# AmandineBtto/NeRAF

Measured on AMD Instinct MI355X. Metric: field-samples/sec (rays + RIR STFT bins), higher is better.
Workload: dtype f16; 1 GPU; RAF FurnishedRoom joint training step (BASELINE configs[2]): 4096 rays + 2048 RIR slices x 513 bins per GPU; radiance + grid refresh + ResNet3D + NAcF + STFT loss, backward, GradScaler + fused Adam...; rays_per_gpu=4096, slices_per_gpu=2048, global_rays=4096, global_slices=2048, parallelism=dp1, distinct_resident_batches=16, deterministic=True

## Files before the change

### include/neraf_hip.h

```cpp
#ifndef NERAF_HIP_H
#define NERAF_HIP_H

#include <stddef.h>
#include <stdint.h>

#ifdef __cplusplus
extern "C" {
#endif

typedef struct neraf_ctx neraf_ctx;
typedef void* neraf_stream_t;

enum {
  NERAF_OK = 0,
  NERAF_EINVAL = -1,
  NERAF_EHIP = -2,
  NERAF_ENOGPU = -3,
  NERAF_ESTATE = -4
};

#define NERAF_ABI_VERSION 1

int neraf_abi_version(void);
int neraf_ctx_create(neraf_ctx** out, int device);
// ... 76 lines not shown
int neraf_stft_loss_bwd(neraf_ctx* ctx, const float* pred, const float* gt, size_t n, size_t n_total,
                        int loss_type, const float* sums, const float* g_sc, const float* g_mag, const float* weights, float extra,
                        float* dpred, neraf_stream_t stream);

typedef struct neraf_grid_desc {
  int n_levels;
  int base_res;
  int max_res;
  int log2_hashmap_size;
  int n_features;
} neraf_grid_desc;

int neraf_grid_layout(const neraf_grid_desc* g, float* scales, int* resolutions, uint32_t* sizes, uint32_t* offsets);

int neraf_hash_encode(neraf_ctx* ctx, const neraf_grid_desc* g, const void* table_f16, const float* x01, long long n_points,
                      float* enc, neraf_stream_t stream);

int neraf_sample_uniform(neraf_ctx* ctx, int R, int S, float near, float far, const float* jitter, uint64_t jitter_seed,
                         float* s_bins, float* e_bins, neraf_stream_t stream);

int neraf_proposal_density(neraf_ctx* ctx, const neraf_grid_desc* g, const void* table_f16, const void* mlp_f16,
                           const float* origins, const float* dirs, const float* e_bins, int R, int S,
                           float avg_density, int coherent_rays, float* density, neraf_stream_t stream);
int neraf_proposal_density_ex(neraf_ctx* ctx, const neraf_grid_desc* g, const void* table_f16, const void* mlp_f16,
                              const float* origins, const float* dirs, const float* e_bins, int64_t e_row_stride, int R, int S,
                              float avg_density, int coherent_rays, float* density, neraf_stream_t stream);

int neraf_pdf_resample(neraf_ctx* ctx, const float* density, const float* s_bins, const float* e_bins, int R, int S,
                       float anneal, const float* jitter, uint64_t jitter_seed, int n_new, float near, float far, float* weights,
                       float* s_new, float* e_new, neraf_stream_t stream);
int neraf_pdf_resample_ex(neraf_ctx* ctx, const float* density, const float* s_bins, const float* e_bins, int64_t bins_row_stride,
                          int R, int S, float anneal, const float* jitter, uint64_t jitter_seed, int n_new, float near, float far,
                          float* weights, float* s_new, float* e_new, neraf_stream_t stream);

int neraf_pdf_resample_mm(neraf_ctx* ctx, const float* density, const float* s_bins, const float* e_bins, int64_t bins_row_stride,
                          int R, int S, float anneal, const float* jitter, uint64_t jitter_seed, int n_new, float near, float far,
                          float* weights, float* s_new, float* e_new, void* minmax_scratch, size_t scratch_bytes, int minmax_mode,
                          neraf_stream_t stream);

int neraf_field_query(neraf_ctx* ctx, const neraf_grid_desc* g, const void* table_f16, const void* wfrag_f16,
                      const void* emb_f16, const float* origins, const float* dirs, const float* e_bins,
                      const int32_t* cam_idx, int R, int S, int mode, const float* aabb_host, float avg_density,
                      int avg_row, int coherent_rays, float* rgb, float* density, neraf_stream_t stream);

int neraf_field_query_train(neraf_ctx* ctx, const neraf_grid_desc* g, const void* table_f16, const void* wfrag_f16,
                            const void* emb_f16, const float* origins, const float* dirs, const float* e_bins,
                            const int32_t* cam_idx, int R, int S, int mode, const float* aabb_host, float avg_density,
                            int avg_row, float* rgb, float* density, void* enc_out, void* denc_out, neraf_stream_t stream);

int neraf_composite(neraf_ctx* ctx, const float* density, const float* rgb, const float* e_bins, int R, int S,
                    int training, float* weights, float* rgb_out, float* depth, float* expected, float* acc,
                    void* scratch, size_t scratch_bytes, neraf_stream_t stream);
int neraf_composite_mm(neraf_ctx* ctx, const float* density, const float* rgb, const float* e_bins, int R, int S,
                       int training, float* weights, float* rgb_out, float* depth, float* expected, float* acc,
                       const void* minmax, neraf_stream_t stream);

int neraf_render_loss(neraf_ctx* ctx, const float* density, const float* rgb_s, const float* e_bins, const float* s_bins,
                      const float* gt_rgb, int R, int S, float distortion_mult, const float* up3, float* d_rgb_s,
                      float* d_density, float* d_density_dist, float* sums, neraf_stream_t stream);
int neraf_interlevel_loss(neraf_ctx* ctx, const float* c_bins, const float* w_fine, int S2, const float* p_bins,
                          const float* p_ebins, const float* p_density, int Sp, int R, float mult, const float* up3,
                          float* d_density, float* sums, neraf_stream_t stream);
size_t neraf_proposal_backward_scratch_bytes(int R, int S, int n_levels);
int neraf_proposal_backward(neraf_ctx* ctx, const neraf_grid_desc* g, const void* table_f16, const void* mlp_f16,
                            const float* origins, const float* dirs, const float* e_bins, const float* d_density, int R,
                            int S, float avg_density, float* table_grad, float* w_grad, void* scratch, size_t scratch_bytes,
                            neraf_stream_t stream);
size_t neraf_field_backward_dump_bytes(int R, int S);
int neraf_field_backward(neraf_ctx* ctx, const neraf_grid_desc* g, const void* table_f16, const void* wfrag_f16,
                         const void* wfrag_bwd_f16, const void* emb_f16, const float* origins, const float* dirs,
                         const float* e_bins, const int32_t* cam_idx, int R, int S, int mode, const float* aabb_host,
                         float avg_density, int avg_row, const float* density, const float* d_rgb, const float* d_density,
                         float* table_grad, float* emb_grad, float* const* w_grads, void* dump, void* splitk_ws,
                         size_t splitk_bytes, neraf_stream_t stream);

int neraf_field_backward_runs(neraf_ctx* ctx, const neraf_grid_desc* g, const void* table_f16, const void* wfrag_f16,
                         const void* wfrag_bwd_f16, const void* emb_f16, const float* origins, const float* dirs,
                         const float* e_bins, const int32_t* cam_idx, int R, int S, int mode, const float* aabb_host,
                         float avg_density, int avg_row, const float* density, const float* d_rgb, const float* d_density,
                         float* table_grad, float* emb_grad, float* const* w_grads, void* dump, void* splitk_ws,
                         size_t splitk_bytes, int pos_run, neraf_stream_t stream);

int neraf_field_backward_rays(neraf_ctx* ctx, const neraf_grid_desc* g, const void* table_f16, const void* wfrag_f16,
                              const void* wfrag_bwd_f16, const void* emb_f16, const float* origins, const float* dirs,
                              const float* e_bins, const int32_t* cam_idx, int R, int S, int mode, const float* aabb_host,
                              float avg_density, int avg_row, const float* density, const float* d_rgb, const float* d_density,
                              float* table_grad, float* emb_grad, float* const* w_grads, void* dump, void* splitk_ws,
                              size_t splitk_bytes, float* d_rays, neraf_stream_t stream);
int neraf_field_backward_ex(neraf_ctx* ctx, const neraf_grid_desc* g, const void* table_f16, const void* wfrag_f16,
                            const void* wfrag_bwd_f16, const void* emb_f16, const float* origins, const float* dirs,
                            const float* e_bins, const int32_t* cam_idx, int R, int S, int mode, const float* aabb_host,
                            float avg_density, int avg_row, const float* density, const float* d_rgb, const float* d_density,
                            float* table_grad, float* emb_grad, float* const* w_grads, void* dump, void* splitk_ws,
                            size_t splitk_bytes, int pos_run, float* d_rays, const void* enc_saved, const void* denc_saved,
                            void* acc_scratch, int accumulate, int emb_rows, neraf_stream_t stream);
int neraf_proposal_backward_ex(neraf_ctx* ctx, const neraf_grid_desc* g, const void* table_f16, const void* mlp_f16,
                               const float* origins, const float* dirs, const float* e_bins, const float* d_density, int R, int S,
                               float avg_density, float* table_grad, float* w0_grad, float* w1_grad, void* scratch,
                               size_t scratch_bytes, void* acc_scratch, float* d_rays, neraf_stream_t stream);
int neraf_proposal_backward_rays(neraf_ctx* ctx, const neraf_grid_desc* g, const void* table_f16, const void* mlp_f16,
                                 const float* origins, const float* dirs, const float* e_bins, const float* d_density, int R,
                                 int S, float avg_density, float* table_grad, float* w_grad, void* scratch, size_t scratch_bytes,
                                 float* d_rays, neraf_stream_t stream);

int neraf_grid_refresh_write(neraf_ctx* ctx, const float* rgb, const float* density, int n, int ndirs, float delta,
                             float* grid, size_t nvox, size_t start, neraf_stream_t stream);

int neraf_grid_refresh_vals(neraf_ctx* ctx, const float* rgb, const float* density, int n, int ndirs, int cell_major, float delta,
                            float* vals, float* grid, size_t nvox, size_t start, neraf_stream_t stream);
int neraf_grid_refresh_vals_bwd(neraf_ctx* ctx, const float* dvals, const float* density, int n, int ndirs, int cell_major,
                                float delta, float* d_rgb, float* d_density, neraf_stream_t stream);

int neraf_refresh_origins(neraf_ctx* ctx, const float* coords, int n, int ndirs, const float* aabb_host, float* out,
                          neraf_stream_t stream);

typedef struct neraf_resnet3d_desc {
  int grid_size;
  int in_channels;
  int n_features;
} neraf_resnet3d_desc;

int neraf_resnet3d_num_convs(const neraf_resnet3d_desc* d);
size_t neraf_resnet3d_packed_bytes(const neraf_resnet3d_desc* d);
size_t neraf_resnet3d_workspace_bytes(const neraf_resnet3d_desc* d);
double neraf_resnet3d_forward_flops(const neraf_resnet3d_desc* d);
int neraf_resnet3d_pack_weights(neraf_ctx* ctx, const neraf_resnet3d_desc* d, const float* const* conv_w, void* packed,
                                neraf_stream_t stream);
int neraf_resnet3d_fwd(neraf_ctx* ctx, const neraf_resnet3d_desc* d, const void* packed, const float* const* bn,
                       const float* grid, void* workspace, float* feat, int use_batch_stats, size_t win_start, int win_cells,
                       neraf_stream_t stream);
int neraf_resnet3d_update_running_stats(neraf_ctx* ctx, const neraf_resnet3d_desc* d, const void* workspace,
                                        float* const* bn, float momentum, int64_t* const* num_batches_tracked,
                                        neraf_stream_t stream);

size_t neraf_resnet3d_bwd_packed_bytes(const neraf_resnet3d_desc* d);
size_t neraf_resnet3d_bwd_workspace_bytes(const neraf_resnet3d_desc* d);
int neraf_resnet3d_pack_weights_bwd(neraf_ctx* ctx, const neraf_resnet3d_desc* d, const float* const* conv_w, void* packed_t,
                                    neraf_stream_t stream);
int neraf_resnet3d_bwd(neraf_ctx* ctx, const neraf_resnet3d_desc* d, const void* packed_t, const float* const* conv_w,
                       const float* const* bn, void* workspace, void* bwd_workspace, const float* dfeat,
                       float* const* w_grads, float* const* bn_grads, size_t cell_start, int n_cells, int n_ch,
                       float* dgrid_cells, neraf_stream_t stream);
int neraf_resnet3d_bwd_reset(neraf_ctx* ctx, void* bwd_workspace);
int neraf_resnet3d_bwd_chain_state(neraf_ctx* ctx, const neraf_resnet3d_desc* d, const void* bwd_workspace, int32_t* e_out,
                                   float* amax_out, int n, int32_t* info2, neraf_stream_t stream);

int neraf_manifest_enable(neraf_ctx* ctx, int on);
int neraf_manifest_get(neraf_ctx* ctx, int index, char* name, int name_cap, double* flops, double* rbytes, double* wbytes);

int neraf_debug_conv_bn_relu_stage(neraf_ctx* ctx, int cin, int cin_real, int cout, int k, int stride, int pad, int din,
                                   const void* x_f16, const float* w, const float* gamma, const float* beta, const float* g,
                                   void* y_f16, float* dx, float* dw, float* dgamma, float* dbeta, neraf_stream_t stream);

int neraf_camera_rays(neraf_ctx* ctx, const float* c2w, const float* fx, const float* fy, const float* cx, const float* cy,
                      const float* distortion, int n_cams,
                      const int64_t* cam_idx, int cam_single, const float* coords, int R, int width, float* origins, float* dirs,
                      int64_t* cam_out, neraf_stream_t stream);
int neraf_camera_apply(neraf_ctx* ctx, const float* pose_adjustment, const int32_t* cam_idx, const float* origins, const float* dirs,
                       int R, float* origins_out, float* dirs_out, int n_cameras, float w_trans, float w_rot, float* reg_out3,
                       neraf_stream_t stream);
int neraf_camera_apply_bwd(neraf_ctx* ctx, const float* pose_adjustment, const int32_t* cam_idx, const float* dirs,
                           const float* d_origins, const float* d_dirs, int g_stride, int R, int n_cameras, float w_trans, float w_rot,
                           const float* g_reg, float* d_pose, neraf_stream_t stream);

int neraf_loss_sum_scale(neraf_ctx* ctx, const float* const* terms, int n, const float* scale, float* out2, neraf_stream_t stream);
int neraf_vision_loss_finalize(neraf_ctx* ctx, const float* sums, const float* k3, float* out4, neraf_stream_t stream);
int neraf_vision_bwd_prologue(neraf_ctx* ctx, const float* u_rgb, const float* u_dens, const float* u_dist, const float* g_rgb,
                              const float* g_inter, const float* g_dist, size_t n_samples, float* d_rgb, float* d_dens, float* up3,
                              float* d_rays, size_t n_ray_floats, float* sums4, neraf_stream_t stream);

int neraf_cvt_f16_segments(neraf_ctx* ctx, const float* const* src, void* const* dst, const long long* len, int n,
                           neraf_stream_t stream);
int neraf_gather_f16(neraf_ctx* ctx, const float* const* src, const long long* src_len, int nsrc, const long long* index, void* dst,
                     long long n, neraf_stream_t stream);

int neraf_resnet3d_debug_locate(const neraf_resnet3d_desc* d, int kind, int index, size_t* offset, int* rows, int* cols);

int neraf_debug_bn_apply(neraf_ctx* ctx, const void* x, const float* const* bn5, int rep, const void* xr, const float* const* bn5_r,
                         int rep_r, const void* res, int M, int Mpad, int C, int relu, float* fin_w, float* fin_w_r, void* out,
                         int form, neraf_stream_t stream);
int neraf_debug_maxpool_fwd(neraf_ctx* ctx, const void* x, const float* const* bn5, int rep, int din, void* out, void* arg,
                            neraf_stream_t stream);
int neraf_debug_maxpool_bwd(neraf_ctx* ctx, const void* arg, const void* g, int din, void* dpost, neraf_stream_t stream);

uint32_t neraf_debug_fastdiv(uint32_t n, uint32_t d);

int neraf_fused_adam_chunk(void);
int neraf_grads_nonfinite(neraf_ctx* ctx, const void* table, const void* g_ptrs, const int* blk_tensor, const int* blk_chunk,
                          int n_blocks, float* found_inf, const void* const* g_ptrs_host, int n_ptrs, int found_is_zero,
                          neraf_stream_t stream);
int neraf_amp_update_scale(neraf_ctx* ctx, float* scale, int32_t* growth_tracker, const float* const* found_infs, int n,
                           double growth_factor, double backoff_factor, int growth_interval, int clear_flags, neraf_stream_t stream);
int neraf_fused_adam(neraf_ctx* ctx, const void* table, const void* g_ptrs, const int* blk_tensor, const int* blk_chunk,
                     int n_blocks, const float* group_lr, int n_groups, int n_tensors, double beta1, double beta2, double eps,
                     float* step, const float* grad_scale, const float* found_inf, neraf_stream_t stream);

int neraf_fused_adam_dual(neraf_ctx* ctx, const void* table, const void* g_ptrs, const int* blk_tensor, const int* blk_chunk,
                          int n_blocks, const float* group_lr, int n_groups, int n_tensors, double beta1, double beta2, double eps,
                          float* step, const float* grad_scale, const float* found_inf, const void* dual, const float* step0,
                          const float* found_inf0, const float* group_lr0, int n_groups0, const void* const* g_ptrs_host, int n_ptrs,
                          neraf_stream_t stream);

#ifdef __cplusplus
}
#endif
#endif
```

### neraf_amd/_lib.py

```python
from __future__ import annotations

import ctypes as C
import os
from typing import Dict, Optional

_HERE = os.path.dirname(os.path.abspath(__file__))
LIB_PATH = os.environ.get("NERAF_HIP_LIB") or os.path.join(_HERE, "libneraf_hip.so")

_lib: Optional[C.CDLL] = None
_ctxs: Dict[int, C.c_void_p] = {}

c_fpp = C.POINTER(C.c_void_p)


class GridDesc(C.Structure):
    _fields_ = [("n_levels", C.c_int), ("base_res", C.c_int), ("max_res", C.c_int), ("log2_hashmap_size", C.c_int),
                ("n_features", C.c_int)]


class ResnetDesc(C.Structure):
    _fields_ = [("grid_size", C.c_int), ("in_channels", C.c_int), ("n_features", C.c_int)]


class NacfDesc(C.Structure):
# ... 14 lines not shown
                                         C.c_void_p]),
    "neraf_gemm_f16_stream": (C.c_int, [C.c_void_p, C.c_void_p, C.c_int, C.c_void_p, C.c_int, C.c_int, C.c_int, C.c_int, C.c_int, C.c_int,
                                        C.c_float, C.c_void_p, C.c_void_p, C.c_int, C.c_void_p, C.c_int, C.c_void_p, C.c_int, C.c_void_p,
                                        C.c_int, C.c_void_p, C.c_void_p, C.c_int, C.c_int, C.c_int, C.c_int, C.c_int, C.c_void_p]),
    "neraf_gemm_bf16": (C.c_int, [C.c_void_p, C.c_void_p, C.c_int, C.c_void_p, C.c_int, C.c_int, C.c_int, C.c_int,
                                  C.c_int, C.c_int, C.c_float, C.c_void_p, C.c_int, C.c_void_p, C.c_int, C.c_void_p,
                                  C.c_int, C.c_void_p, C.c_int, C.c_void_p]),
    "neraf_gemm_bf16_tn": (C.c_int, [C.c_void_p, C.c_void_p, C.c_void_p, C.c_int, C.c_int, C.c_int, C.c_void_p, C.c_void_p, C.c_size_t,
                                     C.c_void_p]),
    "neraf_fused_adam_chunk": (C.c_int, []),
    "neraf_grads_nonfinite": (C.c_int, [C.c_void_p, C.c_void_p, C.c_void_p, C.c_void_p, C.c_void_p, C.c_int, C.c_void_p, C.c_void_p, C.c_int,
                                        C.c_int, C.c_void_p]),
    "neraf_fused_adam": (C.c_int, [C.c_void_p, C.c_void_p, C.c_void_p, C.c_void_p, C.c_void_p, C.c_int, C.c_void_p, C.c_int, C.c_int,
                                   C.c_double, C.c_double, C.c_double, C.c_void_p, C.c_void_p, C.c_void_p, C.c_void_p]),
    "neraf_fused_adam_dual": (C.c_int, [C.c_void_p, C.c_void_p, C.c_void_p, C.c_void_p, C.c_void_p, C.c_int, C.c_void_p, C.c_int, C.c_int,
                                        C.c_double, C.c_double, C.c_double, C.c_void_p, C.c_void_p, C.c_void_p, C.c_void_p, C.c_void_p,
                                        C.c_void_p, C.c_void_p, C.c_int, C.c_void_p, C.c_int, C.c_void_p]),
    "neraf_nacf_packed_bytes": (C.c_size_t, [C.POINTER(NacfDesc)]),
    "neraf_nacf_workspace_bytes": (C.c_size_t, [C.POINTER(NacfDesc), C.c_int, C.c_int]),
    "neraf_nacf_pack_weights": (C.c_int, [C.c_void_p, C.POINTER(NacfDesc), c_fpp, C.c_void_p, C.c_void_p]),
    "neraf_nacf_encode_queries": (C.c_int, [C.c_void_p, C.POINTER(NacfDesc), C.c_void_p, C.c_void_p, C.c_void_p,
                                            C.c_void_p, C.POINTER(C.c_float), C.c_int, C.c_int, C.c_void_p, C.c_int,
                                            C.c_void_p]),
    "neraf_nacf_encode_queries_ex": (C.c_int, [C.c_void_p, C.POINTER(NacfDesc), C.c_void_p, C.c_void_p, C.c_void_p,
                                               C.c_void_p, C.c_int, C.POINTER(C.c_float), C.c_int, C.c_int, C.c_void_p, C.c_int,
                                               C.c_void_p]),
    "neraf_nacf_fwd": (C.c_int, [C.c_void_p, C.POINTER(NacfDesc), C.c_void_p, c_fpp, C.c_void_p, C.c_int, C.c_void_p,
                                 C.c_void_p, C.c_int, C.c_void_p]),
    "neraf_nacf_fwd_dense": (C.c_int, [C.c_void_p, C.POINTER(NacfDesc), C.c_void_p, C.c_void_p, C.c_int, C.c_void_p,
                                       C.c_void_p, C.c_int, C.c_void_p]),
    "neraf_nacf_bwd": (C.c_int, [C.c_void_p, C.POINTER(NacfDesc), C.c_void_p, c_fpp, C.c_void_p, C.c_int, C.c_void_p,
                                 C.c_void_p, c_fpp, C.c_void_p, C.c_void_p, C.c_void_p]),
    "neraf_nacf_bwd_dense": (C.c_int, [C.c_void_p, C.POINTER(NacfDesc), C.c_void_p, C.c_int, C.c_void_p, C.c_void_p,
                                       c_fpp, C.c_void_p, C.c_void_p, C.c_void_p]),
    "neraf_stft_loss_fwd": (C.c_int, [C.c_void_p, C.c_void_p, C.c_void_p, C.c_size_t, C.c_int, C.c_void_p, C.c_void_p,
                                      C.c_void_p]),
    "neraf_stft_loss_sums": (C.c_int, [C.c_void_p, C.c_void_p, C.c_void_p, C.c_size_t, C.c_int, C.c_void_p, C.c_void_p]),
    "neraf_stft_loss_finalize": (C.c_int, [C.c_void_p, C.c_void_p, C.c_size_t, C.c_void_p, C.c_void_p, C.c_void_p]),
    "neraf_stft_loss_bwd": (C.c_int, [C.c_void_p, C.c_void_p, C.c_void_p, C.c_size_t, C.c_size_t, C.c_int, C.c_void_p,
                                      C.c_void_p, C.c_void_p, C.c_void_p, C.c_float, C.c_void_p, C.c_void_p]),
    "neraf_prof_event_overhead": (C.c_int, [C.c_void_p, C.c_void_p, C.c_void_p, C.POINTER(C.c_double)]),
    "neraf_graph_stats": (C.c_int, [C.c_void_p, C.POINTER(C.c_int), C.POINTER(C.c_int)]),
    "neraf_prof_enable": (C.c_int, [C.c_void_p, C.c_int]),
    "neraf_prof_summary": (C.c_int, [C.c_void_p, C.c_int, C.POINTER(C.c_double), C.POINTER(C.c_int), C.POINTER(C.c_double)]),
    "neraf_prof_summary_ex": (C.c_int, [C.c_void_p, C.c_int, C.POINTER(C.c_double), C.POINTER(C.c_int), C.POINTER(C.c_double),
                                        C.POINTER(C.c_double)]),
    "neraf_prof_kernel_name": (C.c_char_p, [C.c_int]),
    "neraf_grid_layout": (C.c_int, [C.POINTER(GridDesc), C.POINTER(C.c_float), C.POINTER(C.c_int), C.POINTER(C.c_uint32),
                                    C.POINTER(C.c_uint32)]),
    "neraf_hash_encode": (C.c_int, [C.c_void_p, C.POINTER(GridDesc), C.c_void_p, C.c_void_p, C.c_longlong, C.c_void_p, C.c_void_p]),
    "neraf_sample_uniform": (C.c_int, [C.c_void_p, C.c_int, C.c_int, C.c_float, C.c_float, C.c_void_p, C.c_uint64, C.c_void_p,
                                       C.c_void_p, C.c_void_p]),
    "neraf_proposal_density": (C.c_int, [C.c_void_p, C.POINTER(GridDesc), C.c_void_p, C.c_void_p, C.c_void_p, C.c_void_p,
                                         C.c_void_p, C.c_int, C.c_int, C.c_float, C.c_int, C.c_void_p, C.c_void_p]),
    "neraf_proposal_density_ex": (C.c_int, [C.c_void_p, C.POINTER(GridDesc), C.c_void_p, C.c_void_p, C.c_void_p, C.c_void_p,
                                            C.c_void_p, C.c_int64, C.c_int, C.c_int, C.c_float, C.c_int, C.c_void_p, C.c_void_p]),
    "neraf_pdf_resample_ex": (C.c_int, [C.c_void_p, C.c_void_p, C.c_void_p, C.c_void_p, C.c_int64, C.c_int, C.c_int, C.c_float,
                                        C.c_void_p, C.c_uint64, C.c_int, C.c_float, C.c_float, C.c_void_p, C.c_void_p, C.c_void_p,
                                        C.c_void_p]),
    "neraf_pdf_resample_mm": (C.c_int, [C.c_void_p, C.c_void_p, C.c_void_p, C.c_void_p, C.c_int64, C.c_int, C.c_int, C.c_float,
                                        C.c_void_p, C.c_uint64, C.c_int, C.c_float, C.c_float, C.c_void_p, C.c_void_p, C.c_void_p,
                                        C.c_void_p, C.c_size_t, C.c_int, C.c_void_p]),
    "neraf_composite_mm": (C.c_int, [C.c_void_p, C.c_void_p, C.c_void_p, C.c_void_p, C.c_int, C.c_int, C.c_int, C.c_void_p,
                                     C.c_void_p, C.c_void_p, C.c_void_p, C.c_void_p, C.c_void_p, C.c_void_p]),
    "neraf_pdf_resample": (C.c_int, [C.c_void_p, C.c_void_p, C.c_void_p, C.c_void_p, C.c_int, C.c_int, C.c_float,
                                     C.c_void_p, C.c_uint64, C.c_int, C.c_float, C.c_float, C.c_void_p, C.c_void_p, C.c_void_p,
                                     C.c_void_p]),
    "neraf_field_query": (C.c_int, [C.c_void_p, C.POINTER(GridDesc), C.c_void_p, C.c_void_p, C.c_void_p, C.c_void_p,
                                    C.c_void_p, C.c_void_p, C.c_void_p, C.c_int, C.c_int, C.c_int, C.POINTER(C.c_float),
                                    C.c_float, C.c_int, C.c_int, C.c_void_p, C.c_void_p, C.c_void_p]),
    "neraf_field_query_train": (C.c_int, [C.c_void_p, C.POINTER(GridDesc), C.c_void_p, C.c_void_p, C.c_void_p, C.c_void_p,
                                          C.c_void_p, C.c_void_p, C.c_void_p, C.c_int, C.c_int, C.c_int, C.POINTER(C.c_float),
                                          C.c_float, C.c_int, C.c_void_p, C.c_void_p, C.c_void_p, C.c_void_p, C.c_void_p]),
    "neraf_render_loss": (C.c_int, [C.c_void_p, C.c_void_p, C.c_void_p, C.c_void_p, C.c_void_p, C.c_void_p, C.c_int, C.c_int,
                                    C.c_float, C.c_void_p, C.c_void_p, C.c_void_p, C.c_void_p, C.c_void_p, C.c_void_p]),
    "neraf_interlevel_loss": (C.c_int, [C.c_void_p, C.c_void_p, C.c_void_p, C.c_int, C.c_void_p, C.c_void_p, C.c_void_p,
                                        C.c_int, C.c_int, C.c_float, C.c_void_p, C.c_void_p, C.c_void_p, C.c_void_p]),
    "neraf_proposal_backward_scratch_bytes": (C.c_size_t, [C.c_int, C.c_int, C.c_int]),
    "neraf_proposal_backward": (C.c_int, [C.c_void_p, C.POINTER(GridDesc), C.c_void_p, C.c_void_p, C.c_void_p, C.c_void_p,
                                          C.c_void_p, C.c_void_p, C.c_int, C.c_int, C.c_float, C.c_void_p, C.c_void_p,
                                          C.c_void_p, C.c_size_t, C.c_void_p]),
    "neraf_field_backward_dump_bytes": (C.c_size_t, [C.c_int, C.c_int]),
    "neraf_field_backward": (C.c_int, [C.c_void_p, C.POINTER(GridDesc), C.c_void_p, C.c_void_p, C.c_void_p, C.c_void_p,
                                       C.c_void_p, C.c_void_p, C.c_void_p, C.c_void_p, C.c_int, C.c_int, C.c_int,
                                       C.POINTER(C.c_float), C.c_float, C.c_int, C.c_void_p, C.c_void_p, C.c_void_p,
                                       C.c_void_p, C.c_void_p, c_fpp, C.c_void_p, C.c_void_p, C.c_size_t, C.c_void_p]),
    "neraf_field_backward_runs": (C.c_int, [C.c_void_p, C.POINTER(GridDesc), C.c_void_p, C.c_void_p, C.c_void_p, C.c_void_p,
                                            C.c_void_p, C.c_void_p, C.c_void_p, C.c_void_p, C.c_int, C.c_int, C.c_int,
                                            C.POINTER(C.c_float), C.c_float, C.c_int, C.c_void_p, C.c_void_p, C.c_void_p,
                                            C.c_void_p, C.c_void_p, c_fpp, C.c_void_p, C.c_void_p, C.c_size_t, C.c_int, C.c_void_p]),
    "neraf_field_backward_rays": (C.c_int, [C.c_void_p, C.POINTER(GridDesc), C.c_void_p, C.c_void_p, C.c_void_p, C.c_void_p,
                                            C.c_void_p, C.c_void_p, C.c_void_p, C.c_void_p, C.c_int, C.c_int, C.c_int,
                                            C.POINTER(C.c_float), C.c_float, C.c_int, C.c_void_p, C.c_void_p, C.c_void_p,
                                            C.c_void_p, C.c_void_p, c_fpp, C.c_void_p, C.c_void_p, C.c_size_t, C.c_void_p, C.c_void_p]),
    "neraf_field_backward_ex": (C.c_int, [C.c_void_p, C.POINTER(GridDesc), C.c_void_p, C.c_void_p, C.c_void_p, C.c_void_p,
                                          C.c_void_p, C.c_void_p, C.c_void_p, C.c_void_p, C.c_int, C.c_int, C.c_int,
                                          C.POINTER(C.c_float), C.c_float, C.c_int, C.c_void_p, C.c_void_p, C.c_void_p,
                                          C.c_void_p, C.c_void_p, c_fpp, C.c_void_p, C.c_void_p, C.c_size_t, C.c_int, C.c_void_p,
                                          C.c_void_p, C.c_void_p, C.c_void_p, C.c_int, C.c_int, C.c_void_p]),
    "neraf_proposal_backward_ex": (C.c_int, [C.c_void_p, C.POINTER(GridDesc), C.c_void_p, C.c_void_p, C.c_void_p, C.c_void_p,
                                             C.c_void_p, C.c_void_p, C.c_int, C.c_int, C.c_float, C.c_void_p, C.c_void_p, C.c_void_p,
                                             C.c_void_p, C.c_size_t, C.c_void_p, C.c_void_p, C.c_void_p]),
    "neraf_proposal_backward_rays": (C.c_int, [C.c_void_p, C.POINTER(GridDesc), C.c_void_p, C.c_void_p, C.c_void_p, C.c_void_p,
                                               C.c_void_p, C.c_void_p, C.c_int, C.c_int, C.c_float, C.c_void_p, C.c_void_p,
                                               C.c_void_p, C.c_size_t, C.c_void_p, C.c_void_p]),
    "neraf_grid_refresh_write": (C.c_int, [C.c_void_p, C.c_void_p, C.c_void_p, C.c_int, C.c_int, C.c_float, C.c_void_p,
                                           C.c_size_t, C.c_size_t, C.c_void_p]),
    "neraf_grid_refresh_vals": (C.c_int, [C.c_void_p, C.c_void_p, C.c_void_p, C.c_int, C.c_int, C.c_int, C.c_float, C.c_void_p,
                                          C.c_void_p, C.c_size_t, C.c_size_t, C.c_void_p]),
    "neraf_grid_refresh_vals_bwd": (C.c_int, [C.c_void_p, C.c_void_p, C.c_void_p, C.c_int, C.c_int, C.c_int, C.c_float, C.c_void_p,
                                              C.c_void_p, C.c_void_p]),
    "neraf_refresh_origins": (C.c_int, [C.c_void_p, C.c_void_p, C.c_int, C.c_int, C.POINTER(C.c_float), C.c_void_p, C.c_void_p]),
    "neraf_resnet3d_num_convs": (C.c_int, [C.POINTER(ResnetDesc)]),
    "neraf_resnet3d_packed_bytes": (C.c_size_t, [C.POINTER(ResnetDesc)]),
    "neraf_resnet3d_workspace_bytes": (C.c_size_t, [C.POINTER(ResnetDesc)]),
    "neraf_resnet3d_forward_flops": (C.c_double, [C.POINTER(ResnetDesc)]),
    "neraf_resnet3d_pack_weights": (C.c_int, [C.c_void_p, C.POINTER(ResnetDesc), c_fpp, C.c_void_p, C.c_void_p]),
    "neraf_resnet3d_fwd": (C.c_int, [C.c_void_p, C.POINTER(ResnetDesc), C.c_void_p, c_fpp, C.c_void_p, C.c_void_p,
                                     C.c_void_p, C.c_int, C.c_size_t, C.c_int, C.c_void_p]),
    "neraf_resnet3d_update_running_stats": (C.c_int, [C.c_void_p, C.POINTER(ResnetDesc), C.c_void_p, c_fpp, C.c_float, c_fpp,
                                                      C.c_void_p]),
    "neraf_resnet3d_bwd_packed_bytes": (C.c_size_t, [C.POINTER(ResnetDesc)]),
    "neraf_resnet3d_bwd_workspace_bytes": (C.c_size_t, [C.POINTER(ResnetDesc)]),
    "neraf_resnet3d_pack_weights_bwd": (C.c_int, [C.c_void_p, C.POINTER(ResnetDesc), c_fpp, C.c_void_p, C.c_void_p]),
    "neraf_manifest_enable": (C.c_int, [C.c_void_p, C.c_int]),
    "neraf_manifest_get": (C.c_int, [C.c_void_p, C.c_int, C.c_char_p, C.c_int, C.POINTER(C.c_double), C.POINTER(C.c_double), C.POINTER(C.c_double)]),
    "neraf_resnet3d_bwd_reset": (C.c_int, [C.c_void_p, C.c_void_p]),
    "neraf_resnet3d_bwd_chain_state": (C.c_int, [C.c_void_p, C.POINTER(ResnetDesc), C.c_void_p, C.POINTER(C.c_int32), C.POINTER(C.c_float),
                                                 C.c_int, C.POINTER(C.c_int32), C.c_void_p]),
    "neraf_resnet3d_bwd": (C.c_int, [C.c_void_p, C.POINTER(ResnetDesc), C.c_void_p, c_fpp, c_fpp, C.c_void_p, C.c_void_p,
                                     C.c_void_p, c_fpp, c_fpp, C.c_size_t, C.c_int, C.c_int, C.c_void_p, C.c_void_p]),
    "neraf_camera_rays": (C.c_int, [C.c_void_p] * 7 + [C.c_int, C.c_void_p, C.c_int, C.c_void_p, C.c_int, C.c_int,
                                    C.c_void_p, C.c_void_p, C.c_void_p, C.c_void_p]),
    "neraf_camera_apply": (C.c_int, [C.c_void_p, C.c_void_p, C.c_void_p, C.c_void_p, C.c_void_p, C.c_int, C.c_void_p, C.c_void_p, C.c_int,
                                     C.c_float, C.c_float, C.c_void_p, C.c_void_p]),
    "neraf_camera_apply_bwd": (C.c_int, [C.c_void_p, C.c_void_p, C.c_void_p, C.c_void_p, C.c_void_p, C.c_void_p, C.c_int, C.c_int, C.c_int,
                                         C.c_float, C.c_float, C.c_void_p, C.c_void_p, C.c_void_p]),
    "neraf_amp_update_scale": (C.c_int, [C.c_void_p, C.c_void_p, C.c_void_p, c_fpp, C.c_int, C.c_double, C.c_double, C.c_int, C.c_int,
                                         C.c_void_p]),
    "neraf_loss_sum_scale": (C.c_int, [C.c_void_p, c_fpp, C.c_int, C.c_void_p, C.c_void_p, C.c_void_p]),
    "neraf_vision_loss_finalize": (C.c_int, [C.c_void_p, C.c_void_p, C.c_void_p, C.c_void_p, C.c_void_p]),
    "neraf_vision_bwd_prologue": (C.c_int, [C.c_void_p] * 7 + [C.c_size_t, C.c_void_p, C.c_void_p, C.c_void_p, C.c_void_p, C.c_size_t,
                                            C.c_void_p, C.c_void_p]),
    "neraf_cvt_f16_segments": (C.c_int, [C.c_void_p, c_fpp, c_fpp, C.POINTER(C.c_longlong), C.c_int, C.c_void_p]),
    "neraf_gather_f16": (C.c_int, [C.c_void_p, c_fpp, C.POINTER(C.c_longlong), C.c_int, C.c_void_p, C.c_void_p, C.c_longlong, C.c_void_p]),
    "neraf_debug_fastdiv": (C.c_uint32, [C.c_uint32, C.c_uint32]),
    "neraf_resnet3d_debug_locate": (C.c_int, [C.POINTER(ResnetDesc), C.c_int, C.c_int, C.POINTER(C.c_size_t), C.POINTER(C.c_int),
                                              C.POINTER(C.c_int)]),
    "neraf_debug_bn_apply": (C.c_int, [C.c_void_p, C.c_void_p, c_fpp, C.c_int, C.c_void_p, c_fpp, C.c_int, C.c_void_p, C.c_int, C.c_int, C.c_int,
                                       C.c_int, C.c_void_p, C.c_void_p, C.c_void_p, C.c_int, C.c_void_p]),
    "neraf_debug_maxpool_fwd": (C.c_int, [C.c_void_p, C.c_void_p, c_fpp, C.c_int, C.c_int, C.c_void_p, C.c_void_p, C.c_void_p]),
    "neraf_debug_maxpool_bwd": (C.c_int, [C.c_void_p, C.c_void_p, C.c_void_p, C.c_int, C.c_void_p, C.c_void_p]),
    "neraf_debug_conv_bn_relu_stage": (C.c_int, [C.c_void_p] + [C.c_int] * 7 + [C.c_void_p] * 11),
    "neraf_composite": (C.c_int, [C.c_void_p, C.c_void_p, C.c_void_p, C.c_void_p, C.c_int, C.c_int, C.c_int, C.c_void_p,
                                  C.c_void_p, C.c_void_p, C.c_void_p, C.c_void_p, C.c_void_p, C.c_size_t, C.c_void_p]),
}


def load() -> C.CDLL:
    global _lib
    if _lib is not None:
        return _lib
    if not os.path.exists(LIB_PATH):
        raise RuntimeError(
            f"{LIB_PATH} is missing: build it with `python -c 'import __graft_entry__ as g; g.build()'` "
            "(or `make -C neraf_amd/csrc`).  neraf_amd has no CPU / eager fallback by design.")
    lib = C.CDLL(LIB_PATH)
    variant = "NERAF_HIP_LIB" in os.environ
    for name, (res, args) in SIGNATURES.items():
        try:
            fn = getattr(lib, name)
        except AttributeError:
            if not variant:
                raise
            setattr(lib, name, lambda *a, **k: 0)
            continue
        fn.restype = res
        fn.argtypes = args
    if lib.neraf_abi_version() != 1:
        raise RuntimeError("libneraf_hip ABI version mismatch")
    _lib = lib
    return lib


def ctx(device_index: int = 0) -> C.c_void_p:
    if device_index in _ctxs:
        return _ctxs[device_index]
    lib = load()
    h = C.c_void_p()
    rc = lib.neraf_ctx_create(C.byref(h), device_index)
    if rc != 0:
        raise RuntimeError(f"neraf_ctx_create(device={device_index}) failed with {rc}: no MI355X/gfx950 GPU visible; "
                           "the NeRAF hot path only runs on the HIP library (no fallback).")
    _ctxs[device_index] = h
    return h


def check(rc: int, device_index: int = 0) -> None:
    if rc != 0:
        msg = load().neraf_last_error(_ctxs.get(device_index)) if device_index in _ctxs else b""
        raise RuntimeError(f"libneraf_hip call failed ({rc}): {msg.decode() if msg else ''}")


def ptr_array(tensors) -> "C.Array":
    arr = (C.c_void_p * len(tensors))()
    for i, t in enumerate(tensors):
        arr[i] = t.data_ptr() if t is not None else None
    return arr


_HOST_F32 = {}


def host_f32(t):
    key = (t.data_ptr(), t._version, t.numel())
    hit = _HOST_F32.get(key)
    if hit is None:
        vals = [float(v) for v in t.detach().reshape(-1).cpu().tolist()]
        hit = ((C.c_float * len(vals))(*vals), t.untyped_storage())
        if len(_HOST_F32) > 64:
            _HOST_F32.clear()
        _HOST_F32[key] = hit
    return hit[0]
```

### neraf_amd/csrc/gemm_f16.hip

```cpp
#include "common.h"
#include <stdlib.h>
#include <type_traits>

namespace {

constexpr int BK = 64;

__device__ __forceinline__ float act_apply(float v, int act) {
  if (act == ACT_LEAKY) return v > 0.f ? v : 0.1f * v;
  if (act == ACT_TANH10) return 10.f * tanhf(v);
  if (act == ACT_RELU) return v > 0.f ? v : 0.f;
  return v;
}

template <bool BF> struct ET;
template <> struct ET<false> {
  typedef _Float16 s; typedef half8 v8; typedef half4 v4;
  static __device__ __forceinline__ f32x4 mfma(v8 a, v8 b, f32x4 c) { return __builtin_amdgcn_mfma_f32_16x16x32_f16(a, b, c, 0, 0, 0); }
};
template <> struct ET<true> {
  typedef __bf16 s; typedef bf16x8 v8; typedef bf16x4 v4;
  static __device__ __forceinline__ f32x4 mfma(v8 a, v8 b, f32x4 c) { return __builtin_amdgcn_mfma_f32_16x16x32_bf16(a, b, c, 0, 0, 0); }
};

template <int BM, int BN, int WAVES_M = 2>
struct Tile {
  static constexpr int NWAVES = WAVES_M * 2, NT = NWAVES * 64;
  static constexpr int WM = BM / WAVES_M, WN = BN / 2;
  static constexpr int FM = WM / 16, FN = WN / 16;
  static constexpr int A_CH = BM * 8 / NT, B_CH = BN * 8 / NT;
  static constexpr int STAGE_BYTES = (BM + BN) * 128;
  static constexpr int IMG16_LD = WN + 8;
  static constexpr int IMG16T_LD = WM + 8;
  static constexpr int IMG32_LD = WN + 4;
  static constexpr int C32_PASSES = (NWAVES * WM * IMG32_LD * 4 > 144 * 1024) ? 2 : 1;
  static constexpr int cmax(int a, int b) { return a > b ? a : b; }
  static constexpr int EPI_BYTES_WAVE = cmax(cmax(WM / C32_PASSES * IMG32_LD * 4, WM * IMG16_LD * 2), WN * IMG16T_LD * 2);
};

template <int BM>
__device__ __forceinline__ void tclass_coords(const ConvGeom& g, int m, int& z, int& y, int& x) {
  const int t = m / BM, cls = t & 7;
  const int r = (t >> 3) * BM + (m - t * BM);
  const int h = g.dout >> 1;
  const int x2 = r % h, y2 = (r / h) % h, z2 = r / (h * h);
  z = 2 * z2 + ((cls >> 2) & 1); y = 2 * y2 + ((cls >> 1) & 1); x = 2 * x2 + (cls & 1);
}
template <int BM, bool TC>
__device__ __forceinline__ int out_row(const GemmParams& p, int m) {
  if (!TC) return m;
  int z, y, x;
  tclass_coords<BM>(p.conv, m, z, y, x);
  return (z * p.conv.dout + y) * p.conv.dout + x;
}

template <int BM, int BN, bool BF, int WAVES_M = 2, bool TC = false>
__device__ __forceinline__ void gemm_epilogue(const GemmParams& p, f32x4 (&acc)[Tile<BM, BN, WAVES_M>::FM][Tile<BM, BN, WAVES_M>::FN],
                                              char* smem, int bm, int bn, int lane, int wave, int M, int N, float* C32, int ldc32) {
  using T = Tile<BM, BN, WAVES_M>;
  using E = typename ET<BF>::s;
  using E4 = typename ET<BF>::v4;
  constexpr int WM = T::WM, WN = T::WN, FM = T::FM, FN = T::FN;
  const int wm = wave >> 1, wn = wave & 1;
  const int frow = lane & 15, fq = lane >> 4;
  const int m_tile0 = bm * BM, n_tile0 = bn * BN;
  const float alpha = p.alpha_dev ? p.alpha * (*p.alpha_dev) : p.alpha;
  const int m_l = frow;
  const int n_l = fq * 4;
#pragma unroll
  for (int i = 0; i < FM; ++i) {
    const int m = m_tile0 + wm * WM + i * 16 + m_l;
#pragma unroll
    for (int j = 0; j < FN; ++j) {
      const int n0 = n_tile0 + wn * WN + j * 16 + n_l;
      f32x4 v = acc[i][j] * alpha;
      if (p.bias) {
        const f32x4 b = *reinterpret_cast<const f32x4*>(p.bias + n0);
        v += b;
      }
#pragma unroll
      for (int r = 0; r < 4; ++r) v[r] = act_apply(v[r], p.act);
      if (p.lmask) {
        const E4 mk = *reinterpret_cast<const E4*>(reinterpret_cast<const E*>(p.lmask) + (size_t)m * p.ldmask + n0);
#pragma unroll
        for (int r = 0; r < 4; ++r) v[r] *= ((float)mk[r] > 0.f) ? 1.f : p.mask_slope;
      }
      if (p.add16) {
        const E4 ad = *reinterpret_cast<const E4*>(reinterpret_cast<const E*>(p.add16) + (size_t)out_row<BM, TC>(p, m) * p.ldadd + n0);
#pragma unroll
        for (int r = 0; r < 4; ++r) v[r] += (float)ad[r];
      }
      if (p.bnb_mask) {
        const E4 mk = *reinterpret_cast<const E4*>(reinterpret_cast<const E*>(p.bnb_mask) + (size_t)m * p.ldbnb + n0);
#pragma unroll
        for (int r = 0; r < 4; ++r) if (!((float)mk[r] > 0.f)) v[r] = 0.f;
      }
#pragma unroll
      for (int r = 0; r < 4; ++r)
        if (m >= M || (n0 + r) >= N) v[r] = 0.f;
      acc[i][j] = v;
    }
  }

  char* img = smem + wave * T::EPI_BYTES_WAVE;
  const int m_w0 = m_tile0 + wm * WM, n_w0 = n_tile0 + wn * WN;

  if (p.colsum || p.colsumsq) {
    float* red = reinterpret_cast<float*>(smem);
    static_assert(2 * BN <= T::NT, "one thread per (sum | sumsq, column)");
#pragma unroll
    for (int j = 0; j < FN; ++j) {
      f32x4 s = f32x4{0.f, 0.f, 0.f, 0.f}, s2 = f32x4{0.f, 0.f, 0.f, 0.f};
      if (p.bnb_x) {
        const int n0 = n_tile0 + wn * WN + j * 16 + n_l;
        const f32x4 mu = *reinterpret_cast<const f32x4*>(p.bnb_fin + n0);
        f32x4 rs = *reinterpret_cast<const f32x4*>(p.bnb_fin + p.bnb_cpad + n0);
#pragma unroll
        for (int r = 0; r < 4; ++r) rs[r] = rsqrtf(rs[r] + 1e-5f);
#pragma unroll
        for (int i = 0; i < FM; ++i) {
          const int m = m_tile0 + wm * WM + i * 16 + m_l;
          const half4 xv = *reinterpret_cast<const half4*>(p.bnb_x + (size_t)out_row<BM, TC>(p, m) * p.ldbnb + n0);
          s += acc[i][j];
#pragma unroll
          for (int r = 0; r < 4; ++r) s2[r] += acc[i][j][r] * (((float)xv[r] - mu[r]) * rs[r]);
        }
      } else {
#pragma unroll
        for (int i = 0; i < FM; ++i) { s += acc[i][j]; s2 += acc[i][j] * acc[i][j]; }
      }
#pragma unroll
      for (int r = 0; r < 4; ++r) {
        float x = s[r], y = s2[r];
#pragma unroll
        for (int o = 1; o < 16; o <<= 1) { x += __shfl_xor(x, o); y += __shfl_xor(y, o); }
        if (frow == 0) {
          const int col = wn * WN + j * 16 + n_l + r;
          red[(wm * 2 + 0) * BN + col] = x;
          red[(wm * 2 + 1) * BN + col] = y;
        }
      }
    }
    __syncthreads();
    const int t = wave * 64 + lane;
    if (t < 2 * BN) {
      const int which = t / BN, col = t - which * BN;
      float v = 0.f;
#pragma unroll
      for (int w = 0; w < WAVES_M; ++w) v += red[(w * 2 + which) * BN + col];
      float* dst = which ? p.colsumsq : p.colsum;
      if (p.stat_det) {
        if (dst) dst[(size_t)(m_tile0 >> 5) * p.stat_stride + n_tile0 + col] = v;
      } else {
        const int rep = p.stat_rep > 1 ? (bm & (p.stat_rep - 1)) * p.stat_stride : 0;
        if (dst) atomicAdd(dst + rep + n_tile0 + col, v);
      }
    }
    __syncthreads();
  }

  if (p.C16) {
    E* im = reinterpret_cast<E*>(img);
#pragma unroll
    for (int i = 0; i < FM; ++i)
#pragma unroll
      for (int j = 0; j < FN; ++j) {
        E4 h;
#pragma unroll
        for (int r = 0; r < 4; ++r) h[r] = (E)acc[i][j][r];
        *reinterpret_cast<E4*>(im + (i * 16 + m_l) * T::IMG16_LD + j * 16 + n_l) = h;
      }
    __syncthreads();
    constexpr int CPR = WN / 8;
    static_assert((WM * CPR) % 64 == 0 || WM * CPR < 64, "whole wave-instructions (or one partial one)");
#pragma unroll
    for (int it = 0; it < (WM * CPR + 63) / 64; ++it) {
      const int idx = it * 64 + lane, row = idx / CPR, ch = idx - row * CPR;
      if (WM * CPR < 64 && idx >= WM * CPR) break;
      const uint4 d = *reinterpret_cast<const uint4*>(im + row * T::IMG16_LD + ch * 8);
      *reinterpret_cast<uint4*>(p.C16 + (size_t)out_row<BM, TC>(p, m_w0 + row) * p.ldc16 + n_w0 + ch * 8) = d;
    }
    __syncthreads();
  }

  if (p.C16T) {
    E* im = reinterpret_cast<E*>(img);
#pragma unroll
    for (int i = 0; i < FM; ++i)
#pragma unroll
      for (int j = 0; j < FN; ++j)
#pragma unroll
        for (int r = 0; r < 4; ++r)
          im[(j * 16 + n_l + r) * T::IMG16T_LD + i * 16 + m_l] = (E)acc[i][j][r];
    __syncthreads();
    constexpr int CPR = WM / 8;
    static_assert((WN * CPR) % 64 == 0 || WN * CPR < 64, "whole wave-instructions (or one partial one)");
#pragma unroll
    for (int it = 0; it < (WN * CPR + 63) / 64; ++it) {
      const int idx = it * 64 + lane, row = idx / CPR, ch = idx - row * CPR;
      if (WN * CPR < 64 && idx >= WN * CPR) break;
      const uint4 d = *reinterpret_cast<const uint4*>(im + row * T::IMG16T_LD + ch * 8);
      *reinterpret_cast<uint4*>(p.C16T + (size_t)(n_w0 + row) * p.ldc16t + m_w0 + ch * 8) = d;
    }
    __syncthreads();
  }

  if (C32) {
    float* im = reinterpret_cast<float*>(img);
    constexpr int FMP = FM / T::C32_PASSES, ROWS = WM / T::C32_PASSES;
#pragma unroll
    for (int pass = 0; pass < T::C32_PASSES; ++pass) {
      if (pass) __syncthreads();
#pragma unroll
      for (int i = 0; i < FMP; ++i)
#pragma unroll
        for (int j = 0; j < FN; ++j)
          *reinterpret_cast<f32x4*>(im + (i * 16 + m_l) * T::IMG32_LD + j * 16 + n_l) = acc[pass * FMP + i][j];
      __syncthreads();
      const int m_p0 = m_w0 + pass * ROWS;
      if (WN % 64 == 0) {
#pragma unroll 4
        for (int row = 0; row < ROWS; ++row) {
          const int m = m_p0 + row;
          if (m >= M) break;
#pragma unroll
          for (int c0 = 0; c0 < WN; c0 += 64) {
            const int n = n_w0 + c0 + lane;
            if (n < N) {
              float* dst = C32 + (size_t)m * ldc32 + n;
              *dst = im[row * T::IMG32_LD + c0 + lane] + (p.c32_beta ? *dst : 0.f);
            }
          }
        }
      } else {
        static_assert((ROWS * WN) % 64 == 0, "whole wave-instructions");
#pragma unroll 4
        for (int it = 0; it < ROWS * WN / 64; ++it) {
          const int idx = it * 64 + lane, row = idx / WN, col = idx - row * WN;
          const int m = m_p0 + row, n = n_w0 + col;
          if (m < M && n < N) {
            float* dst = C32 + (size_t)m * ldc32 + n;
            *dst = im[row * T::IMG32_LD + col] + (p.c32_beta ? *dst : 0.f);
          }
        }
      }
    }
  }
}

template <int N> __device__ __forceinline__ void wait_vmcnt() { asm volatile("s_waitcnt vmcnt(%0)" ::"i"(N) : "memory"); }
template <int LOADS, int MAXT>
__device__ __forceinline__ void wait_tiles(int after) {
  static_assert(MAXT * LOADS <= 63, "vmcnt is a 6-bit counter");
  if constexpr (MAXT <= 0) { wait_vmcnt<0>(); }
  else {
    if (after >= MAXT) wait_vmcnt<MAXT * LOADS>();
    else wait_tiles<LOADS, MAXT - 1>(after);
  }
}

template <int BM, int BN, int NST>
struct PipeTile {
  using T = Tile<BM, BN>;
  static constexpr int LDS_BYTES =
      (NST * T::STAGE_BYTES > T::NWAVES * T::EPI_BYTES_WAVE) ? NST * T::STAGE_BYTES : T::NWAVES * T::EPI_BYTES_WAVE;
};

template <int BM, int BN, int NST, int LOADER, int KS, bool BF, bool TC = false, int NW = 4, bool GRP = false>
__global__ __launch_bounds__(NW * 64) void gemm_f16_nt_pipe_kernel(GemmParams p, int splits) {
  using T = Tile<BM, BN>;
  using E8 = typename ET<BF>::v8;
  constexpr int WM = T::WM, WN = T::WN, FM = T::FM, FN = T::FN;
  constexpr int KH = NW / 4, NTH = NW * 64;
  static_assert((NW == 4 || NW == 8) && T::A_CH % KH == 0 && T::B_CH % KH == 0, "4 waves, or 8 with whole chunks per thread");
  constexpr int A_CH = T::A_CH / KH, B_CH = T::B_CH / KH;
  constexpr int LOADS = A_CH + B_CH;
  extern __shared__ __attribute__((aligned(16))) char smem[];

  const int tid = threadIdx.x;
  const int lane = tid & 63;
  const int wave8 = __builtin_amdgcn_readfirstlane(tid >> 6);
  const int wave = wave8 & 3, kh = wave8 >> 2;
  const int wm = wave >> 1, wn = wave & 1;

  int tiles_m = p.Mpad / BM, tiles_n = p.Npad / BN;
  const int nblocks = GRP ? (int)gridDim.x : tiles_m * tiles_n * splits;
  int bid = blockIdx.x;
  {
    const int q = nblocks >> 3, r = nblocks & 7;
    const int xcd = bid & 7, idx = bid >> 3;
    bid = (xcd < r ? xcd * (q + 1) : r * (q + 1) + (xcd - r) * q) + idx;
  }
  const half_t* Ag = p.A; const half_t* Bg0 = p.B;
  float* C32g = p.C32; int Mg = p.M, Ng = p.N, ldc32g = p.ldc32, grp = 0;
  if constexpr (GRP) {
    while (grp + 1 < p.ngroups && bid >= p.grp[grp + 1].tile_begin * splits) ++grp;
    const GemmParams::Group& G = p.grp[grp];
    bid -= G.tile_begin * splits;
    tiles_m = (G.M + BM - 1) / BM; tiles_n = (G.N + BN - 1) / BN;
    Ag = G.A; Bg0 = G.B; C32g = G.C32; Mg = G.M; Ng = G.N; ldc32g = G.ldc32;
  }
  const int split = bid % splits;
  bid /= splits;
  constexpr int GROUP_M = 4;
  const int group = bid / (GROUP_M * tiles_n);
  const int first_m = group * GROUP_M;
  const int gsz = (tiles_m - first_m) < GROUP_M ? (tiles_m - first_m) : GROUP_M;
  const int in_group = bid - group * GROUP_M * tiles_n;
  const int bm = first_m + in_group % gsz;
  const int bn = in_group / gsz;

  constexpr bool tclass = LOADER == 1 && TC;
  int t0z = 0, t0y = 0, t0x = 0, cy = KS, cx = KS;
  int nk_total = p.K / BK;
  if (tclass) {
    const int cls = bm & 7, padc = -p.conv.pad;
    t0z = (((cls >> 2) & 1) + padc) & 1; t0y = (((cls >> 1) & 1) + padc) & 1; t0x = ((cls & 1) + padc) & 1;
    const int cz = t0z < KS ? (KS - t0z + 1) >> 1 : 0;
    cy = t0y < KS ? (KS - t0y + 1) >> 1 : 0; cx = t0x < KS ? (KS - t0x + 1) >> 1 : 0;
    nk_total = cz * cy * cx * (p.conv.cin >> 6);
    if (nk_total == 0 && p.add16 == p.C16 && !p.C16T && !p.C32 && !p.colsum && !p.colsumsq && splits == 1) return;
  }
  const int per = (nk_total + splits - 1) / splits;
  const int k_begin = split * per;
  const int k_end = (k_begin + per) < nk_total ? (k_begin + per) : nk_total;
  const int nk = k_end > k_begin ? k_end - k_begin : 0;

  const half_t* Bg = Bg0 + (size_t)bn * BN * p.ldb;
  const half_t* b_src[B_CH];
#pragma unroll
  for (int i = 0; i < B_CH; ++i) {
    const int c = i * NTH + tid, row = c >> 3, lc = (c & 7) ^ (row & 7);
    b_src[i] = Bg + (size_t)row * p.ldb + lc * 8;
  }
  const half_t* a_src[A_CH];
  int az[A_CH], ay[A_CH], ax[A_CH], alc[A_CH];
#pragma unroll
  for (int i = 0; i < A_CH; ++i) {
    const int c = i * NTH + tid, row = c >> 3, lc = (c & 7) ^ (row & 7);
    alc[i] = lc;
    az[i] = ay[i] = ax[i] = 0;
    a_src[i] = nullptr;
    if (LOADER == 0) {
      a_src[i] = Ag + (size_t)(bm * BM + row) * p.lda + lc * 8;
    } else {
      const int m = bm * BM + row;
      const int d = p.conv.dout;
      int x = m % d, y = (m / d) % d, z = m / (d * d);
      if (tclass) tclass_coords<BM>(p.conv, m, z, y, x);
      az[i] = z * p.conv.stride - p.conv.pad; ay[i] = y * p.conv.stride - p.conv.pad; ax[i] = x * p.conv.stride - p.conv.pad;
    }
  }
  const bool fastc = LOADER == 1 && (tclass || p.conv.tstride != 2) && nk_total > 0;
  int c_off[A_CH];
  unsigned c_msk[A_CH];
  int jz = 0, jy = 0, jx = 0, jcb = 0;
  const int lim_y = tclass ? cy : KS, lim_x = tclass ? cx : KS;
  const int tsgn = (LOADER == 1 && p.conv.tflip) ? -1 : 1;
  if (fastc) {
    const int cpb = p.conv.cin >> 6, din = p.conv.din;
    int t = k_begin / cpb;
    jcb = k_begin - t * cpb;
    jx = t % lim_x; t /= lim_x; jy = t % lim_y; jz = t / lim_y;
#pragma unroll
    for (int i = 0; i < A_CH; ++i) {
      int bz = az[i], by = ay[i], bx = ax[i];
      if (tclass) { bz = (bz - t0z) >> 1; by = (by - t0y) >> 1; bx = (bx - t0x) >> 1; }
      unsigned m = 0;
#pragma unroll
      for (int a = 0; a < KS; ++a) {
        m |= ((unsigned)(bz + tsgn * a) < (unsigned)din ? 1u : 0u) << a;
        m |= ((unsigned)(by + tsgn * a) < (unsigned)din ? 1u : 0u) << (8 + a);
        m |= ((unsigned)(bx + tsgn * a) < (unsigned)din ? 1u : 0u) << (16 + a);
      }
      c_msk[i] = m;
      c_off[i] = ((bz * din + by) * din + bx) * p.conv.cin + alc[i] * 8;
    }
  }

  typedef __attribute__((address_space(3))) void* lds_ptr_t;
  typedef const __attribute__((address_space(1))) void* gbl_ptr_t;
  auto issue = [&](int kt, int stage) {
    char* sa = smem + stage * T::STAGE_BYTES + wave8 * 1024;
    char* sb = sa + BM * 128;
    int kb = kt;
    if (LOADER == 0) {
#pragma unroll
      for (int i = 0; i < A_CH; ++i)
        __builtin_amdgcn_global_load_lds((gbl_ptr_t)(a_src[i] + (size_t)kt * BK), (lds_ptr_t)(sa + i * (NW * 1024)), 16, 0, 0);
    } else if (LOADER == 1 && fastc) {
      const int cpb = p.conv.cin >> 6, din = p.conv.din;
      const unsigned sel = (1u << jz) | (1u << (8 + jy)) | (1u << (16 + jx));
      const int toff = tsgn * ((jz * din + jy) * din + jx) * p.conv.cin + jcb * 64;
      const int rz = tclass ? t0z + 2 * jz : jz, ry = tclass ? t0y + 2 * jy : jy, rx = tclass ? t0x + 2 * jx : jx;
      kb = ((rz * KS + ry) * KS + rx) * cpb + jcb;
#pragma unroll
      for (int i = 0; i < A_CH; ++i) {
        const half_t* src = (c_msk[i] & sel) == sel ? p.A + (c_off[i] + toff) : p.conv.zero_page;
        __builtin_amdgcn_global_load_lds((gbl_ptr_t)src, (lds_ptr_t)(sa + i * (NW * 1024)), 16, 0, 0);
      }
      if (++jcb == cpb) { jcb = 0; if (++jx == lim_x) { jx = 0; if (++jy == lim_y) { jy = 0; ++jz; } } }
    } else if (LOADER == 1) {
      const int cpb = p.conv.cin >> 6;
      int tap = kt / cpb;
      const int cb = kt - tap * cpb;
      int dz = tap / (KS * KS), dy = (tap / KS) % KS, dx = tap % KS;
      if (tclass) {
        dx = t0x + 2 * (tap % cx); dy = t0y + 2 * ((tap / cx) % cy); dz = t0z + 2 * (tap / (cx * cy));
        tap = (dz * KS + dy) * KS + dx;
        kb = tap * cpb + cb;
      }
      const int din = p.conv.din;
      const int sdz = p.conv.tflip ? -dz : dz, sdy = p.conv.tflip ? -dy : dy, sdx = p.conv.tflip ? -dx : dx;
      const bool half_grid = p.conv.tstride == 2;
#pragma unroll
      for (int i = 0; i < A_CH; ++i) {
        int iz = az[i] + sdz, iy = ay[i] + sdy, ix = ax[i] + sdx;
        bool ok = true;
        if (half_grid) { ok = ((iz | iy | ix) & 1) == 0; iz >>= 1; iy >>= 1; ix >>= 1; }
        ok = ok && (unsigned)iz < (unsigned)din && (unsigned)iy < (unsigned)din && (unsigned)ix < (unsigned)din;
        const half_t* src = ok ? p.A + ((size_t)(iz * din + iy) * din + ix) * p.conv.cin + cb * 64 + alc[i] * 8 : p.conv.zero_page;
        __builtin_amdgcn_global_load_lds((gbl_ptr_t)src, (lds_ptr_t)(sa + i * (NW * 1024)), 16, 0, 0);
      }
    } else {
      const int din = p.conv.din;
#pragma unroll
      for (int i = 0; i < A_CH; ++i) {
        const int tap = kt * 8 + alc[i];
        const int dz = tap / (KS * KS), dy = (tap / KS) % KS, dx = tap % KS;
        const int iz = az[i] + dz, iy = ay[i] + dy, ix = ax[i] + dx;
        const bool ok = tap < KS * KS * KS && (unsigned)iz < (unsigned)din && (unsigned)iy < (unsigned)din && (unsigned)ix < (unsigned)din;
        const half_t* src = ok ? p.A + ((size_t)(iz * din + iy) * din + ix) * 8 : p.conv.zero_page;
        __builtin_amdgcn_global_load_lds((gbl_ptr_t)src, (lds_ptr_t)(sa + i * (NW * 1024)), 16, 0, 0);
      }
    }
#pragma unroll
    for (int i = 0; i < B_CH; ++i)
      __builtin_amdgcn_global_load_lds((gbl_ptr_t)(b_src[i] + (size_t)kb * BK), (lds_ptr_t)(sb + i * (NW * 1024)), 16, 0, 0);
  };

  const int frow = lane & 15, fq = lane >> 4;
  const int a_row_off = (wm * WM + frow) * 128;
  const int b_row_off = (wn * WN + frow) * 128;
  int ch_off[2];
  ch_off[0] = ((0 + fq) ^ (frow & 7)) * 16;
  ch_off[1] = ((4 + fq) ^ (frow & 7)) * 16;

  f32x4 acc[FM][FN];
#pragma unroll
  for (int i = 0; i < FM; ++i)
#pragma unroll
    for (int j = 0; j < FN; ++j) acc[i][j] = f32x4{0.f, 0.f, 0.f, 0.f};

#pragma unroll
  for (int s0 = 0; s0 < NST - 1; ++s0)
    if (s0 < nk) issue(k_begin + s0, s0);

  int stage = 0;
  for (int kt = 0; kt < nk; ++kt) {
    const int after = nk - 1 - kt;
    wait_tiles<LOADS, NST - 2>(after);
    __builtin_amdgcn_s_barrier();
    if (kt + NST - 1 < nk) {
      int st2 = stage + NST - 1; if (st2 >= NST) st2 -= NST;
      issue(k_begin + kt + NST - 1, st2);
    }
    const char* sa = smem + stage * T::STAGE_BYTES;
    const char* sb = sa + BM * 128;
#pragma unroll
    for (int ks0 = 0; ks0 < 2 / KH; ++ks0) {
      const int ks = NW == 8 ? kh : ks0;
      E8 xa[FM], wb[FN];
#pragma unroll
      for (int i = 0; i < FM; ++i)
        xa[i] = *reinterpret_cast<const E8*>(sa + a_row_off + i * 16 * 128 + ch_off[ks]);
#pragma unroll
      for (int j = 0; j < FN; ++j)
        wb[j] = *reinterpret_cast<const E8*>(sb + b_row_off + j * 16 * 128 + ch_off[ks]);
#pragma unroll
      for (int i = 0; i < FM; ++i)
#pragma unroll
        for (int j = 0; j < FN; ++j)
          acc[i][j] = ET<BF>::mfma(wb[j], xa[i], acc[i][j]);
    }
    if (++stage == NST) stage = 0;
  }
  __syncthreads();
  if constexpr (NW == 8) {
    f32x4* pr = reinterpret_cast<f32x4*>(smem) + wave * (FM * FN * 64);
    if (kh == 1) {
#pragma unroll
      for (int i = 0; i < FM; ++i)
#pragma unroll
        for (int j = 0; j < FN; ++j) pr[(i * FN + j) * 64 + lane] = acc[i][j];
    }
    __syncthreads();
    if (kh == 1) return;
#pragma unroll
    for (int i = 0; i < FM; ++i)
#pragma unroll
      for (int j = 0; j < FN; ++j) acc[i][j] += pr[(i * FN + j) * 64 + lane];
    __syncthreads();
  }

  if (splits > 1) {
    float* slab = p.splitk_ws + ((size_t)grp * splits + split) * p.Mpad * p.Npad;
#pragma unroll
    for (int i = 0; i < FM; ++i)
#pragma unroll
      for (int j = 0; j < FN; ++j) {
        const int m = bm * BM + wm * WM + i * 16 + frow;
        const int n0 = bn * BN + wn * WN + j * 16 + fq * 4;
        *reinterpret_cast<f32x4*>(slab + (size_t)m * p.Npad + n0) = acc[i][j];
      }
    return;
  }
  gemm_epilogue<BM, BN, BF, 2, tclass>(p, acc, smem, bm, bn, lane, wave, Mg, Ng, C32g, ldc32g);
}

template <int BM, int BN, int NST, bool BF>
__global__ __launch_bounds__(512) void gemm_f16_nt_wide_kernel(GemmParams p, int splits) {
  constexpr int WAVES_M = 4;
  using T = Tile<BM, BN, WAVES_M>;
  using E8 = typename ET<BF>::v8;
  constexpr int WM = T::WM, WN = T::WN, FM = T::FM, FN = T::FN;
  constexpr int NINSTR = (BM + BN) / 8, LBASE = NINSTR / 8, LREM = NINSTR % 8, LMAX = LBASE + (LREM ? 1 : 0);
  extern __shared__ __attribute__((aligned(16))) char smem[];

  const int tid = threadIdx.x;
  const int lane = tid & 63;
  const int wave = __builtin_amdgcn_readfirstlane(tid >> 6);
  const int wm = wave >> 1, wn = wave & 1;

  const int tiles_m = p.Mpad / BM, tiles_n = p.Npad / BN;
  const int nblocks = tiles_m * tiles_n * splits;
  int bid = blockIdx.x;
  {
    const int q = nblocks >> 3, r = nblocks & 7;
    const int xcd = bid & 7, idx = bid >> 3;
    bid = (xcd < r ? xcd * (q + 1) : r * (q + 1) + (xcd - r) * q) + idx;
  }
  const int split = bid % splits;
  bid /= splits;
  constexpr int GROUP_M = 4;
  const int group = bid / (GROUP_M * tiles_n);
  const int first_m = group * GROUP_M;
  const int gsz = (tiles_m - first_m) < GROUP_M ? (tiles_m - first_m) : GROUP_M;
  const int in_group = bid - group * GROUP_M * tiles_n;
  const int bm = first_m + in_group % gsz;
  const int bn = in_group / gsz;

  const int nk_total = p.K / BK;
  const int per = (nk_total + splits - 1) / splits;
  const int k_begin = split * per;
  const int k_end = (k_begin + per) < nk_total ? (k_begin + per) : nk_total;
  const int nk = k_end > k_begin ? k_end - k_begin : 0;

  const half_t* src[LMAX];
#pragma unroll
  for (int i = 0; i < LMAX; ++i) {
    int q = wave + 8 * i;
    if (q >= NINSTR) q = NINSTR - 1;
    const int row = q * 8 + (lane >> 3), lc = (lane & 7) ^ (lane >> 3);
    src[i] = (row < BM ? p.A + (size_t)(bm * BM + row) * p.lda : p.B + (size_t)(bn * BN + row - BM) * p.ldb) + lc * 8;
  }

  typedef __attribute__((address_space(3))) void* lds_ptr_t;
  typedef const __attribute__((address_space(1))) void* gbl_ptr_t;

  const int frow = lane & 15, fq = lane >> 4;
  const int a_row_off = (wm * WM + frow) * 128;
  const int b_row_off = (BM + wn * WN + frow) * 128;
  int ch_off[2];
  ch_off[0] = ((0 + fq) ^ (frow & 7)) * 16;
  ch_off[1] = ((4 + fq) ^ (frow & 7)) * 16;

  f32x4 acc[FM][FN];
#pragma unroll
  for (int i = 0; i < FM; ++i)
#pragma unroll
    for (int j = 0; j < FN; ++j) acc[i][j] = f32x4{0.f, 0.f, 0.f, 0.f};

  static_assert(NST == 3, "ring depth the phase schedule below is written for");
  auto kloop = [&](auto lw) {
    constexpr int L = decltype(lw)::value;
    auto issue = [&](int kt, int stage) {
      char* s = smem + stage * T::STAGE_BYTES + wave * 1024;
#pragma unroll
      for (int i = 0; i < L; ++i)
        __builtin_amdgcn_global_load_lds((gbl_ptr_t)(src[i] + (size_t)kt * BK), (lds_ptr_t)(s + i * 8192), 16, 0, 0);
    };
    if (nk > 0) issue(k_begin, 0);
    if (nk > 1) { issue(k_begin + 1, 1); wait_vmcnt<L>(); } else wait_vmcnt<0>();
    __builtin_amdgcn_s_barrier();
    if (wave >= 4) __builtin_amdgcn_s_barrier();
    int stage = 0;
    for (int k = 0; k < nk; ++k) {
      E8 xa[2][FM], wb[2][FN];
      const char* st = smem + stage * T::STAGE_BYTES;
      if (k + 2 < nk) issue(k_begin + k + 2, stage == 0 ? 2 : stage - 1);
#pragma unroll
      for (int ks = 0; ks < 2; ++ks) {
#pragma unroll
        for (int i = 0; i < FM; ++i)
          xa[ks][i] = *reinterpret_cast<const E8*>(st + a_row_off + i * 16 * 128 + ch_off[ks]);
#pragma unroll
        for (int j = 0; j < FN; ++j)
          wb[ks][j] = *reinterpret_cast<const E8*>(st + b_row_off + j * 16 * 128 + ch_off[ks]);
      }
      if (k + 2 < nk) wait_vmcnt<L>(); else wait_vmcnt<0>();
      asm volatile("s_waitcnt lgkmcnt(0)" ::: "memory");
      __builtin_amdgcn_s_barrier();
      __builtin_amdgcn_s_setprio(1);
#pragma unroll
      for (int ks = 0; ks < 2; ++ks)
#pragma unroll
        for (int i = 0; i < FM; ++i)
#pragma unroll
          for (int j = 0; j < FN; ++j)
            acc[i][j] = ET<BF>::mfma(wb[ks][j], xa[ks][i], acc[i][j]);
      __builtin_amdgcn_s_setprio(0);
      __builtin_amdgcn_s_barrier();
      if (++stage == NST) stage = 0;
    }
    if (wave < 4) __builtin_amdgcn_s_barrier();
  };
  if (LREM == 0 || wave < LREM) kloop(std::integral_constant<int, LMAX>{});
  else kloop(std::integral_constant<int, LBASE>{});
  __syncthreads();

  if (splits > 1) {
    float* slab = p.splitk_ws + (size_t)split * p.Mpad * p.Npad;
#pragma unroll
    for (int i = 0; i < FM; ++i)
#pragma unroll
      for (int j = 0; j < FN; ++j) {
        const int m = bm * BM + wm * WM + i * 16 + frow;
        const int n0 = bn * BN + wn * WN + j * 16 + fq * 4;
        *reinterpret_cast<f32x4*>(slab + (size_t)m * p.Npad + n0) = acc[i][j];
      }
    return;
  }
  gemm_epilogue<BM, BN, BF, WAVES_M>(p, acc, smem, bm, bn, lane, wave, p.M, p.N, p.C32, p.ldc32);
}

template <bool BF>
__global__ __launch_bounds__(256) void splitk_reduce_kernel(GemmParams p, int splits) {
  using E = typename ET<BF>::s;
  using E4 = typename ET<BF>::v4;
  __shared__ float tile[32][33];
  const int t = threadIdx.x;
  const int row = t >> 3, c4 = (t & 7) * 4;
  const int n0 = blockIdx.x * 32, m0 = blockIdx.y * 32;
  const int grp = blockIdx.z;
  float* C32 = p.C32; int M = p.M, N = p.N, ldc32 = p.ldc32;
  if (p.ngroups > 1) { C32 = p.grp[grp].C32; M = p.grp[grp].M; N = p.grp[grp].N; ldc32 = p.grp[grp].ldc32; }
  const float alpha = p.alpha_dev ? p.alpha * (*p.alpha_dev) : p.alpha;
  const size_t slab = (size_t)p.Mpad * p.Npad;
  const int m = m0 + row, n = n0 + c4;
  const float* src = p.splitk_ws + (size_t)grp * splits * slab + (size_t)m * p.Npad + n;
  f32x4 bias4 = f32x4{0.f, 0.f, 0.f, 0.f}, mu = bias4, var = bias4;
  E4 mk_l, ad, mk_b;
  half4 xv;
  if (p.bias) bias4 = *reinterpret_cast<const f32x4*>(p.bias + n);
  if (p.lmask) mk_l = *reinterpret_cast<const E4*>(reinterpret_cast<const E*>(p.lmask) + (size_t)m * p.ldmask + n);
  if (p.add16) ad = *reinterpret_cast<const E4*>(reinterpret_cast<const E*>(p.add16) + (size_t)m * p.ldadd + n);
  if (p.bnb_mask) mk_b = *reinterpret_cast<const E4*>(reinterpret_cast<const E*>(p.bnb_mask) + (size_t)m * p.ldbnb + n);
  if (p.bnb_x) {
    xv = *reinterpret_cast<const half4*>(p.bnb_x + (size_t)m * p.ldbnb + n);
    mu = *reinterpret_cast<const f32x4*>(p.bnb_fin + n);
    var = *reinterpret_cast<const f32x4*>(p.bnb_fin + p.bnb_cpad + n);
  }
  f32x4 v = f32x4{0.f, 0.f, 0.f, 0.f};
  int s = 0;
  for (; s + 8 <= splits; s += 8) {
    f32x4 a[8];
#pragma unroll
    for (int u = 0; u < 8; ++u) a[u] = *reinterpret_cast<const f32x4*>(src + (size_t)(s + u) * slab);
#pragma unroll
    for (int u = 0; u < 8; ++u) v += a[u];
  }
  for (; s < splits; ++s) v += *reinterpret_cast<const f32x4*>(src + (size_t)s * slab);
  v *= alpha;
  if (p.bias) v += bias4;
#pragma unroll
  for (int r = 0; r < 4; ++r) v[r] = act_apply(v[r], p.act);
  if (p.lmask) {
#pragma unroll
    for (int r = 0; r < 4; ++r) v[r] *= ((float)mk_l[r] > 0.f) ? 1.f : p.mask_slope;
  }
  if (p.add16) {
#pragma unroll
    for (int r = 0; r < 4; ++r) v[r] += (float)ad[r];
  }
  if (p.bnb_mask) {
#pragma unroll
    for (int r = 0; r < 4; ++r) if (!((float)mk_b[r] > 0.f)) v[r] = 0.f;
  }
#pragma unroll
  for (int r = 0; r < 4; ++r) {
    if (m >= M || (n + r) >= N) v[r] = 0.f;
    tile[row][c4 + r] = v[r];
  }
  __shared__ float tile2[32][33];
  if (p.bnb_x) {
#pragma unroll
    for (int r = 0; r < 4; ++r) tile2[row][c4 + r] = v[r] * (((float)xv[r] - mu[r]) * rsqrtf(var[r] + 1e-5f));
  }
  if (p.C16) {
    E4 h;
#pragma unroll
    for (int r = 0; r < 4; ++r) h[r] = (E)v[r];
    *reinterpret_cast<E4*>(reinterpret_cast<E*>(p.C16) + (size_t)m * p.ldc16 + n) = h;
  }
  if (C32 && m < M) {
    float* dst = C32 + (size_t)m * ldc32 + n;
    if (n + 3 < N && (reinterpret_cast<size_t>(dst) & 15) == 0) {
      f32x4 o = v;
      if (p.c32_beta) o += *reinterpret_cast<const f32x4*>(dst);
      *reinterpret_cast<f32x4*>(dst) = o;
    } else {
#pragma unroll
      for (int r = 0; r < 4; ++r) if (n + r < N) dst[r] = v[r] + (p.c32_beta ? dst[r] : 0.f);
    }
  }
  __syncthreads();
  const int tx = t & 31, ty = t >> 5;
  if (p.C16T) {
#pragma unroll
    for (int i = 0; i < 4; ++i) {
      const int nn = n0 + ty + i * 8, mm = m0 + tx;
      reinterpret_cast<E*>(p.C16T)[(size_t)nn * p.ldc16t + mm] = (E)tile[tx][ty + i * 8];
    }
  }
  if ((p.colsum || p.colsumsq) && ty < 2) {
    float cs = 0.f;
    if (ty == 0) {
#pragma unroll 8
      for (int i = 0; i < 32; ++i) cs += tile[i][tx];
    } else if (p.bnb_x) {
#pragma unroll 8
      for (int i = 0; i < 32; ++i) cs += tile2[i][tx];
    } else {
#pragma unroll 8
      for (int i = 0; i < 32; ++i) { const float x = tile[i][tx]; cs += x * x; }
    }
    float* dst = ty == 0 ? p.colsum : p.colsumsq;
    if (p.stat_det) {
      if (dst) dst[(size_t)blockIdx.y * p.stat_stride + n0 + tx] = cs;
    } else {
      const int rep = p.stat_rep > 1 ? (blockIdx.y & (p.stat_rep - 1)) * p.stat_stride : 0;
      if (dst) atomicAdd(dst + rep + n0 + tx, cs);
    }
  }
}

static void gemm_manifest(neraf_ctx* ctx, const GemmParams& p, int loader, int splits, int bm, int bn, double flops, bool wide = false, bool stream = false) {
  double out_elems = (double)p.M * p.N;
  double rA = loader == 0 ? (double)p.M * p.K * 2.0 : (double)p.conv.din * p.conv.din * p.conv.din * p.conv.cin * 2.0;
  double rB = (double)p.N * p.K * 2.0;
  const int ng = p.ngroups > 1 ? p.ngroups : 1;
  if (ng > 1) {
    out_elems = rA = rB = 0.0;
    for (int g = 0; g < ng; ++g) { out_elems += (double)p.grp[g].M * p.grp[g].N; rA += (double)p.grp[g].M * p.K * 2.0; rB += (double)p.grp[g].N * p.K * 2.0; }
  }
  const double epi_r = out_elems * 2.0 * ((p.add16 ? 1 : 0) + (p.lmask ? 1 : 0) + (p.bnb_mask ? 1 : 0) + (p.bnb_x ? 1 : 0));
  const double epi_w = out_elems * (2.0 * ((p.C16 ? 1 : 0) + (p.C16T ? 1 : 0)) + (p.C32 ? 4.0 : 0.0));
  const double slabs = (double)splits * ng * p.Mpad * p.Npad * 4.0;
  char nm[96];
  if (ng > 1)
    snprintf(nm, sizeof(nm), "gemm_f16_nt_pipe_kernel<%d, %d | plain, %d groups, %.0f results K=%d%s", bm, bn, ng, out_elems, p.K, splits > 1 ? " splitK" : "");
  else
    snprintf(nm, sizeof(nm), "%s<%d, %d | %s M=%d N=%d K=%d%s",
             stream ? "gemm_f16_nt_stream_kernel" : (wide ? "gemm_f16_nt_wide_kernel" : "gemm_f16_nt_pipe_kernel"), bm, bn,
             loader == 0 ? "plain" : (p.conv.tflip ? "dgrad" : "conv"), p.M, p.N, p.K, splits > 1 ? " splitK" : "");
  if (splits > 1) {
    neraf_node(ctx, nm, flops, rA + rB, slabs);
    neraf_node(ctx, "splitk_reduce_kernel | K-split slabs -> result", 0.0, slabs + epi_r, epi_w);
  } else {
    neraf_node(ctx, nm, flops, rA + rB + epi_r, epi_w);
  }
}

template <int BM, int BN, int NST, int LOADER, int KS, bool BF, bool TC = false, int NW = 4, bool GRP = false>
int launch_pipe(neraf_ctx* ctx, const GemmParams& p_in, int splits, hipStream_t stream) {
  using PT = PipeTile<BM, BN, NST>;
  GemmParams p = p_in;
  if ((p.ngroups > 1) != GRP) return neraf_fail(ctx, NERAF_EINVAL, "gemm: grouped launches take the grouped instantiation");
  int grp_tiles = 0;
  if (GRP) {
    for (int g = 0; g < p.ngroups; ++g) {
      p.grp[g].tile_begin = grp_tiles;
      grp_tiles += ((p.grp[g].M + BM - 1) / BM) * ((p.grp[g].N + BN - 1) / BN);
    }
  }
  static bool attr_set = false;
  if (!attr_set) {
    NERAF_HIP_CHECK(ctx, hipFuncSetAttribute(reinterpret_cast<const void*>(&gemm_f16_nt_pipe_kernel<BM, BN, NST, LOADER, KS, BF, TC, NW, GRP>),
                                             hipFuncAttributeMaxDynamicSharedMemorySize, PT::LDS_BYTES));
    attr_set = true;
  }
  const int ng = p.ngroups > 1 ? p.ngroups : 1;
  const int ntiles = GRP ? grp_tiles : (p.Mpad / BM) * (p.Npad / BN);
  double flops = 2.0 * p.M * p.N * p.K;
  if (ng > 1) { flops = 0.0; for (int g = 0; g < ng; ++g) flops += 2.0 * p.grp[g].M * p.grp[g].N * p.K; }
  const double exec_flops = (LOADER != 0 && p.conv.tstride > 1) ? (p.alg_flops > 0.0 ? p.alg_flops : flops) : flops;
  if (p.alg_flops > 0.0) flops = p.alg_flops;
  constexpr int kid = LOADER == 2 ? PROF_CONV_STEM
                      : LOADER == 1 ? (BM * BN == 128 * 128 ? PROF_CONV128 : (BM == 128 ? PROF_CONV12864 : (BF ? PROF_CONV64_BF16 : PROF_CONV)))
                                    : (BM * BN == 128 * 128 ? PROF_GEMM128 : (BM == 128 ? PROF_GEMM12864 : (BF ? PROF_GEMM64_BF16 : PROF_GEMM64)));
  ProfScope prof(ctx, stream, kid, flops, exec_flops);
  hipLaunchKernelGGL((gemm_f16_nt_pipe_kernel<BM, BN, NST, LOADER, KS, BF, TC, NW, GRP>), dim3(ntiles * splits), dim3(NW * 64), PT::LDS_BYTES,
                     stream, p, splits);
  NERAF_HIP_CHECK(ctx, hipGetLastError());
  if (ctx && ctx->manifest) gemm_manifest(ctx, p, LOADER, splits, BM, BN, flops);
  if (splits > 1) {
    hipLaunchKernelGGL(splitk_reduce_kernel<BF>, dim3(p.Npad / 32, p.Mpad / 32, ng), dim3(256), 0, stream, p, splits);
    NERAF_HIP_CHECK(ctx, hipGetLastError());
  }
  return NERAF_OK;
}


template <int BM, int BN, int NST, bool BF>
int launch_wide(neraf_ctx* ctx, const GemmParams& p, int splits, hipStream_t stream) {
  using T = Tile<BM, BN, 4>;
  constexpr int LDS_BYTES = (NST * T::STAGE_BYTES > T::NWAVES * T::EPI_BYTES_WAVE) ? NST * T::STAGE_BYTES : T::NWAVES * T::EPI_BYTES_WAVE;
  static_assert(LDS_BYTES <= 160 * 1024, "LDS budget");
  static bool attr_set = false;
  if (!attr_set) {
    NERAF_HIP_CHECK(ctx, hipFuncSetAttribute(reinterpret_cast<const void*>(&gemm_f16_nt_wide_kernel<BM, BN, NST, BF>),
                                             hipFuncAttributeMaxDynamicSharedMemorySize, LDS_BYTES));
    attr_set = true;
  }
  const int ntiles = (p.Mpad / BM) * (p.Npad / BN);
  ProfScope prof(ctx, stream, PROF_GEMM_WIDE, p.alg_flops > 0.0 ? p.alg_flops : 2.0 * p.M * p.N * p.K, 2.0 * p.M * p.N * p.K);
  hipLaunchKernelGGL((gemm_f16_nt_wide_kernel<BM, BN, NST, BF>), dim3(ntiles * splits), dim3(512), LDS_BYTES, stream, p, splits);
  NERAF_HIP_CHECK(ctx, hipGetLastError());
  if (ctx && ctx->manifest) gemm_manifest(ctx, p, 0, splits, BM, BN, p.alg_flops > 0.0 ? p.alg_flops : 2.0 * p.M * p.N * p.K, true);
  if (splits > 1) {
    hipLaunchKernelGGL(splitk_reduce_kernel<BF>, dim3(p.Npad / 32, p.Mpad / 32, 1), dim3(256), 0, stream, p, splits);
    NERAF_HIP_CHECK(ctx, hipGetLastError());
  }
  return NERAF_OK;
}

constexpr int kStreamRows = 64;
constexpr int stream_slices(int n) { return n > 128 ? n / 128 : 1; }

__device__ __forceinline__ float row16_sum(float x) {
  x += __builtin_bit_cast(float, __builtin_amdgcn_mov_dpp(__builtin_bit_cast(int, x), 0xB1, 0xF, 0xF, true));
  x += __builtin_bit_cast(float, __builtin_amdgcn_mov_dpp(__builtin_bit_cast(int, x), 0x4E, 0xF, 0xF, true));
  x += __builtin_bit_cast(float, __builtin_amdgcn_mov_dpp(__builtin_bit_cast(int, x), 0x141, 0xF, 0xF, true));
  x += __builtin_bit_cast(float, __builtin_amdgcn_mov_dpp(__builtin_bit_cast(int, x), 0x140, 0xF, 0xF, true));
  return x;
}

template <int N, int K, int CS, bool STATS>
__global__ __launch_bounds__(512) void gemm_f16_nt_stream_kernel(GemmParams p, int nblocks, int nrg) {
  constexpr int R = kStreamRows, KB = K / 32;
  constexpr int NW = N / CS, FNW = NW / 16;
  constexpr int CPRB = K / 8, SWZ = (CPRB - 1) & 15;
  constexpr int BCH = NW * CPRB / 512;
  constexpr int IC = 64, NPASS = NW / IC, FNP = IC / 16, IMG_LD = IC + 8, CPR = IC / 8, IMG_WAVE = 16 * IMG_LD * 2;
  static_assert(NW * K <= 16384 && NW % 64 == 0 && K % 64 == 0 && NW <= 128 && BCH >= 1, "a workgroup's slice of B must fit 32 KiB of LDS");
  static_assert(8 * 2 * NW * 4 <= 8 * IMG_WAVE, "the statistics' reduction re-uses the result images");
  __shared__ __attribute__((aligned(16))) char bs[NW * K * 2];
  __shared__ __attribute__((aligned(16))) char img_all[8 * IMG_WAVE];

  const int tid = threadIdx.x;
  const int lane = tid & 63;
  const int wave = __builtin_amdgcn_readfirstlane(tid >> 6);
  const int g = wave >> 2, w4 = wave & 3;
  const int frow = lane & 15, fq = lane >> 4;
  int rg, cs;
  if (CS > 1 && (nrg & 7) == 0) { const int q = blockIdx.x >> 3; cs = q % CS; rg = (q / CS) * 8 + (blockIdx.x & 7); }
  else { rg = blockIdx.x / CS; cs = blockIdx.x - rg * CS; }
  const int n_w0 = cs * NW;
  const int nv = 2 * nrg;

  auto load_a = [&](int blk, half8 (&xa)[KB]) {
    const half_t* src = p.A + (size_t)(blk * R + w4 * 16 + frow) * p.lda + fq * 8;
#pragma unroll
    for (int kb = 0; kb < KB; ++kb) xa[kb] = *reinterpret_cast<const half8*>(src + kb * 32);
  };

  int b = 2 * rg + g;
  half8 xa[KB], xn[KB];
  {
    uint4 bv[BCH];
#pragma unroll
    for (int i = 0; i < BCH; ++i) {
      const int c = i * 512 + tid, row = c / CPRB, ch = c % CPRB;
      bv[i] = *reinterpret_cast<const uint4*>(p.B + (size_t)(n_w0 + row) * p.ldb + ch * 8);
    }
    if (b < nblocks) load_a(b, xa);
#pragma unroll
    for (int i = 0; i < BCH; ++i) {
      const int c = i * 512 + tid, row = c / CPRB, ch = c % CPRB;
      *reinterpret_cast<uint4*>(bs + row * (K * 2) + ((ch ^ (row & SWZ)) * 16)) = bv[i];
    }
  }
  __syncthreads();

  const float alpha = p.alpha;
  half_t* im = reinterpret_cast<half_t*>(img_all + wave * IMG_WAVE);
  const char* b_lane = bs + frow * (K * 2);
  f32x4 s[STATS ? FNW : 1], s2[STATS ? FNW : 1];
#pragma unroll
  for (int j = 0; j < (STATS ? FNW : 1); ++j) s[j] = s2[j] = f32x4{0.f, 0.f, 0.f, 0.f};

  for (; b < nblocks; b += nv) {
    const int bnext = b + nv;
    if (bnext < nblocks) load_a(bnext, xn);

    f32x4 acc[FNW];
#pragma unroll
    for (int j = 0; j < FNW; ++j) acc[j] = f32x4{0.f, 0.f, 0.f, 0.f};
#pragma unroll
    for (int kb = 0; kb < KB; ++kb) {
      const int coff = ((kb * 4 + fq) ^ (frow & SWZ)) * 16;
#pragma unroll
      for (int j = 0; j < FNW; ++j) {
        const half8 wb = *reinterpret_cast<const half8*>(b_lane + j * 16 * (K * 2) + coff);
        acc[j] = __builtin_amdgcn_mfma_f32_16x16x32_f16(wb, xa[kb], acc[j], 0, 0, 0);
      }
    }

// ... 423 lines not shown
              const int vox = vbase + h_toff[i][j];
              src = loader == 2 ? Bb + vox * 8 : Bb + (vox * cin + h_cb[j] + lcs[i] * 8);
            }
          }
          __builtin_amdgcn_global_load_lds((gbl_ptr_t)src, (lds_ptr_t)(base + (MHc + j) * HALF + i * 4096), 16, 0, 0);
        }
      }
    };
#pragma unroll
    for (int s0 = 0; s0 < NST - 1; ++s0)
      if (s0 < nk) issue(k_begin + s0, s0);
    int stage = 0;
    for (int kt = 0; kt < nk; ++kt) {
      const int after = nk - 1 - kt;
      if (NST >= 4 && after >= 2) wait_vmcnt<2 * NP>();
      else if (NST >= 3 && after >= 1) wait_vmcnt<NP>();
      else wait_vmcnt<0>();
      __builtin_amdgcn_s_barrier();
      if (kt + NST - 1 < nk) {
        int st2 = stage + NST - 1; if (st2 >= NST) st2 -= NST;
        issue(k_begin + kt + NST - 1, st2);
      }
      char* sa = smem + stage * STAGE_BYTES + ha * HALF;
      char* sb = smem + stage * STAGE_BYTES + (MHc + hb) * HALF;
#pragma unroll
      for (int ks0 = 0; ks0 < (NW == 8 ? 1 : 2); ++ks0) {
        const int ks = NW == 8 ? kh : ks0;
        E8 fa[4], fb[4];
#pragma unroll
        for (int f = 0; f < 4; ++f) {
          const E4 a0 = TrRead<BF>::rd(sa + f_off[f] + ks * 4096);
          const E4 a1 = TrRead<BF>::rd(sa + f_off[f] + ks * 4096 + 512);
          const E4 b0 = TrRead<BF>::rd(sb + f_off[f] + ks * 4096);
          const E4 b1 = TrRead<BF>::rd(sb + f_off[f] + ks * 4096 + 512);
#pragma unroll
          for (int e = 0; e < 4; ++e) { fa[f][e] = a0[e]; fa[f][4 + e] = a1[e]; fb[f][e] = b0[e]; fb[f][4 + e] = b1[e]; }
        }
#pragma unroll
        for (int i = 0; i < 4; ++i)
#pragma unroll
          for (int j = 0; j < 4; ++j)
            acc[i][j] = ET<BF>::mfma(fb[j], fa[i], acc[i][j]);
      }
      if (++stage == NST) stage = 0;
    }
  };
  static_assert(NST == 2 || NST == 3 || NST == 4, "ring depths the waits are written for");
  if (MH == 2) body(std::integral_constant<int, 2>{}); else body(std::integral_constant<int, 1>{});

  const int b64 = bnw * NH + hb;
  const int frow = lane & 15, fq = lane >> 4;
  if constexpr (NW == 8) {
    constexpr int PR_LD = 68;
    __syncthreads();
    float* pr = reinterpret_cast<float*>(smem) + pw * (64 * PR_LD);
    if (kh == 1) {
#pragma unroll
      for (int i = 0; i < 4; ++i)
#pragma unroll
        for (int j = 0; j < 4; ++j)
          *reinterpret_cast<f32x4*>(pr + (i * 16 + frow) * PR_LD + j * 16 + fq * 4) = acc[i][j];
    }
    __syncthreads();
    if (kh == 1) return;
#pragma unroll
    for (int i = 0; i < 4; ++i)
#pragma unroll
      for (int j = 0; j < 4; ++j)
        acc[i][j] += *reinterpret_cast<const f32x4*>(pr + (i * 16 + frow) * PR_LD + j * 16 + fq * 4);
  }
  if (b64 >= n64) return;
  const int N = D.taps * cin, Npad = n64 * 64;
  const int m_base = (bm * MH + ha) * 64, n_base = b64 * 64;
  if (splits == 1 && D.taps == 1) {
    const float alpha = t.alpha_dev ? t.alpha_dev[D.ai] : 1.f;
#pragma unroll
    for (int i = 0; i < 4; ++i)
#pragma unroll
      for (int j = 0; j < 4; ++j) {
        const int m = m_base + i * 16 + frow;
        const int n0 = n_base + j * 16 + fq * 4;
#pragma unroll
        for (int r = 0; r < 4; ++r) {
          const int n = n0 + r;
          if (n < N && (n % cin) < D.cin_real) D.out[wg_out_index(D, m, n)] = acc[i][j][r] * alpha;
        }
      }
    return;
  }
  float* slab = t.slab + D.slab_off + (size_t)split * cout * Npad;
  constexpr int IM_LD = 68;
  __syncthreads();
  float* im = reinterpret_cast<float*>(smem) + pw * (64 * IM_LD);
#pragma unroll
  for (int i = 0; i < 4; ++i)
#pragma unroll
    for (int j = 0; j < 4; ++j)
      *reinterpret_cast<f32x4*>(im + (i * 16 + frow) * IM_LD + j * 16 + fq * 4) = acc[i][j];
  __builtin_amdgcn_wave_barrier();
  asm volatile("s_waitcnt lgkmcnt(0)" ::: "memory");
#pragma unroll
  for (int it = 0; it < 16; ++it) {
    const int row = it * 4 + (lane >> 4), col = (lane & 15) * 4;
    const f32x4 v = *reinterpret_cast<const f32x4*>(im + row * IM_LD + col);
    *reinterpret_cast<f32x4*>(slab + (size_t)(m_base + row) * Npad + n_base + col) = v;
  }
}

struct WgRedTable { int n; const float* alpha_dev; const float* slab; int tile_begin[kMaxWg + 1]; unsigned char item[kMaxWg]; };

__device__ __forceinline__ int wg_red_cb(const WgDesc& D) { return D.taps == 1 ? (D.cin < 256 ? D.cin : 256) : (D.taps > 32 ? D.cin : (D.cin < 128 ? D.cin : 128)); }

__global__ __launch_bounds__(256) void wgrad_grouped_reduce_kernel(WgTable t, WgRedTable r) {
  __shared__ float blk[3584];
  int lo = 0, hi = r.n - 1;
  const int bid = blockIdx.x;
  while (lo < hi) { const int mid = (lo + hi + 1) >> 1; if (r.tile_begin[mid] <= bid) lo = mid; else hi = mid - 1; }
  const WgDesc& D = t.d[r.item[lo]];
  const int tile = bid - r.tile_begin[lo];
  const int taps = D.taps, cin = D.cin, CB = wg_red_cb(D), cbs = cin / CB;
  const int m = tile / cbs, ci0 = (tile - m * cbs) * CB;
  const int Npad = D.tiles_n * 64;
  const size_t slab = (size_t)D.cout * Npad;
  const float* src = r.slab + D.slab_off + (size_t)m * Npad + ci0;
  const int splits = D.splits, pitch = taps + 1, q4 = CB >> 2, total4 = q4 * taps;
  for (int e = threadIdx.x; e < total4; e += 256) {
    const int tap = e / q4, c = (e - tap * q4) * 4;
    const float* p = src + tap * cin + c;
    f32x4 v = f32x4{0.f, 0.f, 0.f, 0.f};
    int s2 = 0;
    for (; s2 + 8 <= splits; s2 += 8) {
      f32x4 a[8];
#pragma unroll
      for (int u = 0; u < 8; ++u) a[u] = *reinterpret_cast<const f32x4*>(p + (size_t)(s2 + u) * slab);
#pragma unroll
      for (int u = 0; u < 8; ++u) v += a[u];
    }
    for (; s2 < splits; ++s2) v += *reinterpret_cast<const f32x4*>(p + (size_t)s2 * slab);
#pragma unroll
    for (int k = 0; k < 4; ++k) blk[taps == 1 ? c + k : (c + k) * pitch + tap] = v[k];
  }
  __syncthreads();
  const float alpha = r.alpha_dev ? r.alpha_dev[D.ai] : 1.f;
  const int creal = (D.cin_real - ci0) < CB ? (D.cin_real - ci0) : CB;
  float* dst = D.out + ((size_t)m * D.cin_real + ci0) * taps;
  for (int j = threadIdx.x; j < creal * taps; j += 256) {
    const int c = j / taps, tap = j - c * taps;
    dst[j] = blk[taps == 1 ? c : c * pitch + tap] * alpha;
  }
}

static const int kWide = [] { const char* e = getenv("NERAF_GEMM_WIDE"); return e ? atoi(e) : 1; }();
static const int kSplitMinK = [] { const char* e = getenv("NERAF_SPLIT_MIN_K"); return e ? atoi(e) : 32; }();

static bool conv_waves8() { static const bool v = [] { const char* e = getenv("NERAF_CONV_WAVES"); return e && atoi(e) == 8; }(); return v; }

constexpr int kStreamMinM = 32768;

template <int LOADER, int KS, bool BF>
int dispatch_tile(neraf_ctx* ctx, const GemmParams& p_in, hipStream_t stream) {
  GemmParams p = p_in;
  const int cus = ctx ? ctx->num_cus : 256;
  static const int kTclass = [] { const char* e = getenv("NERAF_DGRAD_TCLASS"); return e ? atoi(e) : 1; }();
  p.conv.tclass = 0;
  if (LOADER == 1 && kTclass && p.conv.tstride == 2 && p.conv.tflip && (p.conv.dout & 1) == 0 && p.ngroups <= 1 &&
      p.Mpad == p.conv.dout * p.conv.dout * p.conv.dout && (p.Mpad % 512) == 0 && (p.Npad % 64) == 0 && !p.lmask && !p.C16T && !p.C32 &&
      !p.colsum && !p.colsumsq) {
    p.conv.tclass = 1;
    if constexpr (LOADER == 1) { if (conv_waves8()) return launch_pipe<64, 64, 4, LOADER, KS, BF, true, 8>(ctx, p, 1, stream); }
    return launch_pipe<64, 64, 4, LOADER, KS, BF, LOADER == 1>(ctx, p, 1, stream);
  }
  if (p.stream_body == 1 && !(LOADER == 0 && !BF && stream_qualifies(p)))
    return neraf_fail(ctx, NERAF_EINVAL, "gemm: shape or epilogue outside the streaming body's");
  if constexpr (LOADER == 0 && !BF) {
    const bool det_stats = p.stat_det && (p.colsum || p.colsumsq);
    if (p.stream_body != 2 && stream_qualifies(p) && (p.stream_body == 1 || (p.Mpad >= kStreamMinM && !det_stats)))
      return launch_stream(ctx, p, stream);
  }
  const int nk = p.K / BK;
  int bm = 128, bn = 128;
  const bool can128 = (p.Mpad % 128) == 0 && (p.Npad % 128) == 0;
  static const int kTile64 = [] { const char* e = getenv("NERAF_CONV_TILE64"); return e ? atoi(e) : 1; }();
  if (p.tile_n == 64 && (p.Mpad % 128) == 0 && !(kTile64 && LOADER == 1)) { bm = 128; bn = 64; }
  else if (!can128 || (p.Mpad / 128) * (p.Npad / 128) < cus) { bm = 64; bn = 64; }
  const int ng = p.ngroups > 1 ? p.ngroups : 1;
  int ntiles = (p.Mpad / bm) * (p.Npad / bn);
  bool uniform = true;
  if (ng > 1) {
    bm = 64; bn = 64; ntiles = 0;
    for (int g = 0; g < ng; ++g) {
      ntiles += (round_up(p.grp[g].M, 64) / 64) * (round_up(p.grp[g].N, 64) / 64);
      uniform = uniform && round_up(p.grp[g].M, 64) == p.Mpad && round_up(p.grp[g].N, 64) == p.Npad;
    }
  }
  int splits = 1;
  static const int kOversub = [] { const char* e = getenv("NERAF_SPLIT_OVERSUB"); const int v = e ? atoi(e) : 2; return v < 1 ? 1 : (v > 4 ? 4 : v); }();
  if (p.splitk_ws && uniform && ntiles * 2 <= cus && nk >= kSplitMinK) {
    splits = ((LOADER != 0 && ntiles >= 64) ? kOversub : 1) * cus / ntiles;
    if (splits > nk / 4) splits = nk / 4;
    if (splits > 128) splits = 128;
    while (splits >= 2 && (size_t)splits * ng * p.Mpad * p.Npad * 4 > p.splitk_ws_bytes) splits >>= 1;
    if (splits < 2) splits = 1;
  }
  if (LOADER == 0 && ng == 1 && kWide && (p.Mpad % 256) == 0) {
    if ((p.Npad % 160) == 0 && (p.Mpad / 256) * (p.Npad / 160) * 4 >= cus * 3) return launch_wide<256, 160, 3, BF>(ctx, p, 1, stream);
    if ((p.Npad % 128) == 0 && (p.Mpad / 256) * (p.Npad / 128) >= cus) return launch_wide<256, 128, 3, BF>(ctx, p, 1, stream);
  }
  if (LOADER == 0 && ng == 1 && kWide && bm == 128 && bn == 128 && splits == 1 && ntiles < 2 * cus)
    return launch_wide<128, 128, 3, BF>(ctx, p, 1, stream);
  static const int kTile32 = [] { const char* e = getenv("NERAF_TILE32"); return e ? atoi(e) : 128; }();
  if constexpr (LOADER == 0) {
    if (ng > 1) {
      if (kTile32 && splits == 1 && ntiles <= kTile32) return launch_pipe<32, 32, 4, LOADER, KS, BF, false, 4, true>(ctx, p, 1, stream);
      return launch_pipe<64, 64, 4, LOADER, KS, BF, false, 4, true>(ctx, p, splits, stream);
    }
    if (kTile32 && splits == 1 && bm == 64 && bn == 64 && ntiles <= kTile32 && !p.C16T)
      return launch_pipe<32, 32, 4, LOADER, KS, BF>(ctx, p, 1, stream);
  }
  if (bm == 128 && bn == 128) return launch_pipe<128, 128, 2, LOADER, KS, BF>(ctx, p, splits, stream);
  if (bm == 128 && bn == 64) return launch_pipe<128, 64, 3, LOADER, KS, BF>(ctx, p, splits, stream);
  if constexpr (LOADER == 1) { if (conv_waves8()) return launch_pipe<64, 64, 4, LOADER, KS, BF, false, 8>(ctx, p, splits, stream); }
  return launch_pipe<64, 64, 4, LOADER, KS, BF>(ctx, p, splits, stream);
}

}

int launch_wgrad_grouped(neraf_ctx* ctx, const WgradItem* items, int n, const half_t* zero_page, float* slab_ws, size_t slab_bytes,
                         const float* alpha_dev, hipStream_t stream, bool bf16) {
  if (n <= 0 || n > kMaxWg || !items || !zero_page) return neraf_fail(ctx, NERAF_EINVAL, "wgrad_grouped: bad arguments");
  static const int nst = [] { const char* e = getenv("NERAF_WGRAD_NST"); const int v = e ? atoi(e) : 3; return v < 2 ? 2 : (v > 4 ? 4 : v); }();
  static const int rounds = [] { const char* e = getenv("NERAF_WGRAD_ROUNDS"); return e ? atoi(e) : 8; }();
  static const int wide = [] { const char* e = getenv("NERAF_WGRAD_WIDE"); return e ? atoi(e) : 1; }();
  static const int wide_nst = [] { const char* e = getenv("NERAF_WGRAD_WIDE_NST"); const int v = e ? atoi(e) : 2; return (v == 3 || v == 4) ? v : 2; }();
  static const int wide_rounds = [] { const char* e = getenv("NERAF_WGRAD_WIDE_ROUNDS"); return e ? atoi(e) : 4; }();
  static const int wide_waves = [] { const char* e = getenv("NERAF_WGRAD_WAVES"); return (e && atoi(e) == 4) ? 4 : 8; }();
  const int LDS_BYTES = nst * 128 * 128;
  static bool attr_set = false;
  if (!attr_set) {
    NERAF_HIP_CHECK(ctx, hipFuncSetAttribute(reinterpret_cast<const void*>(&wgrad_grouped_tn_kernel<2, false>), hipFuncAttributeMaxDynamicSharedMemorySize, 2 * 128 * 128));
    NERAF_HIP_CHECK(ctx, hipFuncSetAttribute(reinterpret_cast<const void*>(&wgrad_grouped_tn_kernel<3, false>), hipFuncAttributeMaxDynamicSharedMemorySize, 3 * 128 * 128));
    NERAF_HIP_CHECK(ctx, hipFuncSetAttribute(reinterpret_cast<const void*>(&wgrad_grouped_tn_kernel<4, false>), hipFuncAttributeMaxDynamicSharedMemorySize, 4 * 128 * 128));
    NERAF_HIP_CHECK(ctx, hipFuncSetAttribute(reinterpret_cast<const void*>(&wgrad_wide_tn_kernel<2, false>), hipFuncAttributeMaxDynamicSharedMemorySize, 2 * 5 * 8192));
    NERAF_HIP_CHECK(ctx, hipFuncSetAttribute(reinterpret_cast<const void*>(&wgrad_wide_tn_kernel<3, false>), hipFuncAttributeMaxDynamicSharedMemorySize, 3 * 5 * 8192));
    NERAF_HIP_CHECK(ctx, hipFuncSetAttribute(reinterpret_cast<const void*>(&wgrad_wide_tn_kernel<4, false>), hipFuncAttributeMaxDynamicSharedMemorySize, 4 * 5 * 8192));
    NERAF_HIP_CHECK(ctx, hipFuncSetAttribute(reinterpret_cast<const void*>(&wgrad_wide_tn_kernel<2, false, 8>), hipFuncAttributeMaxDynamicSharedMemorySize, 2 * 5 * 8192));
    NERAF_HIP_CHECK(ctx, hipFuncSetAttribute(reinterpret_cast<const void*>(&wgrad_wide_tn_kernel<2, true>), hipFuncAttributeMaxDynamicSharedMemorySize, 2 * 5 * 8192));
    NERAF_HIP_CHECK(ctx, hipFuncSetAttribute(reinterpret_cast<const void*>(&wgrad_grouped_tn_kernel<3, true>), hipFuncAttributeMaxDynamicSharedMemorySize, 3 * 128 * 128));
    attr_set = true;
  }
  const int cus = ctx ? ctx->num_cus : 256;
  WgTable t{};
  WgRedTable r{};
  static const int xcd_order = [] { const char* e = getenv("NERAF_WGRAD_XCD"); return e ? atoi(e) : 0; }();
  t.n = n; t.zero_page = zero_page; t.alpha_dev = alpha_dev; t.slab = slab_ws; t.order = wide ? xcd_order : 0;
  r.alpha_dev = alpha_dev; r.slab = slab_ws;
  double total_steps = 0.0;
  for (int i = 0; i < n; ++i) {
    const WgradItem& it = items[i];
    const int taps = it.ksize * it.ksize * it.ksize;
    total_steps += (double)(it.cout / 64) * (round_up(taps * it.cin, 64) / 64) * (it.K / 64) / (wide ? 4.0 : 1.0);
  }
  int target = (int)(total_steps / (cus * (double)(wide ? wide_rounds : rounds))) + 1;
  if (target < 16) target = 16;
  size_t slab_off = 0; int blocks = 0, red_tiles = 0, nred = 0;
  double flops = 0.0, exec_flops = 0.0;
  for (int i = 0; i < n; ++i) {
    const WgradItem& it = items[i];
    const int taps = it.ksize * it.ksize * it.ksize;
    if ((it.cout % 64) || (it.K % 64) || it.dout <= 0 || (it.dout & (it.dout - 1)) || (it.cin % 64 && it.cin != 8) || taps * it.cin > 65535)
      return neraf_fail(ctx, NERAF_EINVAL, "wgrad_grouped: cout % 64, K % 64, power-of-two output edge, cin % 64 (or the 8-channel stem)");
    WgDesc& d = t.d[i];
    d.dy = it.dy; d.x = it.x; d.out = it.out; d.K = it.K;
    if (it.alpha_idx < 0 || it.alpha_idx > 255) return neraf_fail(ctx, NERAF_EINVAL, "wgrad_grouped: alpha_idx out of range");
    d.ai = (unsigned char)it.alpha_idx;
    d.cout = (unsigned short)it.cout; d.cin = (unsigned short)it.cin; d.cin_real = (unsigned short)it.cin_real; d.taps = (unsigned short)taps;
    d.din = (unsigned short)it.din; d.stride = (unsigned char)it.stride; d.ksize = (unsigned char)it.ksize; d.pad = (signed char)it.pad;
    d.dl = (unsigned char)(31 - __builtin_clz((unsigned)it.dout));
    d.loader = (it.ksize == 1 && it.stride == 1) ? 0 : (it.cin == 8 ? 2 : 1);
    const int tiles_n = round_up(taps * it.cin, 64) / 64, tiles_m = it.cout / 64, nk = it.K / 64;
    d.tiles_n = (unsigned short)tiles_n;
    int splits = (nk + target - 1) / target;
    if (splits > nk / 4) splits = nk / 4;
    if (splits < 1) splits = 1;
    if (splits > 128) splits = 128;
    d.splits = (unsigned short)splits;
    d.block_begin = blocks;
    d.mh = (unsigned char)(it.cout % 128 == 0 ? 2 : 1);
    if (wide) blocks += (it.cout / (64 * d.mh)) * ((tiles_n + (d.mh == 2 ? 2 : 4) - 1) / (d.mh == 2 ? 2 : 4)) * splits;
    else blocks += tiles_m * tiles_n * splits;
    d.slab_off = slab_off;
    if (splits > 1 || taps > 1) {
      slab_off += (size_t)splits * it.cout * tiles_n * 64;
      r.item[nred] = (unsigned char)i; r.tile_begin[nred] = red_tiles; ++nred;
      const int cb = taps == 1 ? (it.cin < 256 ? it.cin : 256) : (taps > 32 ? it.cin : (it.cin < 128 ? it.cin : 128));
      red_tiles += it.cout * (it.cin / cb);
    }
    flops += 2.0 * it.cout * taps * it.cin_real * (double)it.dout * it.dout * it.dout;
    exec_flops += 2.0 * it.cout * (double)tiles_n * 64 * (double)it.K;
  }
  if (slab_off * 4 > slab_bytes) return neraf_fail(ctx, NERAF_EINVAL, "wgrad_grouped: split-K scratch too small");
  t.total_blocks = blocks;
  r.n = nred; r.tile_begin[nred] = red_tiles;
  {
    ProfScope prof(ctx, stream, PROF_WGRAD, flops, exec_flops);
    if (bf16) {
      if (wide) hipLaunchKernelGGL((wgrad_wide_tn_kernel<2, true>), dim3(blocks), dim3(256), 2 * 5 * 8192, stream, t);
      else hipLaunchKernelGGL((wgrad_grouped_tn_kernel<3, true>), dim3(blocks), dim3(256), 3 * 128 * 128, stream, t);
    }
    else if (wide && wide_nst == 2 && wide_waves == 8) hipLaunchKernelGGL((wgrad_wide_tn_kernel<2, false, 8>), dim3(blocks), dim3(512), 2 * 5 * 8192, stream, t);
    else if (wide && wide_nst == 2) hipLaunchKernelGGL((wgrad_wide_tn_kernel<2, false>), dim3(blocks), dim3(256), 2 * 5 * 8192, stream, t);
    else if (wide && wide_nst == 4) hipLaunchKernelGGL((wgrad_wide_tn_kernel<4, false>), dim3(blocks), dim3(256), 4 * 5 * 8192, stream, t);
    else if (wide) hipLaunchKernelGGL((wgrad_wide_tn_kernel<3, false>), dim3(blocks), dim3(256), 3 * 5 * 8192, stream, t);
    else if (nst == 2) hipLaunchKernelGGL((wgrad_grouped_tn_kernel<2, false>), dim3(blocks), dim3(256), LDS_BYTES, stream, t);
    else if (nst == 3) hipLaunchKernelGGL((wgrad_grouped_tn_kernel<3, false>), dim3(blocks), dim3(256), LDS_BYTES, stream, t);
    else hipLaunchKernelGGL((wgrad_grouped_tn_kernel<4, false>), dim3(blocks), dim3(256), LDS_BYTES, stream, t);
  }
  if (nred > 0) hipLaunchKernelGGL(wgrad_grouped_reduce_kernel, dim3(red_tiles), dim3(256), 0, stream, t, r);
  NERAF_HIP_CHECK(ctx, hipGetLastError());
  if (ctx && ctx->manifest) {
    double rb = 0.0, wb = 0.0;
    for (int i = 0; i < n; ++i) {
      const WgradItem& it = items[i];
      const double taps = (double)it.ksize * it.ksize * it.ksize;
      rb += (double)it.K * it.cout * 2.0 + (double)it.din * it.din * it.din * it.cin * 2.0;
      wb += (double)it.cout * it.cin_real * taps * 4.0;
    }
    neraf_node(ctx, "wgrad_ | all 43 weight gradients, TN GEMM", flops, rb, nred > 0 ? (double)slab_off * 4.0 : wb);
    if (nred > 0) neraf_node(ctx, "wgrad_grouped_reduce_kernel | slabs -> [cout][cin][taps]", 0.0, (double)slab_off * 4.0, wb);
  }
  return NERAF_OK;
}


int launch_gemm_f16(neraf_ctx* ctx, const GemmParams& p_in, hipStream_t stream) {
  GemmParams p = p_in;
  if (p.K <= 0 || (p.K % BK) != 0) return neraf_fail(ctx, NERAF_EINVAL, "gemm: K must be a positive multiple of 64");
  if (p.ngroups == 1) {
    const GemmParams::Group& G = p.grp[0];
    p.A = G.A; p.B = G.B; p.C32 = G.C32; p.ldc32 = G.ldc32; p.M = G.M; p.N = G.N;
    p.Mpad = round_up(G.M, 64); p.Npad = round_up(G.N, 64);
    p.ngroups = 0;
  }
  if (p.ngroups > 1) {
    if (p.ngroups > kMaxGemmGroups || p.conv.loader != 0 || p.C16 || p.C16T || p.colsum || p.colsumsq || p.lmask || p.add16)
      return neraf_fail(ctx, NERAF_EINVAL, "gemm: grouped launches are plain GEMMs with fp32 results only");
    for (int g = 0; g < p.ngroups; ++g) {
      const GemmParams::Group& G = p.grp[g];
      if (!G.A || !G.B || !G.C32 || G.M <= 0 || G.N <= 0)
        return neraf_fail(ctx, NERAF_EINVAL, "gemm: every group needs operands, a result and positive M, N");
    }
    if ((p.Mpad && p.Mpad != round_up(p.grp[0].M, 64)) || (p.Npad && p.Npad != round_up(p.grp[0].N, 64)))
      return neraf_fail(ctx, NERAF_EINVAL, "gemm: a grouped launch's Mpad / Npad, if given, are group 0's M / N rounded up to 64");
    p.A = p.grp[0].A; p.B = p.grp[0].B; p.C32 = p.grp[0].C32; p.ldc32 = p.grp[0].ldc32;
    p.M = p.grp[0].M; p.N = p.grp[0].N; p.Mpad = round_up(p.M, 64); p.Npad = round_up(p.N, 64);
  }
  if ((p.Mpad % 64) != 0 || (p.Npad % 64) != 0 || p.M > p.Mpad || p.N > p.Npad || p.M <= 0 || p.N <= 0)
    return neraf_fail(ctx, NERAF_EINVAL, "gemm: Mpad/Npad must be multiples of 64 covering M/N");
  if (!p.stat_det && p.stat_rep > 1 && (p.stat_rep & (p.stat_rep - 1))) return neraf_fail(ctx, NERAF_EINVAL, "gemm: stat_rep must be a power of two");
  if ((p.conv.loader == 0 && (p.lda % 8)) || (p.ldb % 8) || (p.C16 && (p.ldc16 % 8)) || (p.C16T && (p.ldc16t % 8)) ||
      (p.lmask && (p.ldmask % 4)))
    return neraf_fail(ctx, NERAF_EINVAL, "gemm: leading dimensions must keep 16-byte alignment");
  switch (p.conv.loader) {
    case 0: return p.bf16 ? dispatch_tile<0, 1, true>(ctx, p, stream) : dispatch_tile<0, 1, false>(ctx, p, stream);
// ... 78 lines not shown
```

### neraf_amd/csrc/resnet3d_bwd.hip

```cpp
#include "resnet3d_common.h"
#include <algorithm>
#include <mutex>
#include <stddef.h>
#include <stdlib.h>
#include <string.h>
#include <unordered_map>

namespace {

struct PackTTable {
  int n;
  const float* src[kMaxConv];
  int tile_begin[kMaxConv + 1];
  unsigned long long dst_off[kMaxConv];
  int cout[kMaxConv], cin[kMaxConv], taps[kMaxConv], kcols[kMaxConv], nrows[kMaxConv];
};

__global__ __launch_bounds__(256) void pack_dgrad_weights_kernel(PackTTable t, char* __restrict__ packed) {
  extern __shared__ half_t brick[];
  int lo = 0, hi = t.n - 1;
  const int bid = blockIdx.x;
  while (lo < hi) { const int mid = (lo + hi + 1) >> 1; if (t.tile_begin[mid] <= bid) lo = mid; else hi = mid - 1; }
  const int i = lo;
  const int tile = bid - t.tile_begin[i];
// ... 246 lines not shown
  if ((threadIdx.x & 63) == 0) red[threadIdx.x >> 6] = m;
  __syncthreads();
  const float amx = fmaxf(fmaxf(red[0], red[1]), fmaxf(red[2], red[3]));
  int es = 0;
  if (amx > 0.f && amx < 3.0e38f) {
    es = target_log2 - (int)floorf(log2f(amx));
    es = es > 100 ? 100 : (es < -100 ? -100 : es);
  }
  const float S = exp2f((float)es);
  if (blockIdx.x == 0) {
    const int dfeat_bad = __syncthreads_or(nan_seen) || !(amx < 3.0e38f);
    if (threadIdx.x == 0) { scale[0] = S; scale[1] = 1.f / S; }
    if ((int)threadIdx.x < kChainMax) { s_par.p[threadIdx.x] = par.p[threadIdx.x]; s_am[threadIdx.x] = 0u; }
    const bool valid = magic == kChainMagic;
    __syncthreads();
    bool any = false;
#pragma unroll
    for (int k = 0; k < kWords; ++k) {
      const int i = threadIdx.x + k * 256;
      if (i < n_groups * kAmaxRep && v[k]) { amax[(size_t)i * kAmaxStride] = 0u; if (valid) atomicMax(&s_am[i / kAmaxRep], v[k]); any = true; }
    }
    const int recorded = __syncthreads_or(any ? 1 : 0);
    if (threadIdx.x < 64) {
      const int lane = threadIdx.x;
      const bool in = lane < n_groups;
      const unsigned mx = in ? s_am[lane] : 0u;
      const int p = (in && lane > 0) ? s_par.p[lane] : 0;
      const int eo = (in && valid) ? e_in : 0;
      const int eo_p = __shfl(eo, p);
      int ok = (lane == 0 || !in) ? 1 : (mx < 0x477fe000u ? 1 : 0);
      int anc = p;
#pragma unroll
      for (int r = 0; r < 6; ++r) { ok &= __shfl(ok, anc); anc = __shfl(anc, anc); }
      const int okp = __shfl(ok, p);
      const bool measured = okp && mx > 0u && mx < 0x7f800000u;
      const bool blind = okp && in && lane > 0 && mx >= 0x7f800000u;
      int done = (lane == 0 || !in || measured || blind) ? 1 : 0;
      int acc = (lane == 0 || !in) ? 0 : (measured ? eo + kChainTarget - ((int)(mx >> 23) - 127) : (blind ? eo - kChainOverflowStep : eo - eo_p));
      int link = done ? lane : p;
#pragma unroll
      for (int r = 0; r < 6; ++r) {
        const int a2 = __shfl(acc, link), d2 = __shfl(done, link), l2 = __shfl(link, link);
        if (!done) { acc += a2; done = d2; link = l2; }
      }
      const int lim_lo = max(-100, -120 - es), lim_hi = min(100, 120 - es);
      const int e = acc < lim_lo ? lim_lo : (acc > lim_hi ? lim_hi : acc);
      const unsigned long long bad = __ballot(in && !ok);
      if (in) { cs->e[lane] = e; cs->pow2[lane] = exp2f((float)e); cs->inv[lane] = exp2f((float)(-es - e)); }
      if (lane == 0) {
        if (!valid) cs->unsettled = (unsigned)n_groups;
        else if (recorded) cs->unsettled = (unsigned)__popcll(bad);
        cs->passes = valid ? passes_in + 1u : 1u;
        cs->dfeat_bad = dfeat_bad ? 1u : 0u;
        cs->magic = kChainMagic;
      }
    }
  }
  const float k = S / (float)M;
  const size_t total = (size_t)Mpad * C;
  for (size_t idx = (size_t)blockIdx.x * 256 + threadIdx.x; idx < total; idx += (size_t)gridDim.x * 256) {
    const int row = (int)(idx / C), c = (int)(idx % C);
    g[idx] = (half_t)(row < M ? dfeat[c] * k : 0.f);
  }
}

constexpr int kGatherCz = 2, kGatherCy = 4, kGatherCx = 4;
constexpr int kGatherWin = (kGatherCz + 1) * (kGatherCy + 1) * (kGatherCx + 1);
static_assert(kGatherCz * kGatherCy * kGatherCx * 8 == 256, "one cell-chunk per thread");

inline unsigned gather_blocks(int din) {
  const int nc = (din + 1) / 2;
  return (unsigned)(((nc + kGatherCz - 1) / kGatherCz) * ((nc + kGatherCy - 1) / kGatherCy) * ((nc + kGatherCx - 1) / kGatherCx));
}

__global__ __launch_bounds__(256) void maxpool_bwd_gather_kernel(const unsigned char* __restrict__ arg, int din, int dout,
                                                                const half_t* __restrict__ g, half_t* __restrict__ dpost, size_t rows_pad_in) {
  __shared__ unsigned long long s_arg[kGatherWin * 8];
  __shared__ uint4 s_g[kGatherWin * 8];
  const int tid = threadIdx.x;
  const int nc = (din + 1) / 2;
  const int nbx = (nc + kGatherCx - 1) / kGatherCx, nby = (nc + kGatherCy - 1) / kGatherCy;
  const int bx = blockIdx.x % nbx, by = (blockIdx.x / nbx) % nby, bz = blockIdx.x / (nbx * nby);
  const int oz0 = bz * kGatherCz, oy0 = by * kGatherCy, ox0 = bx * kGatherCx;
  {
    constexpr int kSt = (kGatherWin * 8 + 255) / 256;
    unsigned long long am_s[kSt]; uint4 g_s[kSt]; bool inside[kSt];
#pragma unroll
    for (int k = 0; k < kSt; ++k) {
      const int e = min(k * 256 + tid, kGatherWin * 8 - 1);
      const int w = e >> 3;
      const int oz = oz0 + w / ((kGatherCx + 1) * (kGatherCy + 1)), oy = oy0 + (w / (kGatherCx + 1)) % (kGatherCy + 1), ox = ox0 + w % (kGatherCx + 1);
      inside[k] = oz < dout && oy < dout && ox < dout;
      const size_t ov = ((size_t)min(oz, dout - 1) * dout + min(oy, dout - 1)) * dout + min(ox, dout - 1);
      am_s[k] = *reinterpret_cast<const unsigned long long*>(arg + ov * 64 + (e & 7) * 8);
      g_s[k] = *reinterpret_cast<const uint4*>(g + ov * 64 + (e & 7) * 8);
    }
#pragma unroll
    for (int k = 0; k < kSt; ++k) {
      const int e = k * 256 + tid;
      if (e < kGatherWin * 8) { s_arg[e] = inside[k] ? am_s[k] : ~0ull; s_g[e] = inside[k] ? g_s[k] : make_uint4(0u, 0u, 0u, 0u); }
    }
  }
  if (blockIdx.x == 0) {
    const size_t first = cube(din) * 8, total = rows_pad_in * 8;
    for (size_t e = first + tid; e < total; e += 256) reinterpret_cast<uint4*>(dpost)[e] = make_uint4(0u, 0u, 0u, 0u);
  }
  __syncthreads();
  const int ch = tid & 7, lc = tid >> 3;
  const int lx = lc % kGatherCx, ly = (lc / kGatherCx) % kGatherCy, lz = lc / (kGatherCx * kGatherCy);
  unsigned long long am[8];
  half8 gv[8];
#pragma unroll
  for (int k = 0; k < 8; ++k) {
    const int w = ((lz + (k >> 2)) * (kGatherCy + 1) + ly + ((k >> 1) & 1)) * (kGatherCx + 1) + lx + (k & 1);
    am[k] = s_arg[w * 8 + ch];
    const uint4 raw = s_g[w * 8 + ch];
    gv[k] = *reinterpret_cast<const half8*>(&raw);
  }
#pragma unroll
  for (int pz = 0; pz < 2; ++pz)
#pragma unroll
    for (int py = 0; py < 2; ++py)
#pragma unroll
      for (int px = 0; px < 2; ++px) {
        const int iz = 2 * (oz0 + lz) + pz, iy = 2 * (oy0 + ly) + py, ix = 2 * (ox0 + lx) + px;
        if (iz >= din || iy >= din || ix >= din) continue;
        float acc[8];
#pragma unroll
        for (int j = 0; j < 8; ++j) acc[j] = 0.f;
#pragma unroll
        for (int a = 0; a <= pz; ++a)
#pragma unroll
          for (int b = 0; b <= py; ++b)
#pragma unroll
            for (int c = 0; c <= px; ++c) {
              const unsigned tap = (unsigned)((pz ? 2 - 2 * a : 1) * 9 + (py ? 2 - 2 * b : 1) * 3 + (px ? 2 - 2 * c : 1));
              const int k = a * 4 + b * 2 + c;
#pragma unroll
              for (int j = 0; j < 8; ++j)
                if (((am[k] >> (8 * j)) & 0xffu) == tap) acc[j] += (float)gv[k][j];
            }
        half8 o;
#pragma unroll
        for (int j = 0; j < 8; ++j) o[j] = (half_t)acc[j];
        *reinterpret_cast<half8*>(dpost + (((size_t)iz * din + iy) * din + ix) * 64 + ch * 8) = o;
      }
}

__global__ void set_f32x2_kernel(float* p, float a, float b) { if (threadIdx.x == 0 && blockIdx.x == 0) { p[0] = a; p[1] = b; } }
__global__ void set_u64_kernel(unsigned long long* p, unsigned long long v) { if (threadIdx.x == 0 && blockIdx.x == 0) p[0] = v; }

__global__ __launch_bounds__(256) void stem_w_relayout_kernel(const float* __restrict__ W, float* __restrict__ Wt) {
  const int idx = blockIdx.x * 256 + threadIdx.x;
  if (idx >= 125 * 8 * 64) return;
  const int co = idx & 63, c = (idx >> 6) & 7, tap = idx >> 9;
  Wt[idx] = c < 7 ? W[((size_t)co * 7 + c) * 125 + tap] : 0.f;
}

__global__ __launch_bounds__(256) void stem_dgrid_kernel(const half_t* __restrict__ dy, const float* __restrict__ Wt, int S, int dout,
                                                        const unsigned long long* __restrict__ start_dev, int n, int nch,
                                                        const float* __restrict__ inv_scale, float* __restrict__ dgrid) {
  const int lane = threadIdx.x & 63;
  const int i = blockIdx.x * 4 + (threadIdx.x >> 6);
  if (i >= n) return;
  const size_t cell = (size_t)start_dev[0] + i;
  const int x = (int)(cell % S), y = (int)((cell / S) % S), z = (int)(cell / ((size_t)S * S));
  float acc[7] = {0.f, 0.f, 0.f, 0.f, 0.f, 0.f, 0.f};
  for (int dz = 0; dz < 5; ++dz) {
    const int nz = z + 2 - dz; if (nz < 0 || (nz & 1) || (nz >> 1) >= dout) continue;
    for (int dyy = 0; dyy < 5; ++dyy) {
      const int ny = y + 2 - dyy; if (ny < 0 || (ny & 1) || (ny >> 1) >= dout) continue;
      for (int dx = 0; dx < 5; ++dx) {
        const int nx = x + 2 - dx; if (nx < 0 || (nx & 1) || (nx >> 1) >= dout) continue;
        const float d = (float)dy[((size_t)((nz >> 1) * dout + (ny >> 1)) * dout + (nx >> 1)) * 64 + lane];
        const float* w = Wt + (size_t)((dz * 5 + dyy) * 5 + dx) * 512 + lane;
#pragma unroll
        for (int c = 0; c < 7; ++c) if (c < nch) acc[c] = fmaf(d, w[c * 64], acc[c]);
      }
    }
  }
#pragma unroll
  for (int c = 0; c < 7; ++c) {
    if (c >= nch) break;
    float v = acc[c];
#pragma unroll
    for (int o = 32; o > 0; o >>= 1) v += __shfl_xor(v, o);
    if (lane == 0) dgrid[(size_t)c * n + i] = v * inv_scale[0];
  }
}

__global__ void f16_to_f32_kernel(const half_t* __restrict__ a, size_t n, const float* __restrict__ mul, float* __restrict__ o) {
  const size_t i = (size_t)blockIdx.x * blockDim.x + threadIdx.x;
  if (i < n) o[i] = (float)a[i] * mul[0];
}

struct BwdLayout {
  size_t wt[64];
  size_t packed_total;
  size_t scale;
  size_t chain, amax;
  size_t sums[64];
  size_t sums_fin[64];
  size_t sums_begin, sums_bytes;
  size_t g[2];
  size_t dy[64];
  size_t gm, da;
  size_t dpost;
  size_t wtmp;
  size_t splitk; size_t splitk_bytes;
  size_t total;
};

inline int bwd_rows_per_block(const ConvSpec& c) {
  static const int min_rows = [] { const char* e = getenv("NERAF_BN_BWD_MIN_ROWS"); return e ? atoi(e) : 32; }();
  static const int max_blocks = [] { const char* e = getenv("NERAF_BN_BWD_MAX_BLOCKS"); return e ? atoi(e) : 512; }();
  const int M = (int)cube(c.dout);
  return std::max(min_rows, round_up((M + max_blocks - 1) / max_blocks, 32));
}
inline int bwd_stat_rep(const ConvSpec& c) {
  if (2 * round_up(c.cout, 128) > kStatStride) return 1;
  const int M = (int)cube(c.dout), rpb = bwd_rows_per_block(c);
  const int nrb = (M + rpb - 1) / rpb;
  int r = 1;
  while (r < 16 && r * 8 < nrb) r <<= 1;
  return r;
}

void make_bwd_layout(const Arch& A, BwdLayout* L) {
  size_t off = 0;
  auto take = [&](size_t bytes) { size_t o = off; off += round_up_sz(bytes, 256); return o; };
  for (int i = 0; i < A.nconv; ++i) {
    const ConvSpec& c = A.conv[i];
    const int nrows = c.cin == 64 || c.cin == 8 ? 64 : round_up(c.cin, 128);
    L->wt[i] = take((size_t)nrows * c.k * c.k * c.k * c.cout * 2);
  }
  L->packed_total = off;
  off = 0;
  L->scale = take(256);
  L->chain = take(sizeof(ChainState));
  L->amax = take((size_t)kChainMax * kAmaxRep * kAmaxStride * 4);
  L->sums_begin = off;
  for (int i = 0; i < A.nconv; ++i) {
    const int rep = bwd_stat_rep(A.conv[i]);
    if (neraf_deterministic()) L->sums[i] = take(det_slots(A.conv[i]) * 2 * round_up(A.conv[i].cout, 128) * 4);
    else L->sums[i] = take(rep > 1 ? (size_t)rep * kStatStride * 4 : (size_t)2 * round_up(A.conv[i].cout, 128) * 4);
  }
  L->sums_bytes = off - L->sums_begin;
  for (int i = 0; i < A.nconv; ++i) L->sums_fin[i] = take((size_t)2 * round_up(A.conv[i].cout, 128) * 4);
  size_t max_act = 0, max_wtmp = 0;
  for (int i = 0; i < A.nconv; ++i) {
    const ConvSpec& c = A.conv[i];
    const size_t rows_out = rows_pad(c.dout), rows_in = rows_pad(c.din);
    if (i > 0) {
      max_act = std::max(max_act, rows_out * c.cout * 2);
      max_act = std::max(max_act, rows_in * c.cin * 2);
    }
    max_wtmp = std::max(max_wtmp, (size_t)125 * 8 * 64 * 4);
  }
  for (int i = 0; i < 2; ++i) L->g[i] = take(max_act);
  for (int i = 0; i < A.nconv; ++i) L->dy[i] = take(rows_pad(A.conv[i].dout) * A.conv[i].cout * 2);
  L->gm = take(max_act); L->da = take(max_act);
  L->dpost = take(cube(A.conv[0].dout) * 64 * 4);
  L->wtmp = take(max_wtmp);
  L->splitk_bytes = (size_t)192 << 20;
  L->splitk = take(L->splitk_bytes);
  L->total = off;
}

struct Ctx {
  neraf_ctx* ctx; hipStream_t st; const Arch* A; const Layout* L; const BwdLayout* B;
  const char* packed_t; char* ws; char* bws; const float* const* bn; float* const* w_grads; float* const* bn_grads;
  const float* pow2(int t) const { return reinterpret_cast<const ChainState*>(bws + B->chain)->pow2 + t; }
  const float* inv(int t) const { return reinterpret_cast<const ChainState*>(bws + B->chain)->inv + t; }
  const float* inv_base() const { return reinterpret_cast<const ChainState*>(bws + B->chain)->inv; }
  bool track = true;
  unsigned* amax(int t) const { return track ? reinterpret_cast<unsigned*>(bws + B->amax) + (size_t)t * kAmaxRep * kAmaxStride : nullptr; }
};

int bn_backward(const Ctx& c, int ci, const half_t* g16, const float* g32, const half_t* act, half_t* dx, half_t* dy_masked,
                int k_in, int k_out, int k_mask, bool sums_done = false) {
  const ConvSpec& cs = c.A->conv[ci];
  BnBwdArgs p{};
  p.s = bn_src_bwd(*c.A, *c.L, c.ws, c.bn, ci);
  p.g16 = g16; p.g32 = g32; p.act = act;
  p.M = (int)cube(cs.dout); p.Mpad = (int)rows_pad(cs.dout); p.C = cs.cout;
  p.rows_per_block = bwd_rows_per_block(cs);
  p.sums = (float*)(c.bws + c.B->sums[ci]); p.rep = bwd_stat_rep(cs);
  p.dx = dx; p.dy_masked = dy_masked;
  p.dgamma = c.bn_grads[2 * ci]; p.dbeta = c.bn_grads[2 * ci + 1]; p.inv_scale = c.inv(k_in);
  p.osc = c.pow2(k_out); p.isc = c.pow2(k_in); p.msc = dy_masked ? c.pow2(k_mask) : nullptr;
  p.amax_out = c.amax(k_out); p.amax_in = g16 ? c.amax(k_in) : nullptr;
  const int nrb = (p.M + p.rows_per_block - 1) / p.rows_per_block;
  p.det = neraf_deterministic() ? 1 : 0;
  if (!sums_done) hipLaunchKernelGGL(bn_bwd_reduce_kernel, dim3(nrb, p.C / 64), dim3(256), 0, c.st, p);
  if (c.ctx && c.ctx->manifest) {
    char nm[96];
    const double elems = (double)p.M * p.C;
    if (!sums_done) {
      snprintf(nm, sizeof(nm), "bn_bwd_reduce_kernel | M=%d C=%d", p.M, p.C);
      neraf_node(c.ctx, nm, 0.0, elems * (2.0 + (g16 ? 2.0 : 4.0) + (act ? 2.0 : 0.0)), 0.0);
    }
    snprintf(nm, sizeof(nm), "bn_bwd_apply_kernel | M=%d C=%d%s", p.M, p.C, dy_masked ? " + masked copy" : "");
    neraf_node(c.ctx, nm, 0.0, elems * (2.0 + (g16 ? 2.0 : 4.0) + (act ? 2.0 : 0.0)), (double)p.Mpad * p.C * 2.0 * (dy_masked ? 2 : 1));
  }
  static const int skip_small = [] { const char* e = getenv("NERAF_SKIP_SMALL_BN"); return e ? atoi(e) : 0; }();
  if (skip_small >= 2 && cube(cs.dout) <= 4096 && cs.k == 1) return NERAF_OK;
  if (p.det) {
    float* fin = (float*)(c.bws + c.B->sums_fin[ci]);
    run_slot_sum(c.st, p.sums, det_slots(cs), p.s.cpad, 0.f, 0, fin);
    p.sums = fin; p.rep = 1;
  }
  hipLaunchKernelGGL(bn_bwd_apply_kernel, dim3(p.Mpad / 64, p.C / 64), dim3(256), 0, c.st, p);
  NERAF_HIP_CHECK(c.ctx, hipGetLastError());
  return NERAF_OK;
}

inline WgradItem wgrad_item(const Ctx& c, int ci, const half_t* dy, const half_t* x_in, int t_dy) {
  const ConvSpec& cs = c.A->conv[ci];
  WgradItem it{};
  it.dy = dy; it.x = x_in; it.out = c.w_grads[ci];
  it.cout = cs.cout; it.cin = cs.cin; it.cin_real = cs.cin_real; it.ksize = cs.k; it.stride = cs.stride; it.pad = cs.pad;
  it.din = cs.din; it.dout = cs.dout; it.K = (int)rows_pad(cs.dout);
  it.alpha_idx = t_dy;
  return it;
}

int conv_wgrad(const Ctx& c, int ci, const half_t* dy, const half_t* x_in, int t_dy) {
  const WgradItem it = wgrad_item(c, ci, dy, x_in, t_dy);
  return launch_wgrad_grouped(c.ctx, &it, 1, (const half_t*)(c.ws + c.L->zero_page), (float*)(c.bws + c.B->splitk), c.B->splitk_bytes,
                              c.inv_base(), c.st);
}

inline bool fuse_bn_sums(const ConvSpec& bn_conv) {
  static const int on = [] { const char* e = getenv("NERAF_BN_FUSE_SUMS"); return e ? atoi(e) : 1; }();
  static const long max_vox = [] { const char* e = getenv("NERAF_BN_FUSE_MAX_VOX"); return e ? atol(e) : 4096l; }();
  return on && (long)cube(bn_conv.dout) <= max_vox && (bn_conv.cout % 64) == 0;
}

int conv_dgrad(const Ctx& c, int ci, const half_t* dy, const half_t* add16, half_t* dx, int bn_ci = -1, const half_t* bn_act = nullptr) {
  const ConvSpec& cs = c.A->conv[ci];
  GemmParams g{};
  const int taps = cs.k * cs.k * cs.k;
  g.A = (const half_t*)dy; g.lda = cs.cout;
  g.B = (const half_t*)(c.packed_t + c.B->wt[ci]); g.ldb = taps * cs.cout;
  g.M = (int)cube(cs.din); g.N = cs.cin; g.K = taps * cs.cout; g.Mpad = (int)rows_pad(cs.din);
  g.Npad = cs.cin == 64 ? 64 : round_up(cs.cin, 128); g.tile_n = cs.cin == 64 ? 64 : 0; g.alpha = 1.f;
  g.alg_flops = 2.0 * (double)cube(cs.dout) * taps * cs.cin_real * cs.cout;
  g.add16 = (const half_t*)add16; g.ldadd = cs.cin;
  g.C16 = (half_t*)dx; g.ldc16 = cs.cin;
  g.splitk_ws = (float*)(c.bws + c.B->splitk); g.splitk_ws_bytes = c.B->splitk_bytes;
  if (bn_ci >= 0) {
    const ConvSpec& bs = c.A->conv[bn_ci];
    float* sums = (float*)(c.bws + c.B->sums[bn_ci]);
    g.colsum = sums; g.colsumsq = sums + round_up(bs.cout, 128);
    g.stat_rep = bwd_stat_rep(bs); g.stat_stride = kStatStride;
    if (neraf_deterministic()) { g.stat_det = 1; g.stat_rep = 0; g.stat_stride = 2 * round_up(bs.cout, 128); }
    g.bnb_x = (const half_t*)(c.ws + c.L->pre[bn_ci]); g.ldbnb = bs.cout; g.bnb_mask = (const half_t*)bn_act;
    g.bnb_fin = (const float*)(c.ws + c.L->fin[bn_ci]); g.bnb_cpad = round_up(bs.cout, 128);
  }
  if (cs.k == 1 && cs.stride == 1) {
    g.conv.loader = 0;
  } else {
    g.conv.loader = 1; g.conv.cin = cs.cout; g.conv.din = cs.dout; g.conv.dout = cs.din; g.conv.stride = 1; g.conv.pad = -cs.pad;
    g.conv.ksize = cs.k; g.conv.tflip = 1; g.conv.tstride = cs.stride;
    g.conv.zero_page = (const half_t*)(c.ws + c.L->zero_page);
  }
  return launch_gemm_f16(c.ctx, g, c.st);
}

}

extern "C" size_t neraf_resnet3d_bwd_packed_bytes(const neraf_resnet3d_desc* d) {
  Arch A; BwdLayout B;
  if (make_arch(d, &A)) return 0;
  make_bwd_layout(A, &B);
  return B.packed_total;
}

extern "C" size_t neraf_resnet3d_bwd_workspace_bytes(const neraf_resnet3d_desc* d) {
  Arch A; BwdLayout B;
  if (make_arch(d, &A)) return 0;
  make_bwd_layout(A, &B);
  return B.total;
}

extern "C" int neraf_resnet3d_pack_weights_bwd(neraf_ctx* ctx, const neraf_resnet3d_desc* d, const float* const* conv_w, void* packed_t,
                                               neraf_stream_t stream) {
  Arch A; BwdLayout B;
  if (make_arch(d, &A) || !conv_w || !packed_t) return neraf_fail(ctx, NERAF_EINVAL, "resnet3d_pack_weights_bwd: bad arguments");
  make_bwd_layout(A, &B);
  hipStream_t st = (hipStream_t)stream;
  PackTTable t{};
  BrickTable bt{};
  int acc = 0, max_taps = 1, tiles = 0, max_run = 0;
  for (int i = 1; i < A.nconv; ++i) {
    const ConvSpec& c = A.conv[i];
    const int taps = c.k * c.k * c.k;
    const int nrows = c.cin == 64 || c.cin == 8 ? 64 : round_up(c.cin, 128);
    if (brick_packable(c) && nrows == c.cin) {
      const int j = bt.n++;
      int cob, cib;
      brick_shape(c, 1, &cob, &cib);
      bt.src[j] = conv_w[i]; bt.tile_begin[j] = tiles; bt.dst_off[j] = B.wt[i];
      bt.cout[j] = c.cout; bt.cin[j] = c.cin; bt.taps[j] = taps; bt.cib[j] = cib; bt.cob[j] = cob;
      tiles += (c.cout / cob) * (c.cin / cib);
      max_run = std::max(max_run, cob * (cib * taps + 2));
      continue;
    }
    const int j = t.n++;
    t.src[j] = conv_w[i]; t.tile_begin[j] = acc; t.dst_off[j] = B.wt[i];
    t.cout[j] = c.cout; t.cin[j] = c.cin_real; t.taps[j] = taps; t.kcols[j] = taps * c.cout; t.nrows[j] = nrows;
    acc += (c.cout / 32) * (nrows / 32);
    max_taps = std::max(max_taps, taps);
  }
  t.tile_begin[t.n] = acc;
  bt.tile_begin[bt.n] = tiles;
  if (t.n > 0)
    if (int e = launch_pack_dgrad(ctx, t, acc, max_taps, (char*)packed_t, st)) return e;
  if (bt.n > 0) {
    const size_t lds = brick_lds_bytes(max_run);
    static size_t attr_lds = 0;
    if (lds > attr_lds) {
      NERAF_HIP_CHECK(ctx, hipFuncSetAttribute(reinterpret_cast<const void*>(&pack_bricks_kernel<1>),
                                               hipFuncAttributeMaxDynamicSharedMemorySize, (int)lds));
      attr_lds = lds;
    }
    hipLaunchKernelGGL(pack_bricks_kernel<1>, dim3((unsigned)tiles), dim3(256), lds, st, bt, (char*)packed_t);
    NERAF_HIP_CHECK(ctx, hipGetLastError());
  }
  return NERAF_OK;
}

static int resnet3d_bwd_body(neraf_ctx* ctx, const Arch& A, const Layout& L, const BwdLayout& B, const void* packed_t,
                             const float* const* conv_w, const float* const* bn, char* ws, char* bws, const float* dfeat,
                             float* const* w_grads, float* const* bn_grads, int n_cells, int n_ch, float* dgrid_cells, hipStream_t st,
                             bool track) {
  float* scale = (float*)(bws + B.scale);
  neraf_zero_async(st, bws + B.sums_begin, B.sums_bytes);
  neraf_node(ctx, "neraf_zero_kernel | BatchNorm-backward accumulators", 0.0, 0.0, (double)B.sums_bytes);
  const int Mlast = (int)cube(A.final_edge);
  Ctx c{ctx, st, &A, &L, &B, (const char*)packed_t, ws, bws, bn, w_grads, bn_grads};
  c.track = track;
  half_t* g = (half_t*)(bws + B.g[0]);
  half_t* g_next = (half_t*)(bws + B.g[1]);
  ChainParents par{};
  int n_k = 0;
  auto new_k = [&](int parent) { par.p[n_k] = (unsigned char)parent; return n_k++; };
  int k_g = new_k(0);
  const int total_k = 1 + 3 * A.nblock + 1;
  if (total_k > kChainMax) return neraf_fail(ctx, NERAF_EINVAL, "resnet3d_bwd: chain table too small");
  {
    const int Mpad = (int)rows_pad(A.final_edge);
    const size_t n = (size_t)Mpad * A.n_features;
    unsigned blocks = (unsigned)((n + 255) / 256);
    if (blocks > 1024) blocks = 1024;
    ChainParents pp{};
    int k = 1, kg = 0;
    for (int b = A.nblock - 1; b >= 0; --b) { pp.p[k] = (unsigned char)kg; pp.p[k + 1] = (unsigned char)k; pp.p[k + 2] = (unsigned char)(k + 1); kg = k + 2; k += 3; }
    pp.p[k] = (unsigned char)kg;
    hipLaunchKernelGGL(bwd_prologue_kernel, dim3(blocks), dim3(256), 0, st, dfeat, scale, kChainTarget + (int)ceilf(log2f((float)Mlast)), Mlast, Mpad,
                       A.n_features, g, reinterpret_cast<ChainState*>(bws + B.chain), reinterpret_cast<unsigned*>(bws + B.amax), total_k, pp);
    neraf_node(ctx, "bwd_prologue_kernel | S0, scale groups, average-pool backward", 0.0, 4096.0 + (double)total_k * kAmaxRep * 4.0, (double)n * 2.0);
  }
  half_t* gm = (half_t*)(bws + B.gm); half_t* da = (half_t*)(bws + B.da);
  WgradItem items[64]; int n_items = 0;
  bool g_sums_done = false;
  for (int b = A.nblock - 1; b >= 0; --b) {
    const BlockSpec& Bk = A.block[b];
    const int i0 = Bk.conv[0], i1 = Bk.conv[1], i2 = Bk.conv[2];
    const half_t* out = (const half_t*)(ws + L.out[b]);
    const half_t* a1 = (const half_t*)(ws + L.a1[b]);
    const half_t* a2 = (const half_t*)(ws + L.a2[b]);
    const half_t* x_in = b == 0 ? (const half_t*)(ws + L.act_pool) : (const half_t*)(ws + L.out[b - 1]);
    half_t* dy0 = (half_t*)(bws + B.dy[i0]); half_t* dy1 = (half_t*)(bws + B.dy[i1]); half_t* dy2 = (half_t*)(bws + B.dy[i2]);
    half_t* dyds = Bk.ds >= 0 ? (half_t*)(bws + B.dy[Bk.ds]) : nullptr;
    const int k2 = new_k(k_g), k1 = new_k(k2), k0 = new_k(k1);
    if (int e = bn_backward(c, i2, g, nullptr, out, dy2, Bk.ds < 0 ? gm : nullptr, k_g, k2, k0, g_sums_done)) return e;
    g_sums_done = false;
    items[n_items++] = wgrad_item(c, i2, dy2, a2, k2);
    const bool f1 = fuse_bn_sums(A.conv[i1]);
    if (int e = conv_dgrad(c, i2, dy2, nullptr, da, f1 ? i1 : -1, f1 ? a2 : nullptr)) return e;
    if (int e = bn_backward(c, i1, da, nullptr, a2, dy1, nullptr, k2, k1, -1, f1)) return e;
    items[n_items++] = wgrad_item(c, i1, dy1, a1, k1);
    const bool f0 = fuse_bn_sums(A.conv[i0]) && A.conv[i1].stride == 1;
    if (int e = conv_dgrad(c, i1, dy1, nullptr, da, f0 ? i0 : -1, f0 ? a1 : nullptr)) return e;
    if (int e = bn_backward(c, i0, da, nullptr, a1, dy0, nullptr, k1, k0, -1, f0)) return e;
    items[n_items++] = wgrad_item(c, i0, dy0, x_in, k0);
    if (Bk.ds >= 0) {
      if (int e = bn_backward(c, Bk.ds, g, nullptr, out, dyds, nullptr, k_g, k0, -1)) return e;
      items[n_items++] = wgrad_item(c, Bk.ds, dyds, x_in, k0);
      if (int e = conv_dgrad(c, i0, dy0, nullptr, g_next)) return e;
      if (int e = conv_dgrad(c, Bk.ds, dyds, g_next, g_next)) return e;
    } else {
      const bool fg = b > 0 && A.block[b - 1].ds < 0 && fuse_bn_sums(A.conv[A.block[b - 1].conv[2]]);
      if (int e = conv_dgrad(c, i0, dy0, gm, g_next, fg ? A.block[b - 1].conv[2] : -1, fg ? (const half_t*)(ws + L.out[b - 1]) : nullptr)) return e;
      g_sums_done = fg;
    }
    half_t* t = g; g = g_next; g_next = t;
    k_g = k0;
  }
  {
    const ConvSpec& c0 = A.conv[0];
    half_t* dpost = (half_t*)(bws + B.dpost);
    const size_t rp = rows_pad(c0.dout);
    hipLaunchKernelGGL(maxpool_bwd_gather_kernel, dim3(gather_blocks(c0.dout)), dim3(256), 0, st,
                       (const unsigned char*)(ws + L.pool_arg), c0.dout, A.pooled, g, dpost, rp);
    NERAF_HIP_CHECK(ctx, hipGetLastError());
    neraf_node(ctx, "maxpool_bwd_gather_kernel | max-pool routing", 0.0, (double)cube(A.pooled) * 64 * 3.0, (double)rp * 64 * 2.0);
    half_t* dy0 = (half_t*)(bws + B.dy[0]);
    const int k_s = new_k(k_g);
    if (int e = bn_backward(c, 0, dpost, nullptr, nullptr, dy0, nullptr, k_g, k_s, -1)) return e;
    items[n_items++] = wgrad_item(c, 0, dy0, (const half_t*)(ws + L.x0), k_s);
    if (n_cells > 0) {
      float* Wt = (float*)(bws + B.wtmp);
      hipLaunchKernelGGL(stem_w_relayout_kernel, dim3((125 * 8 * 64 + 255) / 256), dim3(256), 0, st, conv_w[0], Wt);
      hipLaunchKernelGGL(stem_dgrid_kernel, dim3((n_cells + 3) / 4), dim3(256), 0, st, dy0, Wt, A.S, c0.dout,
                         reinterpret_cast<const unsigned long long*>(bws + B.scale + 64), n_cells, n_ch, c.inv(k_s), dgrid_cells);
      NERAF_HIP_CHECK(ctx, hipGetLastError());
      neraf_node(ctx, "stem_w_relayout_kernel | W[co][c][tap] -> Wt[tap][c][co]", 0.0, 125.0 * 7 * 64 * 4, 125.0 * 8 * 64 * 4);
      neraf_node(ctx, "stem_dgrid_kernel | grid gradient of the refresh window", 2.0 * n_cells * (125.0 / 8.0) * 64 * n_ch, (double)n_cells * (125.0 / 8.0) * 128.0,
                 (double)n_cells * n_ch * 4.0);
    }
  }
  if (n_k != total_k) return neraf_fail(ctx, NERAF_EINVAL, "resnet3d_bwd: scale group count mismatch");
  (void)par;
  return launch_wgrad_grouped(ctx, items, n_items, (const half_t*)(ws + L.zero_page), (float*)(bws + B.splitk), B.splitk_bytes, c.inv_base(), st);
}

static std::mutex g_calib_mu;
static std::unordered_map<const void*, unsigned> g_calibrated;
constexpr int kMaxCalibrationPasses = 48;

__global__ void chain_set_kernel(ChainState* cs, int e0, int e1, int e2) {
  if (threadIdx.x != 0 || blockIdx.x != 0) return;
  const int e[3] = {e0, e1, e2};
  for (int t = 0; t < 3; ++t) { cs->e[t] = e[t]; cs->pow2[t] = exp2f((float)e[t]); cs->inv[t] = exp2f((float)-e[t]); }
  cs->magic = kChainMagic;
}

extern "C" int neraf_resnet3d_bwd_reset(neraf_ctx* ctx, void* bwd_workspace) {
  (void)ctx;
  std::lock_guard<std::mutex> lk(g_calib_mu);
  g_calibrated.erase(bwd_workspace);
  return NERAF_OK;
}

extern "C" int neraf_resnet3d_bwd(neraf_ctx* ctx, const neraf_resnet3d_desc* d, const void* packed_t, const float* const* conv_w,
                                  const float* const* bn, void* workspace, void* bwd_workspace, const float* dfeat,
                                  float* const* w_grads, float* const* bn_grads, size_t cell_start, int n_cells, int n_ch,
                                  float* dgrid_cells, neraf_stream_t stream) {
  Arch A; Layout L; BwdLayout B;
  if (make_arch(d, &A) || !packed_t || !conv_w || !bn || !workspace || !bwd_workspace || !dfeat || !w_grads || !bn_grads ||
      (n_cells > 0 && (!dgrid_cells || n_ch < 1 || n_ch > 7 || cell_start + (size_t)n_cells > cube(d->grid_size))))
    return neraf_fail(ctx, NERAF_EINVAL, "resnet3d_bwd: bad arguments");
  make_layout(A, &L);
  make_bwd_layout(A, &B);
  hipStream_t st = (hipStream_t)stream;
  char* bws = (char*)bwd_workspace;
  hipLaunchKernelGGL(set_u64_kernel, dim3(1), dim3(64), 0, st, reinterpret_cast<unsigned long long*>(bws + B.scale + 64),
                     (unsigned long long)cell_start);
  static const bool track_env = [] { const char* e = getenv("NERAF_CHAIN_AMAX"); return !(e && atoi(e) == 0); }();
  static const unsigned period = [] { const char* e = getenv("NERAF_CHAIN_AMAX_PERIOD"); const int v = e ? atoi(e) : 4; return (unsigned)(v < 1 ? 1 : v); }();
  auto run = [&](hipStream_t s2, bool track) {
    return resnet3d_bwd_body(ctx, A, L, B, packed_t, conv_w, bn, (char*)workspace, bws, dfeat, w_grads, bn_grads, n_cells, n_ch, dgrid_cells, s2,
                             track);
  };

  bool fresh;
  unsigned pass_no;
  {
    std::lock_guard<std::mutex> lk(g_calib_mu);
    auto it = g_calibrated.find(bwd_workspace);
    fresh = it == g_calibrated.end();
    if (fresh) it = g_calibrated.emplace(bwd_workspace, 0u).first;
    pass_no = it->second++;
  }
  const bool track = track_env && (pass_no % period) == 0;
  auto body = [&](hipStream_t s2) { return run(s2, track); };
  if (fresh) {
    struct ProfPause { neraf_ctx* c; bool was; ProfPause(neraf_ctx* c_) : c(c_), was(c_ && c_->prof) { if (c) c->prof = false; }
                       ~ProfPause() { if (c) c->prof = was; } } pause(ctx);
    auto forget = [&] { std::lock_guard<std::mutex> lk(g_calib_mu); g_calibrated.erase(bwd_workspace); };
    NERAF_HIP_CHECK(ctx, hipMemsetAsync(bws + B.chain, 0, sizeof(ChainState), st));
    bool settled = false, postponed = false;
    unsigned unsettled = 0;
    for (int i = 0; i < kMaxCalibrationPasses && !settled && !postponed; ++i) {
      if (int e = run(st, true)) { forget(); return e; }
      struct { unsigned unsettled, passes, dfeat_bad; } rd = {0u, 0u, 0u};
      static_assert(offsetof(ChainState, dfeat_bad) == offsetof(ChainState, unsettled) + 8, "read as one block");
      hipError_t he = hipMemcpyAsync(&rd, bws + B.chain + offsetof(ChainState, unsettled), sizeof(rd), hipMemcpyDeviceToHost, st);
      if (he == hipSuccess) he = hipStreamSynchronize(st);
      if (he != hipSuccess) { forget(); NERAF_HIP_CHECK(ctx, he); }
      unsettled = rd.unsettled;
      postponed = rd.dfeat_bad != 0;
      settled = i >= 1 && unsettled == 0;
    }
    if (postponed) forget();
    else if (!settled) {
      forget();
      char msg[200];
      snprintf(msg, sizeof(msg), "resnet3d_bwd: the fp16 gradient chain did not calibrate in %d passes (%u scale groups still overflow): "
               "non-finite activations or weights?", kMaxCalibrationPasses, unsettled);
      return neraf_fail(ctx, NERAF_ESTATE, msg);
    }
  }
  ArgHash k;
  k.add(0x62776432u); k.add(d->grid_size); k.add(packed_t); k.ptrs((const void* const*)conv_w, A.nconv);
  k.ptrs((const void* const*)bn, 4 * A.nconv); k.add(workspace); k.add(bwd_workspace); k.add(dfeat);
  k.ptrs((const void* const*)w_grads, A.nconv); k.ptrs((const void* const*)bn_grads, 2 * A.nconv);
  k.add(n_cells); k.add(n_ch); k.add(dgrid_cells); k.add(track);
  return neraf_run_graphed(ctx, st, k.h, body);
}

extern "C" int neraf_resnet3d_bwd_chain_state(neraf_ctx* ctx, const neraf_resnet3d_desc* d, const void* bwd_workspace, int32_t* e_out,
                                              float* amax_out, int n, int32_t* info2, neraf_stream_t stream) {
  Arch A; BwdLayout B;
  if (make_arch(d, &A) || !bwd_workspace || !e_out || !amax_out || n < 1 || n > kChainMax)
    return neraf_fail(ctx, NERAF_EINVAL, "resnet3d_bwd_chain_state: bad arguments");
  make_bwd_layout(A, &B);
  const char* bws = (const char*)bwd_workspace;
  NERAF_HIP_CHECK(ctx, hipStreamSynchronize((hipStream_t)stream));
  ChainState cs;
  NERAF_HIP_CHECK(ctx, hipMemcpy(&cs, bws + B.chain, sizeof(cs), hipMemcpyDeviceToHost));
  std::vector<unsigned> am((size_t)n * kAmaxRep * kAmaxStride);
  NERAF_HIP_CHECK(ctx, hipMemcpy(am.data(), bws + B.amax, am.size() * 4, hipMemcpyDeviceToHost));
  for (int t = 0; t < n; ++t) {
    unsigned mx = 0;
    for (int r = 0; r < kAmaxRep; ++r) mx = std::max(mx, am[((size_t)t * kAmaxRep + r) * kAmaxStride]);
    float f; memcpy(&f, &mx, 4);
    e_out[t] = cs.magic == kChainMagic ? cs.e[t] : 0;
    amax_out[t] = f;
  }
  if (info2) { info2[0] = (int32_t)cs.unsettled; info2[1] = (int32_t)cs.passes; }
  return NERAF_OK;
}

extern "C" int neraf_debug_maxpool_bwd(neraf_ctx* ctx, const void* arg, const void* g, int din, void* dpost, neraf_stream_t stream) {
  if (!arg || !g || !dpost || din < 2 || din > 256) return neraf_fail(ctx, NERAF_EINVAL, "debug_maxpool_bwd: bad arguments");
  hipLaunchKernelGGL(maxpool_bwd_gather_kernel, dim3(gather_blocks(din)), dim3(256), 0, (hipStream_t)stream, (const unsigned char*)arg,
                     din, (din - 1) / 2 + 1, (const half_t*)g, (half_t*)dpost, rows_pad(din));
  NERAF_HIP_CHECK(ctx, hipGetLastError());
  return NERAF_OK;
}

extern "C" int neraf_debug_conv_bn_relu_stage(neraf_ctx* ctx, int cin, int cin_real, int cout, int k, int stride, int pad, int din,
                                              const void* x_f16, const float* w, const float* gamma, const float* beta, const float* g,
                                              void* y_f16, float* dx, float* dw, float* dgamma, float* dbeta, neraf_stream_t stream) {
  hipStream_t st = (hipStream_t)stream;
  Arch A{};
  A.S = din; A.nconv = 1; A.nblock = 0; A.pooled = din; A.final_edge = din; A.n_features = 1024;
  const int dout = (din + 2 * pad - k) / stride + 1;
  A.conv[0] = ConvSpec{cin, cout, k, stride, pad, din, dout, cin_real};
  Layout L{}; BwdLayout B{};
  make_layout(A, &L);
  make_bwd_layout(A, &B);
  const size_t act = std::max(rows_pad(dout) * (size_t)cout, rows_pad(din) * (size_t)cin) * 2 + 256;
  char *ws = nullptr, *bws = nullptr, *packed = nullptr, *packed_t = nullptr, *extra = nullptr;
  NERAF_HIP_CHECK(ctx, hipMalloc(&ws, L.total));
  NERAF_HIP_CHECK(ctx, hipMalloc(&bws, B.total));
  NERAF_HIP_CHECK(ctx, hipMalloc(&packed, L.packed_total));
  NERAF_HIP_CHECK(ctx, hipMalloc(&packed_t, B.packed_total + 256));
  NERAF_HIP_CHECK(ctx, hipMalloc(&extra, 5 * act));
  NERAF_HIP_CHECK(ctx, hipMemsetAsync(ws, 0, L.total, st));
  NERAF_HIP_CHECK(ctx, hipMemsetAsync(bws, 0, B.total, st));
  NERAF_HIP_CHECK(ctx, hipMemsetAsync(extra, 0, 5 * act, st));
  const float* wl[1] = {w};
  {
    PackTable t{};
    t.n = 1; t.src[0] = w; t.begin[0] = 0; t.dst_off[0] = L.w[0]; t.cout[0] = cout; t.cin_real[0] = cin_real; t.cin[0] = cin;
    t.taps[0] = k * k * k; t.kpad[0] = conv_kpad(A.conv[0]); t.begin[1] = (unsigned long long)conv_npad(A.conv[0]) * conv_kpad(A.conv[0]);
    hipLaunchKernelGGL(pack_all_conv_weights_kernel, dim3((unsigned)((t.begin[1] + 255) / 256)), dim3(256), 0, st, t, packed);
  }
  half_t* xin = (half_t*)extra;
  NERAF_HIP_CHECK(ctx, hipMemcpyAsync(xin, x_f16, cube(din) * cin * 2, hipMemcpyDeviceToDevice, st));
  if (int e = run_conv(ctx, st, A, L, 0, packed, ws, xin)) return e;
  const float* bnp[4] = {gamma, beta, gamma, gamma};
  half_t* yact = (half_t*)(extra + act);
  {
    BnApplyArgs a{};
    a.a = bn_src_fwd(A, L, ws, bnp, 0, 1);
    a.M = (int)cube(dout); a.Mpad = (int)rows_pad(dout); a.C = cout; a.relu = 1; a.out = yact;
    if (int e = run_bn_apply(ctx, st, a)) return e;
  }
  NERAF_HIP_CHECK(ctx, hipMemcpyAsync(y_f16, yact, cube(dout) * cout * 2, hipMemcpyDeviceToDevice, st));
  if (dx && cin % 64 == 0) {
    PackTTable t{};
    const int nrows = cin == 64 || cin == 8 ? 64 : round_up(cin, 128);
    t.n = 1; t.src[0] = w; t.tile_begin[0] = 0; t.dst_off[0] = B.wt[0]; t.cout[0] = cout; t.cin[0] = cin_real; t.taps[0] = k * k * k;
    t.kcols[0] = t.taps[0] * cout; t.nrows[0] = nrows;
    t.tile_begin[1] = (cout / 32) * (nrows / 32);
    if (int e = launch_pack_dgrad(ctx, t, t.tile_begin[1], t.taps[0], packed_t, st)) return e;
  }
  float* wg[1] = {dw};
  float* bng[2] = {dgamma, dbeta};
  Ctx c{ctx, st, &A, &L, &B, packed_t, ws, bws, bnp, wg, bng};
  hipLaunchKernelGGL(chain_set_kernel, dim3(1), dim3(64), 0, st, reinterpret_cast<ChainState*>(bws + B.chain), 0, 6, 0);
  half_t* dy = (half_t*)(extra + 2 * act);
  half_t* dxb = (half_t*)(extra + 3 * act);
  if (int e = bn_backward(c, 0, nullptr, g, yact, dy, nullptr, 0, 1, -1)) return e;
  if (int e = conv_wgrad(c, 0, dy, xin, 1)) return e;
  if (dx && cin % 64 == 0) {
    if (int e = conv_dgrad(c, 0, dy, nullptr, dxb)) return e;
    const size_t n = cube(din) * cin;
    hipLaunchKernelGGL(f16_to_f32_kernel, dim3((unsigned)((n + 255) / 256)), dim3(256), 0, st, dxb, n, c.inv(1), dx);
  }
  NERAF_HIP_CHECK(ctx, hipStreamSynchronize(st));
  (void)wl;
  (void)hipFree(ws); (void)hipFree(bws); (void)hipFree(packed); (void)hipFree(packed_t); (void)hipFree(extra);
  return NERAF_OK;
}
```

### neraf_amd/csrc/resnet3d_common.h

```cpp
#pragma once
#include "common.h"

namespace {

constexpr int kMaxConv = 56;
struct ConvSpec { int cin, cout, k, stride, pad, din, dout; int cin_real; };
struct BlockSpec { int conv[3]; int ds; int planes; };

struct Arch {
  int S;
  int nconv;
  ConvSpec conv[64];
  int nblock;
  BlockSpec block[16];
  int pooled;
  int final_edge;
  int n_features;
};

int make_arch(const neraf_resnet3d_desc* d, Arch* A) {
  if (!d || d->in_channels != 7 || (d->n_features != 1024 && d->n_features != 2048) ||
      (d->grid_size != 128 && d->grid_size != 64 && d->grid_size != 256)) return NERAF_EINVAL;
  A->S = d->grid_size;
  A->n_features = d->n_features;
// ... 75 lines not shown
  L->act_pool = take(rows_pad(A.pooled) * 64 * 2);
  for (int b = 0; b < A.nblock; ++b) {
    const ConvSpec& c0 = A.conv[A.block[b].conv[0]]; const ConvSpec& c1 = A.conv[A.block[b].conv[1]];
    const ConvSpec& c2 = A.conv[A.block[b].conv[2]];
    L->a1[b] = take(rows_pad(c0.dout) * c0.cout * 2);
    L->a2[b] = take(rows_pad(c1.dout) * c1.cout * 2);
    L->out[b] = take(rows_pad(c2.dout) * c2.cout * 2);
  }
  L->splitk_bytes = (size_t)64 << 20;
  L->splitk = take(L->splitk_bytes);
  L->pool_arg = take(cube(A.pooled) * 64);
  L->total = off;
}


struct BnSrc {
  const half_t* x;
  const float* stats;
  const float* fin_r;
  float* fin_w;
  const float* gamma; const float* beta; const float* rmean; const float* rvar;
  int cpad, rep;
  int read_mode;
};

__device__ __forceinline__ float stat_ld(const float* p, int mode) {
  if (mode == 2) return __hip_atomic_load(p, __ATOMIC_RELAXED, __HIP_MEMORY_SCOPE_SYSTEM);
  if (mode == 1) return atomicAdd(const_cast<float*>(p), 0.f);
  return *p;
}

inline int bn_stat_read_mode() {
  static const int m = [] { const char* e = getenv("NERAF_BN_STAT_READ"); const int v = e ? atoi(e) : 2; return (v < 0 || v > 2) ? 2 : v; }();
  return m;
}

__device__ __forceinline__ void bn_mean_var(const BnSrc& s, int c, float inv_m, float& mean, float& var) {
  if (s.fin_r) {
    mean = s.fin_r[c]; var = s.fin_r[s.cpad + c];
  } else if (s.stats) {
    float a = 0.f, b = 0.f, a1 = 0.f, b1 = 0.f, a2 = 0.f, b2 = 0.f, a3 = 0.f, b3 = 0.f;
    const int md = s.read_mode;
    const float* q = s.stats + c;
    int r = 0;
    for (; r + 4 <= s.rep; r += 4) {
      a += stat_ld(q + r * kStatStride, md); b += stat_ld(q + r * kStatStride + s.cpad, md);
      a1 += stat_ld(q + (r + 1) * kStatStride, md); b1 += stat_ld(q + (r + 1) * kStatStride + s.cpad, md);
      a2 += stat_ld(q + (r + 2) * kStatStride, md); b2 += stat_ld(q + (r + 2) * kStatStride + s.cpad, md);
      a3 += stat_ld(q + (r + 3) * kStatStride, md); b3 += stat_ld(q + (r + 3) * kStatStride + s.cpad, md);
    }
    for (; r < s.rep; ++r) { a += stat_ld(q + r * kStatStride, md); b += stat_ld(q + r * kStatStride + s.cpad, md); }
    a = (a + a1) + (a2 + a3); b = (b + b1) + (b2 + b3);
    mean = a * inv_m;
    var = fmaxf(b * inv_m - mean * mean, 0.f);
  } else {
    mean = s.rmean[c]; var = s.rvar[c];
  }
}

__device__ __forceinline__ void bn_scale_shift(const BnSrc& s, int c, float inv_m, float& scale, float& shift) {
  float mean, var;
  bn_mean_var(s, c, inv_m, mean, var);
  if (s.fin_w && blockIdx.x == 0) { s.fin_w[c] = mean; s.fin_w[s.cpad + c] = var; }
  const float rstd = rsqrtf(var + 1e-5f);
  scale = s.gamma[c] * rstd;
  shift = s.beta[c] - mean * scale;
}


__global__ __launch_bounds__(1024) void slot_sum_kernel(const float* __restrict__ src, int nslots, int stride, int cpad, float inv_m,
                                                       int to_meanvar, float* __restrict__ dst) {
  __shared__ float part[2][16][64];
  const int col = threadIdx.x & 63, q = threadIdx.x >> 6;
  const int c = blockIdx.x * 64 + col;
  float a = 0.f, b = 0.f;
  for (int sl = q; sl < nslots; sl += 16) { a += src[(size_t)sl * stride + c]; b += src[(size_t)sl * stride + cpad + c]; }
  part[0][q][col] = a; part[1][q][col] = b;
  __syncthreads();
  if (threadIdx.x < 128) {
    const int which = threadIdx.x >> 6;
    float v[16];
#pragma unroll
    for (int k = 0; k < 16; ++k) v[k] = part[which][k][col];
#pragma unroll
    for (int w = 1; w < 16; w <<= 1)
#pragma unroll
      for (int k = 0; k < 16; k += 2 * w) v[k] += v[k + w];
    part[which][0][col] = v[0];
  }
  __syncthreads();
  if (threadIdx.x < 64) {
    const float s0 = part[0][0][col], s1 = part[1][0][col];
    if (to_meanvar) {
      const float mean = s0 * inv_m;
      dst[c] = mean; dst[cpad + c] = fmaxf(s1 * inv_m - mean * mean, 0.f);
    } else {
      dst[c] = s0; dst[cpad + c] = s1;
    }
  }
}

inline void run_slot_sum(hipStream_t st, const float* src, size_t nslots, int cpad, float inv_m, int to_meanvar, float* dst) {
  hipLaunchKernelGGL(slot_sum_kernel, dim3(cpad / 64), dim3(1024), 0, st, src, (int)nslots, 2 * cpad, cpad, inv_m, to_meanvar, dst);
}

inline BnSrc bn_src_fwd(const Arch& A, const Layout& L, char* ws, const float* const* bn, int ci, int use_batch) {
  const ConvSpec& c = A.conv[ci];
  BnSrc s{};
  s.read_mode = bn_stat_read_mode();
  s.x = (const half_t*)(ws + L.pre[ci]);
  s.stats = use_batch ? (const float*)(ws + L.stat[ci]) : nullptr;
  s.fin_w = use_batch ? (float*)(ws + L.fin[ci]) : nullptr;
  if (use_batch && neraf_deterministic()) { s.stats = nullptr; s.fin_w = nullptr; s.fin_r = (const float*)(ws + L.fin[ci]); }
  s.gamma = bn[4 * ci + 0]; s.beta = bn[4 * ci + 1]; s.rmean = bn[4 * ci + 2]; s.rvar = bn[4 * ci + 3];
  s.cpad = round_up(c.cout, 128); s.rep = stat_rep(c);
  return s;
}

inline BnSrc bn_src_bwd(const Arch& A, const Layout& L, const char* ws, const float* const* bn, int ci) {
  const ConvSpec& c = A.conv[ci];
  BnSrc s{};
  s.x = (const half_t*)(ws + L.pre[ci]);
  s.fin_r = (const float*)(ws + L.fin[ci]);
  s.gamma = bn[4 * ci + 0]; s.beta = bn[4 * ci + 1]; s.rmean = bn[4 * ci + 2]; s.rvar = bn[4 * ci + 3];
  s.cpad = round_up(c.cout, 128); s.rep = 1;
  s.read_mode = bn_stat_read_mode();
  return s;
}


struct PackTable {
  int n;
  const float* src[kMaxConv];
  unsigned long long begin[kMaxConv + 1];
  unsigned long long dst_off[kMaxConv];
  int cout[kMaxConv], cin_real[kMaxConv], cin[kMaxConv], taps[kMaxConv], kpad[kMaxConv];
};

__global__ __launch_bounds__(256) void pack_all_conv_weights_kernel(PackTable t, char* __restrict__ packed) {
  const unsigned long long idx = (unsigned long long)blockIdx.x * 256 + threadIdx.x;
  if (idx >= t.begin[t.n]) return;
  int lo = 0, hi = t.n - 1;
  while (lo < hi) { const int mid = (lo + hi + 1) >> 1; if (t.begin[mid] <= idx) lo = mid; else hi = mid - 1; }
  const int i = lo;
  const unsigned long long e = idx - t.begin[i];
  const int kpad = t.kpad[i], cin = t.cin[i];
  const int n = (int)(e / kpad), k = (int)(e % kpad);
  const int tap = k / cin, c = k % cin;
  float v = 0.f;
  if (n < t.cout[i] && tap < t.taps[i] && c < t.cin_real[i]) v = t.src[i][((size_t)n * t.cin_real[i] + c) * t.taps[i] + tap];
  reinterpret_cast<half_t*>(packed + t.dst_off[i])[e] = (half_t)v;
}

struct BrickTable {
  int n;
  const float* src[kMaxConv];
  int tile_begin[kMaxConv + 1];
  unsigned long long dst_off[kMaxConv];
  int cout[kMaxConv], cin[kMaxConv], taps[kMaxConv], cib[kMaxConv], cob[kMaxConv];
};

template <int MODE>
__global__ __launch_bounds__(256) void pack_bricks_kernel(BrickTable t, char* __restrict__ packed) {
  extern __shared__ unsigned short brick16[];
  int lo = 0, hi = t.n - 1;
  const int bid = blockIdx.x;
  while (lo < hi) { const int mid = (lo + hi + 1) >> 1; if (t.tile_begin[mid] <= bid) lo = mid; else hi = mid - 1; }
  const int i = lo;
  const int tile = bid - t.tile_begin[i];
  const int taps = t.taps[i], cin = t.cin[i], cout = t.cout[i], cib = t.cib[i], cob = t.cob[i];
  const int ci_tiles = cin / cib;
  const int co0 = (tile / ci_tiles) * cob, ci0 = (tile % ci_tiles) * cib;
  const int run = cib * taps;
  const int pitch = ((run >> 1) & 1) ? run : run + 2;
  const float* src = t.src[i] + ((size_t)co0 * cin + ci0) * taps;
  {
    const int run4 = run >> 2, total4 = cob * run4;
    const size_t row_stride = (size_t)cin * taps;
    auto put4 = [&](int e, const f32x4& v) {
      const int co_l = e / run4, i4 = e - co_l * run4;
      unsigned short* dst = brick16 + co_l * pitch + 4 * i4;
#pragma unroll
      for (int k = 0; k < 4; ++k) {
        const half_t h = (half_t)v[k];
        dst[k] = *reinterpret_cast<const unsigned short*>(&h);
      }
    };
    auto get4 = [&](int e) {
      const int co_l = e / run4, i4 = e - co_l * run4;
      return reinterpret_cast<const f32x4*>(src + (size_t)co_l * row_stride)[i4];
    };
    int e = threadIdx.x;
    for (; e + 768 < total4; e += 1024) {
      const f32x4 v0 = get4(e), v1 = get4(e + 256), v2 = get4(e + 512), v3 = get4(e + 768);
      put4(e, v0); put4(e + 256, v1); put4(e + 512, v2); put4(e + 768, v3);
    }
    for (; e < total4; e += 256) put4(e, get4(e));
  }
  __syncthreads();
  if (MODE == 0) {
    uint4* out = reinterpret_cast<uint4*>(packed + t.dst_off[i]) + (((size_t)co0 * taps * cin) >> 3);
    const int c8 = cin >> 3, per_row = taps * c8, total = cob * per_row;
    for (int e = threadIdx.x; e < total; e += 256) {
      const int co_l = e / per_row, r = e - co_l * per_row, tap = r / c8, ci = (r - tap * c8) * 8;
      const unsigned short* sp = brick16 + co_l * pitch + ci * taps + tap;
      uint4 v;
      v.x = (unsigned)sp[0] | ((unsigned)sp[taps] << 16);
      v.y = (unsigned)sp[2 * taps] | ((unsigned)sp[3 * taps] << 16);
      v.z = (unsigned)sp[4 * taps] | ((unsigned)sp[5 * taps] << 16);
      v.w = (unsigned)sp[6 * taps] | ((unsigned)sp[7 * taps] << 16);
      out[e] = v;
    }
  } else {
    uint4* out = reinterpret_cast<uint4*>(packed + t.dst_off[i]);
    const int c8 = cout >> 3, per_ci = taps * c8, total = cib * per_ci;
    for (int e = threadIdx.x; e < total; e += 256) {
      const int ci_l = e / per_ci, r = e - ci_l * per_ci, tap = r / c8, co = (r - tap * c8) * 8;
      const unsigned short* sp = brick16 + co * pitch + ci_l * taps + tap;
      uint4 v;
      v.x = (unsigned)sp[0] | ((unsigned)sp[pitch] << 16);
      v.y = (unsigned)sp[2 * pitch] | ((unsigned)sp[3 * pitch] << 16);
      v.z = (unsigned)sp[4 * pitch] | ((unsigned)sp[5 * pitch] << 16);
      v.w = (unsigned)sp[6 * pitch] | ((unsigned)sp[7 * pitch] << 16);
      out[(((size_t)(ci0 + ci_l) * taps * cout) >> 3) + r] = v;
    }
  }
}

inline bool brick_packable(const ConvSpec& c) {
  return c.cin == c.cin_real && (c.cin % 64) == 0 && (c.cout % 64) == 0 && (c.k == 1 || c.k == 3);
}
inline void brick_shape(const ConvSpec& c, int mode, int* cob, int* cib) {
  const int taps = c.k * c.k * c.k, budget = 14336;
  if (mode == 0) {
    *cib = c.cin;
    int b = budget / (c.cin * taps);
    b = b >= 32 ? 32 : (b >= 16 ? 16 : (b >= 8 ? 8 : (b >= 4 ? 4 : (b >= 2 ? 2 : 1))));
    while (c.cout % b) b >>= 1;
    *cob = b;
  } else {
    *cob = c.cout;
    int b = budget / (c.cout * taps);
    b = b >= 32 ? 32 : (b >= 16 ? 16 : (b >= 8 ? 8 : (b >= 4 ? 4 : (b >= 2 ? 2 : 1))));
    while (c.cin % b) b >>= 1;
    if (b < 4) b = 4;
    *cib = b;
  }
}
inline size_t brick_lds_bytes(int max_elems) { return (size_t)max_elems * 2; }

struct BnApplyArgs {
  BnSrc a; BnSrc r; const half_t* res;
  int M, Mpad, C; int relu;
  half_t* out;
};

__global__ __launch_bounds__(256) void bn_apply_kernel(BnApplyArgs p) {
  extern __shared__ __attribute__((aligned(16))) float sm[];
  float* sc = sm; float* sh = sm + p.C; float* scr = sm + 2 * p.C; float* shr = sm + 3 * p.C;
  const float inv_m = 1.f / (float)p.M;
  const int cpr = p.C >> 3;
  const size_t total = (size_t)p.Mpad * cpr;
  size_t idx = (size_t)blockIdx.x * 256 + threadIdx.x;
  half8 x, rr;
  auto issue = [&](size_t i) {
    const size_t row = i / cpr; const int c0 = (int)(i % cpr) * 8;
    if (row < (size_t)p.M) {
      x = *reinterpret_cast<const half8*>(p.a.x + row * p.C + c0);
      if (p.r.x) rr = *reinterpret_cast<const half8*>(p.r.x + row * p.C + c0);
      else if (p.res) rr = *reinterpret_cast<const half8*>(p.res + row * p.C + c0);
    }
  };
  if (idx < total) issue(idx);
  for (int c = threadIdx.x; c < p.C; c += 256) {
    bn_scale_shift(p.a, c, inv_m, sc[c], sh[c]);
    if (p.r.x) bn_scale_shift(p.r, c, inv_m, scr[c], shr[c]);
  }
  __syncthreads();
  while (idx < total) {
    const size_t row = idx / cpr; const int c0 = (int)(idx % cpr) * 8;
    half8 o;
    if (row < (size_t)p.M) {
      float scv[8], shv[8], scrv[8], shrv[8];
      *reinterpret_cast<f32x4*>(scv) = *reinterpret_cast<const f32x4*>(sc + c0); *reinterpret_cast<f32x4*>(scv + 4) = *reinterpret_cast<const f32x4*>(sc + c0 + 4);
      *reinterpret_cast<f32x4*>(shv) = *reinterpret_cast<const f32x4*>(sh + c0); *reinterpret_cast<f32x4*>(shv + 4) = *reinterpret_cast<const f32x4*>(sh + c0 + 4);
      if (p.r.x) {
        *reinterpret_cast<f32x4*>(scrv) = *reinterpret_cast<const f32x4*>(scr + c0); *reinterpret_cast<f32x4*>(scrv + 4) = *reinterpret_cast<const f32x4*>(scr + c0 + 4);
        *reinterpret_cast<f32x4*>(shrv) = *reinterpret_cast<const f32x4*>(shr + c0); *reinterpret_cast<f32x4*>(shrv + 4) = *reinterpret_cast<const f32x4*>(shr + c0 + 4);
      }
#pragma unroll
      for (int j = 0; j < 8; ++j) {
        float v = fmaf((float)x[j], scv[j], shv[j]);
        if (p.r.x) v += fmaf((float)rr[j], scrv[j], shrv[j]);
        else if (p.res) v += (float)rr[j];
        if (p.relu) v = fmaxf(v, 0.f);
        o[j] = (half_t)v;
      }
    } else {
#pragma unroll
      for (int j = 0; j < 8; ++j) o[j] = (half_t)0.f;
    }
    *reinterpret_cast<half8*>(p.out + row * p.C + c0) = o;
    idx += (size_t)gridDim.x * 256;
    if (idx < total) issue(idx);
  }
}

inline int run_conv(neraf_ctx* ctx, hipStream_t st, const Arch& A, const Layout& L, int ci, const char* packed, char* ws,
             const half_t* input) {
  const ConvSpec& c = A.conv[ci];
  GemmParams g{};
  const int M = (int)cube(c.dout);
  g.A = input; g.lda = c.cin;
  g.B = (const half_t*)(packed + L.w[ci]); g.ldb = conv_kpad(c);
  g.M = M; g.N = c.cout; g.K = conv_kpad(c); g.Mpad = (int)rows_pad(c.dout); g.Npad = conv_npad(c); g.alpha = 1.f;
  g.tile_n = c.cout == 64 ? 64 : 0;
  g.alg_flops = 2.0 * (double)cube(c.dout) * (c.k * c.k * c.k) * c.cin_real * c.cout;
  g.C16 = (half_t*)(ws + L.pre[ci]); g.ldc16 = c.cout;
  float* stats = (float*)(ws + L.stat[ci]);
// ... 98 lines not shown
```

Measured before the change: 272.7 million field-samples/s.

## Optimize ResNet3D backward: compact stride-2 dgrad, heavy-first tclass order, stem dgrid rewrite

Adds a compact path for 1x1 stride-2 transposed dgrad that computes only the nonzero rows, and a heavy-class-first, XCD-aware block ordering for 3x3 tclass dgrad with 32x32 tiles when there are few tiles. The LOADER==2 stem conv gets precomputed bound masks and offsets with incremental tap stepping, replacing per-tap divisions. The stem grid-gradient kernel is restructured to load the 27 contributing dy values up front and iterate only over valid parity taps. The stem weight relayout moves into the backward weight-pack kernel so it no longer runs every step. Debug entry points are added for testing. The changes bring more code complexity and more remapping logic that has to be right.

```diff
diff --git a/include/neraf_hip.h b/include/neraf_hip.h
--- a/include/neraf_hip.h
+++ b/include/neraf_hip.h
@@ -252,6 +252,13 @@
                                    const void* x_f16, const float* w, const float* gamma, const float* beta, const float* g,
                                    void* y_f16, float* dx, float* dw, float* dgamma, float* dbeta, neraf_stream_t stream);
 
+int neraf_debug_stem_conv(neraf_ctx* ctx, int din, int cin_real, const void* x_f16, const float* w, void* y_f16, float* sums,
+                          neraf_stream_t stream);
+int neraf_debug_conv_transpose(neraf_ctx* ctx, int cin, int cout, int k, int din, const void* dy_f16, const float* w, void* dx_f16,
+                               int in_place, neraf_stream_t stream);
+int neraf_debug_stem_dgrid(neraf_ctx* ctx, int S, const void* dy_f16, const float* w, unsigned long long start, int n_cells, int n_ch,
+                           float inv_scale, float* out, neraf_stream_t stream);
+
 int neraf_camera_rays(neraf_ctx* ctx, const float* c2w, const float* fx, const float* fy, const float* cx, const float* cy,
                       const float* distortion, int n_cams,
                       const int64_t* cam_idx, int cam_single, const float* coords, int R, int width, float* origins, float* dirs,
diff --git a/neraf_amd/_lib.py b/neraf_amd/_lib.py
--- a/neraf_amd/_lib.py
+++ b/neraf_amd/_lib.py
@@ -190,6 +190,10 @@
     "neraf_debug_maxpool_fwd": (C.c_int, [C.c_void_p, C.c_void_p, c_fpp, C.c_int, C.c_int, C.c_void_p, C.c_void_p, C.c_void_p]),
     "neraf_debug_maxpool_bwd": (C.c_int, [C.c_void_p, C.c_void_p, C.c_void_p, C.c_int, C.c_void_p, C.c_void_p]),
     "neraf_debug_conv_bn_relu_stage": (C.c_int, [C.c_void_p] + [C.c_int] * 7 + [C.c_void_p] * 11),
+    "neraf_debug_stem_conv": (C.c_int, [C.c_void_p, C.c_int, C.c_int, C.c_void_p, C.c_void_p, C.c_void_p, C.c_void_p, C.c_void_p]),
+    "neraf_debug_stem_dgrid": (C.c_int, [C.c_void_p, C.c_int, C.c_void_p, C.c_void_p, C.c_ulonglong, C.c_int, C.c_int, C.c_float, C.c_void_p,
+                                         C.c_void_p]),
+    "neraf_debug_conv_transpose": (C.c_int, [C.c_void_p] + [C.c_int] * 4 + [C.c_void_p] * 3 + [C.c_int, C.c_void_p]),
     "neraf_composite": (C.c_int, [C.c_void_p, C.c_void_p, C.c_void_p, C.c_void_p, C.c_int, C.c_int, C.c_int, C.c_void_p,
                                   C.c_void_p, C.c_void_p, C.c_void_p, C.c_void_p, C.c_void_p, C.c_size_t, C.c_void_p]),
 }
diff --git a/neraf_amd/csrc/gemm_f16.hip b/neraf_amd/csrc/gemm_f16.hip
--- a/neraf_amd/csrc/gemm_f16.hip
+++ b/neraf_amd/csrc/gemm_f16.hip
@@ -46,15 +46,20 @@
   const int x2 = r % h, y2 = (r / h) % h, z2 = r / (h * h);
   z = 2 * z2 + ((cls >> 2) & 1); y = 2 * y2 + ((cls >> 1) & 1); x = 2 * x2 + (cls & 1);
 }
-template <int BM, bool TC>
+template <int BM, int RMAP>
 __device__ __forceinline__ int out_row(const GemmParams& p, int m) {
-  if (!TC) return m;
+  if (RMAP == 0) return m;
   int z, y, x;
-  tclass_coords<BM>(p.conv, m, z, y, x);
+  if (RMAP == 2) {
+    const int h = p.conv.dout >> 1;
+    x = 2 * (m % h); y = 2 * ((m / h) % h); z = 2 * (m / (h * h));
+  } else {
+    tclass_coords<BM>(p.conv, m, z, y, x);
+  }
   return (z * p.conv.dout + y) * p.conv.dout + x;
 }
 
-template <int BM, int BN, bool BF, int WAVES_M = 2, bool TC = false>
+template <int BM, int BN, bool BF, int WAVES_M = 2, int TC = 0>
 __device__ __forceinline__ void gemm_epilogue(const GemmParams& p, f32x4 (&acc)[Tile<BM, BN, WAVES_M>::FM][Tile<BM, BN, WAVES_M>::FN],
                                               char* smem, int bm, int bn, int lane, int wave, int M, int N, float* C32, int ldc32) {
   using T = Tile<BM, BN, WAVES_M>;
@@ -307,14 +312,25 @@
   const int first_m = group * GROUP_M;
   const int gsz = (tiles_m - first_m) < GROUP_M ? (tiles_m - first_m) : GROUP_M;
   const int in_group = bid - group * GROUP_M * tiles_n;
-  const int bm = first_m + in_group % gsz;
-  const int bn = in_group / gsz;
+  int bm = first_m + in_group % gsz;
+  int bn = in_group / gsz;
 
   constexpr bool tclass = LOADER == 1 && TC;
+  constexpr int RMAP = TC ? (LOADER == 1 ? 1 : 2) : 0;
   int t0z = 0, t0y = 0, t0x = 0, cy = KS, cx = KS;
   int nk_total = p.K / BK;
   if (tclass) {
-    const int cls = bm & 7, padc = -p.conv.pad;
+    const int padc = -p.conv.pad;
+    if (KS == 3 && p.conv.tclass == 2) {
+      const int q = nblocks >> 3, pc = q >> 3;
+      const int xcd = blockIdx.x & 7, idx = blockIdx.x >> 3;
+      const int rank = idx / pc, u = idx - rank * pc;
+      const int two = (0x01243567u >> (4 * rank)) & 7;
+      const int cls_h = (padc & 1) ? two : two ^ 7;
+      bm = xcd * (q / tiles_n) + (u / tiles_n) * 8 + cls_h;
+      bn = u % tiles_n;
+    }
+    const int cls = bm & 7;
     t0z = (((cls >> 2) & 1) + padc) & 1; t0y = (((cls >> 1) & 1) + padc) & 1; t0x = ((cls & 1) + padc) & 1;
     const int cz = t0z < KS ? (KS - t0z + 1) >> 1 : 0;
     cy = t0y < KS ? (KS - t0y + 1) >> 1 : 0; cx = t0x < KS ? (KS - t0x + 1) >> 1 : 0;
@@ -377,6 +393,25 @@
       c_off[i] = ((bz * din + by) * din + bx) * p.conv.cin + alc[i] * 8;
     }
   }
+  int sz = 0, sy = 0, sx = 0;
+  if (LOADER == 2) {
+    const int din = p.conv.din;
+    int t = k_begin * 8 + alc[0];
+    sx = t % KS; t /= KS; sy = t % KS; sz = t / KS;
+    if (sz > KS) sz = KS;
+#pragma unroll
+    for (int i = 0; i < A_CH; ++i) {
+      unsigned m = 0;
+#pragma unroll
+      for (int a = 0; a < KS; ++a) {
+        m |= ((unsigned)(az[i] + a) < (unsigned)din ? 1u : 0u) << a;
+        m |= ((unsigned)(ay[i] + a) < (unsigned)din ? 1u : 0u) << (8 + a);
+        m |= ((unsigned)(ax[i] + a) < (unsigned)din ? 1u : 0u) << (16 + a);
+      }
+      c_msk[i] = m;
+      c_off[i] = ((az[i] * din + ay[i]) * din + ax[i]) * 8;
+    }
+  }
 
   typedef __attribute__((address_space(3))) void* lds_ptr_t;
   typedef const __attribute__((address_space(1))) void* gbl_ptr_t;
@@ -424,15 +459,17 @@
       }
     } else {
       const int din = p.conv.din;
+      const unsigned sel = (1u << sz) | (1u << (8 + sy)) | (1u << (16 + sx));
+      const int toff = ((sz * din + sy) * din + sx) * 8;
 #pragma unroll
       for (int i = 0; i < A_CH; ++i) {
-        const int tap = kt * 8 + alc[i];
-        const int dz = tap / (KS * KS), dy = (tap / KS) % KS, dx = tap % KS;
-        const int iz = az[i] + dz, iy = ay[i] + dy, ix = ax[i] + dx;
-        const bool ok = tap < KS * KS * KS && (unsigned)iz < (unsigned)din && (unsigned)iy < (unsigned)din && (unsigned)ix < (unsigned)din;
-        const half_t* src = ok ? p.A + ((size_t)(iz * din + iy) * din + ix) * 8 : p.conv.zero_page;
+        const half_t* src = (c_msk[i] & sel) == sel ? p.A + (c_off[i] + toff) : p.conv.zero_page;
         __builtin_amdgcn_global_load_lds((gbl_ptr_t)src, (lds_ptr_t)(sa + i * (NW * 1024)), 16, 0, 0);
       }
+      constexpr int Q0 = 8 % KS, Q1 = (8 / KS) % KS, Q2 = 8 / (KS * KS);
+      sx += Q0; if (sx >= KS) { sx -= KS; ++sy; }
+      sy += Q1; if (sy >= KS) { sy -= KS; ++sz; }
+      sz += Q2; if (sz > KS) sz = KS;
     }
 #pragma unroll
     for (int i = 0; i < B_CH; ++i)
@@ -515,7 +552,7 @@
       }
     return;
   }
-  gemm_epilogue<BM, BN, BF, 2, tclass>(p, acc, smem, bm, bn, lane, wave, Mg, Ng, C32g, ldc32g);
+  gemm_epilogue<BM, BN, BF, 2, RMAP>(p, acc, smem, bm, bn, lane, wave, Mg, Ng, C32g, ldc32g);
 }
 
 template <int BM, int BN, int NST, bool BF>
@@ -773,7 +810,8 @@
   else
     snprintf(nm, sizeof(nm), "%s<%d, %d | %s M=%d N=%d K=%d%s",
              stream ? "gemm_f16_nt_stream_kernel" : (wide ? "gemm_f16_nt_wide_kernel" : "gemm_f16_nt_pipe_kernel"), bm, bn,
-             loader == 0 ? "plain" : (p.conv.tflip ? "dgrad" : "conv"), p.M, p.N, p.K, splits > 1 ? " splitK" : "");
+             p.conv.tclass == 3 ? "dgrad s2 compact" : (loader == 0 ? "plain" : (p.conv.tflip ? "dgrad" : "conv")), p.M, p.N, p.K,
+             splits > 1 ? " splitK" : "");
   if (splits > 1) {
     neraf_node(ctx, nm, flops, rA + rB, slabs);
     neraf_node(ctx, "splitk_reduce_kernel | K-split slabs -> result", 0.0, slabs + epi_r, epi_w);
@@ -1503,6 +1541,7 @@
 
 static const int kWide = [] { const char* e = getenv("NERAF_GEMM_WIDE"); return e ? atoi(e) : 1; }();
 static const int kSplitMinK = [] { const char* e = getenv("NERAF_SPLIT_MIN_K"); return e ? atoi(e) : 32; }();
+static const int kTile32 = [] { const char* e = getenv("NERAF_TILE32"); return e ? atoi(e) : 128; }();
 
 static bool conv_waves8() { static const bool v = [] { const char* e = getenv("NERAF_CONV_WAVES"); return e && atoi(e) == 8; }(); return v; }
 
@@ -1514,10 +1553,31 @@
   const int cus = ctx ? ctx->num_cus : 256;
   static const int kTclass = [] { const char* e = getenv("NERAF_DGRAD_TCLASS"); return e ? atoi(e) : 1; }();
   p.conv.tclass = 0;
+  if constexpr (LOADER == 1 && KS == 1) {
+    static const int kCompact = [] { const char* e = getenv("NERAF_DGRAD_COMPACT"); return e ? atoi(e) : 1; }();
+    const int h = p.conv.din, rows = h * h * h;
+    if (kCompact && p.conv.tstride == 2 && p.conv.tflip && p.conv.pad == 0 && p.conv.dout == 2 * h && p.ngroups <= 1 &&
+        p.M == 8 * rows && (rows % 64) == 0 && (p.Npad % 64) == 0 && p.lda == p.conv.cin && p.K == p.conv.cin && p.C16 &&
+        p.add16 == p.C16 && p.ldadd == p.ldc16 && !p.lmask && !p.C16T && !p.C32 && !p.colsum && !p.colsumsq && !p.bnb_x && !p.bnb_mask) {
+      p.conv.tclass = 3;
+      p.M = p.Mpad = rows;
+      const int ntiles = (rows / 64) * (p.Npad / 64);
+      if (kTile32 && ntiles <= kTile32) return launch_pipe<32, 32, 4, 0, 1, BF, true>(ctx, p, 1, stream);
+      return launch_pipe<64, 64, 4, 0, 1, BF, true>(ctx, p, 1, stream);
+    }
+  }
   if (LOADER == 1 && kTclass && p.conv.tstride == 2 && p.conv.tflip && (p.conv.dout & 1) == 0 && p.ngroups <= 1 &&
       p.Mpad == p.conv.dout * p.conv.dout * p.conv.dout && (p.Mpad % 512) == 0 && (p.Npad % 64) == 0 && !p.lmask && !p.C16T && !p.C32 &&
       !p.colsum && !p.colsumsq) {
-    p.conv.tclass = 1;
+    static const int kHeavyFirst = [] { const char* e = getenv("NERAF_DGRAD_HEAVY_FIRST"); return e ? atoi(e) : 1; }();
+    if constexpr (LOADER == 1 && KS == 3) {
+      static const int kTclass32 = [] { const char* e = getenv("NERAF_DGRAD_TILE32"); return e ? atoi(e) : 256; }();
+      if (kTclass32 && (p.Mpad / 64) * (p.Npad / 64) <= kTclass32) {
+        p.conv.tclass = (kHeavyFirst && ((p.Mpad / 32) % 64) == 0) ? 2 : 1;
+        return launch_pipe<32, 32, 4, LOADER, KS, BF, true>(ctx, p, 1, stream);
+      }
+    }
+    p.conv.tclass = (KS == 3 && kHeavyFirst && ((p.Mpad / 64) % 64) == 0) ? 2 : 1;
     if constexpr (LOADER == 1) { if (conv_waves8()) return launch_pipe<64, 64, 4, LOADER, KS, BF, true, 8>(ctx, p, 1, stream); }
     return launch_pipe<64, 64, 4, LOADER, KS, BF, LOADER == 1>(ctx, p, 1, stream);
   }
@@ -1559,7 +1619,6 @@
   }
   if (LOADER == 0 && ng == 1 && kWide && bm == 128 && bn == 128 && splits == 1 && ntiles < 2 * cus)
     return launch_wide<128, 128, 3, BF>(ctx, p, 1, stream);
-  static const int kTile32 = [] { const char* e = getenv("NERAF_TILE32"); return e ? atoi(e) : 128; }();
   if constexpr (LOADER == 0) {
     if (ng > 1) {
       if (kTile32 && splits == 1 && ntiles <= kTile32) return launch_pipe<32, 32, 4, LOADER, KS, BF, false, 4, true>(ctx, p, 1, stream);
diff --git a/neraf_amd/csrc/resnet3d_bwd.hip b/neraf_amd/csrc/resnet3d_bwd.hip
--- a/neraf_amd/csrc/resnet3d_bwd.hip
+++ b/neraf_amd/csrc/resnet3d_bwd.hip
@@ -422,9 +422,7 @@
 
 __global__ __launch_bounds__(256) void stem_w_relayout_kernel(const float* __restrict__ W, float* __restrict__ Wt) {
   const int idx = blockIdx.x * 256 + threadIdx.x;
-  if (idx >= 125 * 8 * 64) return;
-  const int co = idx & 63, c = (idx >> 6) & 7, tap = idx >> 9;
-  Wt[idx] = c < 7 ? W[((size_t)co * 7 + c) * 125 + tap] : 0.f;
+  if (idx < kStemWtElems) stem_wt_relayout(W, Wt, idx);
 }
 
 __global__ __launch_bounds__(256) void stem_dgrid_kernel(const half_t* __restrict__ dy, const float* __restrict__ Wt, int S, int dout,
@@ -435,19 +433,49 @@
   if (i >= n) return;
   const size_t cell = (size_t)start_dev[0] + i;
   const int x = (int)(cell % S), y = (int)((cell / S) % S), z = (int)(cell / ((size_t)S * S));
+  const int t0z = z & 1, t0y = y & 1, t0x = x & 1;
+  const int bz = (z + 2 - t0z) >> 1, by = (y + 2 - t0y) >> 1, bx = (x + 2 - t0x) >> 1;
+  bool okz[3], oky[3], okx[3];
+  int sz[3], sy[3], sx[3], tz[3], ty[3], tx[3];
+#pragma unroll
+  for (int j = 0; j < 3; ++j) {
+    const int az = bz - j, ay = by - j, ax = bx - j;
+    okz[j] = t0z + 2 * j < 5 && az >= 0 && az < dout; oky[j] = t0y + 2 * j < 5 && ay >= 0 && ay < dout; okx[j] = t0x + 2 * j < 5 && ax >= 0 && ax < dout;
+    sz[j] = min(max(az, 0), dout - 1); sy[j] = min(max(ay, 0), dout - 1); sx[j] = min(max(ax, 0), dout - 1);
+    tz[j] = min(t0z + 2 * j, 4); ty[j] = min(t0y + 2 * j, 4); tx[j] = min(t0x + 2 * j, 4);
+  }
+  half_t d[27];
+#pragma unroll
+  for (int jz = 0; jz < 3; ++jz)
+#pragma unroll
+    for (int jy = 0; jy < 3; ++jy)
+#pragma unroll
+      for (int jx = 0; jx < 3; ++jx)
+        d[(jz * 3 + jy) * 3 + jx] = dy[((size_t)(sz[jz] * dout + sy[jy]) * dout + sx[jx]) * 64 + lane];
   float acc[7] = {0.f, 0.f, 0.f, 0.f, 0.f, 0.f, 0.f};
-  for (int dz = 0; dz < 5; ++dz) {
-    const int nz = z + 2 - dz; if (nz < 0 || (nz & 1) || (nz >> 1) >= dout) continue;
-    for (int dyy = 0; dyy < 5; ++dyy) {
-      const int ny = y + 2 - dyy; if (ny < 0 || (ny & 1) || (ny >> 1) >= dout) continue;
-      for (int dx = 0; dx < 5; ++dx) {
-        const int nx = x + 2 - dx; if (nx < 0 || (nx & 1) || (nx >> 1) >= dout) continue;
-        const float d = (float)dy[((size_t)((nz >> 1) * dout + (ny >> 1)) * dout + (nx >> 1)) * 64 + lane];
-        const float* w = Wt + (size_t)((dz * 5 + dyy) * 5 + dx) * 512 + lane;
-#pragma unroll
-        for (int c = 0; c < 7; ++c) if (c < nch) acc[c] = fmaf(d, w[c * 64], acc[c]);
+#pragma unroll
+  for (int jz = 0; jz < 3; ++jz) {
+    float w[9][7];
+#pragma unroll
+    for (int jy = 0; jy < 3; ++jy)
+#pragma unroll
+      for (int jx = 0; jx < 3; ++jx) {
+        const float* wp = Wt + (size_t)((tz[jz] * 5 + ty[jy]) * 5 + tx[jx]) * 512 + lane;
+#pragma unroll
+        for (int c = 0; c < 7; ++c) w[jy * 3 + jx][c] = wp[c * 64];
       }
-    }
+#pragma unroll
+    for (int jy = 0; jy < 3; ++jy)
+#pragma unroll
+      for (int jx = 0; jx < 3; ++jx) {
+        const bool ok = okz[jz] && oky[jy] && okx[jx];
+        const float dv = (float)d[(jz * 3 + jy) * 3 + jx];
+#pragma unroll
+        for (int c = 0; c < 7; ++c) {
+          const float a = fmaf(dv, w[jy * 3 + jx][c], acc[c]);
+          acc[c] = (ok && c < nch) ? a : acc[c];
+        }
+      }
   }
 #pragma unroll
   for (int c = 0; c < 7; ++c) {
@@ -607,6 +635,8 @@
   return on && (long)cube(bn_conv.dout) <= max_vox && (bn_conv.cout % 64) == 0;
 }
 
+inline bool stem_wt_packed(const Arch& A) { return A.conv[0].k == 5 && A.conv[0].cin_real == 7 && A.conv[0].cout == 64; }
+
 int conv_dgrad(const Ctx& c, int ci, const half_t* dy, const half_t* add16, half_t* dx, int bn_ci = -1, const half_t* bn_act = nullptr) {
   const ConvSpec& cs = c.A->conv[ci];
   GemmParams g{};
@@ -687,7 +717,13 @@
   bt.tile_begin[bt.n] = tiles;
   if (t.n > 0)
     if (int e = launch_pack_dgrad(ctx, t, acc, max_taps, (char*)packed_t, st)) return e;
+  const bool stem_wt = stem_wt_packed(A);
+  if (stem_wt && bt.n == 0) {
+    hipLaunchKernelGGL(stem_w_relayout_kernel, dim3((kStemWtElems + 255) / 256), dim3(256), 0, st, conv_w[0], (float*)((char*)packed_t + B.wt[0]));
+    NERAF_HIP_CHECK(ctx, hipGetLastError());
+  }
   if (bt.n > 0) {
+    if (stem_wt) { bt.stem_w = conv_w[0]; bt.stem_off = B.wt[0]; tiles += (kStemWtElems + 1023) / 1024; }
     const size_t lds = brick_lds_bytes(max_run);
     static size_t attr_lds = 0;
     if (lds > attr_lds) {
@@ -782,13 +818,13 @@
     if (int e = bn_backward(c, 0, dpost, nullptr, nullptr, dy0, nullptr, k_g, k_s, -1)) return e;
     items[n_items++] = wgrad_item(c, 0, dy0, (const half_t*)(ws + L.x0), k_s);
     if (n_cells > 0) {
-      float* Wt = (float*)(bws + B.wtmp);
-      hipLaunchKernelGGL(stem_w_relayout_kernel, dim3((125 * 8 * 64 + 255) / 256), dim3(256), 0, st, conv_w[0], Wt);
+      if (!stem_wt_packed(A)) return neraf_fail(ctx, NERAF_EINVAL, "resnet3d_bwd: the grid gradient needs the 7 -> 64 channel 5x5x5 stem");
+      const float* Wt = (const float*)((const char*)packed_t + B.wt[0]);
       hipLaunchKernelGGL(stem_dgrid_kernel, dim3((n_cells + 3) / 4), dim3(256), 0, st, dy0, Wt, A.S, c0.dout,
                          reinterpret_cast<const unsigned long long*>(bws + B.scale + 64), n_cells, n_ch, c.inv(k_s), dgrid_cells);
       NERAF_HIP_CHECK(ctx, hipGetLastError());
-      neraf_node(ctx, "stem_w_relayout_kernel | W[co][c][tap] -> Wt[tap][c][co]", 0.0, 125.0 * 7 * 64 * 4, 125.0 * 8 * 64 * 4);
-      neraf_node(ctx, "stem_dgrid_kernel | grid gradient of the refresh window", 2.0 * n_cells * (125.0 / 8.0) * 64 * n_ch, (double)n_cells * (125.0 / 8.0) * 128.0,
+      neraf_node(ctx, "stem_dgrid_kernel | grid gradient of the refresh window", 2.0 * n_cells * (125.0 / 8.0) * 64 * n_ch,
+                 (double)n_cells * 27.0 * 128.0 + 125.0 * 7 * 64 * 4,
                  (double)n_cells * n_ch * 4.0);
     }
   }
@@ -979,3 +1015,83 @@
   (void)hipFree(ws); (void)hipFree(bws); (void)hipFree(packed); (void)hipFree(packed_t); (void)hipFree(extra);
   return NERAF_OK;
 }
+
+extern "C" int neraf_debug_stem_conv(neraf_ctx* ctx, int din, int cin_real, const void* x_f16, const float* w, void* y_f16, float* sums,
+                                     neraf_stream_t stream) {
+  if (!x_f16 || !w || !y_f16 || !sums || din < 2 || din > 256 || (din & 1) || cin_real < 1 || cin_real > 8)
+    return neraf_fail(ctx, NERAF_EINVAL, "debug_stem_conv: bad arguments");
+  hipStream_t st = (hipStream_t)stream;
+  const ConvSpec c{8, 64, 5, 2, 2, din, din / 2, cin_real};
+  const size_t wbytes = (size_t)conv_npad(c) * conv_kpad(c) * 2;
+  char *packed = nullptr, *zero = nullptr;
+  NERAF_HIP_CHECK(ctx, hipMalloc(&packed, wbytes));
+  NERAF_HIP_CHECK(ctx, hipMalloc(&zero, 256));
+  NERAF_HIP_CHECK(ctx, hipMemsetAsync(zero, 0, 256, st));
+  NERAF_HIP_CHECK(ctx, hipMemsetAsync(sums, 0, 256 * 4, st));
+  PackTable t{};
+  t.n = 1; t.src[0] = w; t.begin[0] = 0; t.dst_off[0] = 0; t.cout[0] = 64; t.cin_real[0] = cin_real; t.cin[0] = 8;
+  t.taps[0] = 125; t.kpad[0] = conv_kpad(c); t.begin[1] = (unsigned long long)conv_npad(c) * conv_kpad(c);
+  hipLaunchKernelGGL(pack_all_conv_weights_kernel, dim3((unsigned)((t.begin[1] + 255) / 256)), dim3(256), 0, st, t, packed);
+  GemmParams g{};
+  g.A = (const half_t*)x_f16; g.lda = 8;
+  g.B = (const half_t*)packed; g.ldb = conv_kpad(c);
+  g.M = (int)cube(c.dout); g.N = 64; g.K = conv_kpad(c); g.Mpad = (int)rows_pad(c.dout); g.Npad = 64; g.alpha = 1.f; g.tile_n = 64;
+  g.C16 = (half_t*)y_f16; g.ldc16 = 64;
+  g.colsum = sums; g.colsumsq = sums + 128;
+  g.conv.loader = 2; g.conv.din = din; g.conv.dout = c.dout; g.conv.stride = 2; g.conv.pad = 2; g.conv.ksize = 5; g.conv.cin = 8;
+  g.conv.zero_page = (const half_t*)zero;
+  const int e = launch_gemm_f16(ctx, g, st);
+  NERAF_HIP_CHECK(ctx, hipStreamSynchronize(st));
+  (void)hipFree(packed); (void)hipFree(zero);
+  return e;
+}
+
+extern "C" int neraf_debug_conv_transpose(neraf_ctx* ctx, int cin, int cout, int k, int din, const void* dy_f16, const float* w,
+                                          void* dx_f16, int in_place, neraf_stream_t stream) {
+  if (!dy_f16 || !w || !dx_f16 || (k != 1 && k != 3) || din < 2 || din > 64 || (din & 1) || (cube(din) % 128) || cin < 64 || (cin % 64) ||
+      cout < 64 || (cout % 64))
+    return neraf_fail(ctx, NERAF_EINVAL, "debug_conv_transpose: bad arguments");
+  hipStream_t st = (hipStream_t)stream;
+  Arch A{};
+  A.S = din; A.nconv = 1; A.nblock = 0; A.pooled = din; A.final_edge = din; A.n_features = 1024;
+  A.conv[0] = ConvSpec{cin, cout, k, 2, k / 2, din, din / 2, cin};
+  Layout L{}; BwdLayout B{};
+  make_layout(A, &L);
+  make_bwd_layout(A, &B);
+  char *ws = nullptr, *bws = nullptr, *packed_t = nullptr;
+  NERAF_HIP_CHECK(ctx, hipMalloc(&ws, L.total));
+  NERAF_HIP_CHECK(ctx, hipMalloc(&bws, B.total));
+  NERAF_HIP_CHECK(ctx, hipMalloc(&packed_t, B.packed_total + 256));
+  NERAF_HIP_CHECK(ctx, hipMemsetAsync(ws + L.zero_page, 0, 256, st));
+  PackTTable t{};
+  const int nrows = cin == 64 ? 64 : round_up(cin, 128);
+  t.n = 1; t.src[0] = w; t.tile_begin[0] = 0; t.dst_off[0] = B.wt[0]; t.cout[0] = cout; t.cin[0] = cin; t.taps[0] = k * k * k;
+  t.kcols[0] = t.taps[0] * cout; t.nrows[0] = nrows;
+  t.tile_begin[1] = (cout / 32) * (nrows / 32);
+  int e = launch_pack_dgrad(ctx, t, t.tile_begin[1], t.taps[0], packed_t, st);
+  if (!e) {
+    Ctx c{ctx, st, &A, &L, &B, packed_t, ws, bws, nullptr, nullptr, nullptr};
+    e = conv_dgrad(c, 0, (const half_t*)dy_f16, in_place ? (const half_t*)dx_f16 : nullptr, (half_t*)dx_f16);
+  }
+  NERAF_HIP_CHECK(ctx, hipStreamSynchronize(st));
+  (void)hipFree(ws); (void)hipFree(bws); (void)hipFree(packed_t);
+  return e;
+}
+
+extern "C" int neraf_debug_stem_dgrid(neraf_ctx* ctx, int S, const void* dy_f16, const float* w, unsigned long long start, int n_cells,
+                                      int n_ch, float inv_scale, float* out, neraf_stream_t stream) {
+  if (!dy_f16 || !w || !out || S < 2 || S > 256 || (S & 1) || n_cells < 1 || n_ch < 1 || n_ch > 7 || start + (size_t)n_cells > cube(S))
+    return neraf_fail(ctx, NERAF_EINVAL, "debug_stem_dgrid: bad arguments");
+  hipStream_t st = (hipStream_t)stream;
+  char* tmp = nullptr;
+  NERAF_HIP_CHECK(ctx, hipMalloc(&tmp, 256 + (size_t)kStemWtElems * 4));
+  hipLaunchKernelGGL(set_u64_kernel, dim3(1), dim3(64), 0, st, reinterpret_cast<unsigned long long*>(tmp), start);
+  hipLaunchKernelGGL(set_f32x2_kernel, dim3(1), dim3(64), 0, st, reinterpret_cast<float*>(tmp + 64), inv_scale, 0.f);
+  hipLaunchKernelGGL(stem_w_relayout_kernel, dim3((kStemWtElems + 255) / 256), dim3(256), 0, st, w, reinterpret_cast<float*>(tmp + 256));
+  hipLaunchKernelGGL(stem_dgrid_kernel, dim3((n_cells + 3) / 4), dim3(256), 0, st, (const half_t*)dy_f16, reinterpret_cast<const float*>(tmp + 256),
+                     S, S / 2, reinterpret_cast<const unsigned long long*>(tmp), n_cells, n_ch, reinterpret_cast<const float*>(tmp + 64), out);
+  NERAF_HIP_CHECK(ctx, hipGetLastError());
+  NERAF_HIP_CHECK(ctx, hipStreamSynchronize(st));
+  (void)hipFree(tmp);
+  return NERAF_OK;
+}
diff --git a/neraf_amd/csrc/resnet3d_common.h b/neraf_amd/csrc/resnet3d_common.h
--- a/neraf_amd/csrc/resnet3d_common.h
+++ b/neraf_amd/csrc/resnet3d_common.h
@@ -251,7 +251,14 @@
   reinterpret_cast<half_t*>(packed + t.dst_off[i])[e] = (half_t)v;
 }
 
+constexpr int kStemWtElems = 125 * 8 * 64;
+__device__ __forceinline__ void stem_wt_relayout(const float* __restrict__ W, float* __restrict__ Wt, int idx) {
+  const int co = idx & 63, c = (idx >> 6) & 7, tap = idx >> 9;
+  Wt[idx] = c < 7 ? W[((size_t)co * 7 + c) * 125 + tap] : 0.f;
+}
+
 struct BrickTable {
+  const float* stem_w; unsigned long long stem_off;
   int n;
   const float* src[kMaxConv];
   int tile_begin[kMaxConv + 1];
@@ -264,6 +271,14 @@
   extern __shared__ unsigned short brick16[];
   int lo = 0, hi = t.n - 1;
   const int bid = blockIdx.x;
+  if (MODE == 1 && bid >= t.tile_begin[t.n]) {
+    float* Wt = reinterpret_cast<float*>(packed + t.stem_off);
+    for (int e = threadIdx.x; e < 1024; e += 256) {
+      const int idx = (bid - t.tile_begin[t.n]) * 1024 + e;
+      if (idx < kStemWtElems) stem_wt_relayout(t.stem_w, Wt, idx);
+    }
+    return;
+  }
   while (lo < hi) { const int mid = (lo + hi + 1) >> 1; if (t.tile_begin[mid] <= bid) lo = mid; else hi = mid - 1; }
   const int i = lo;
   const int tile = bid - t.tile_begin[i];
```

After: 276.1 million field-samples/s, median of 6. 1.01x the previous value.
